# Wangkkklll/GausPcc

Measured on AMD Instinct MI355X. Metric: Mpoints/s encode+decode @1M anchors, higher is better.
Workload: dtype f32

## Files before the change

gauspcc_amd/csrc/codec.hip:

```cpp
#include <algorithm>
#include <chrono>

#include "hostcoder.hpp"
#include "codec_shared.hpp"
#include "container.hpp"
#include "rangecoder_dev.hpp"

using namespace gpcc;

namespace {

constexpr int ENC_RETRY_SMALLER_CHUNKS = -1000;
constexpr int DEC_RETRY_UNFUSED = -1001;

struct PosLevels {
    int L;
    uint32_t cbase[MAXLV], lohi_base[MAXLV], slots[MAXLV], nch[MAXLV];
    int clog[MAXLV];
    const uint32_t *m2r[MAXLV];
};

__global__ __launch_bounds__(256) void k_set_pos(PosLevels S, int64_t nC, uint32_t *__restrict__ pos_out, uint32_t *__restrict__ slots_out)
{
    const int64_t i = (int64_t)blockIdx.x * 256 + threadIdx.x;
// ... 70 lines not shown
    static const bool v0_device = dev_env_int("GAUSPCC_V0_DEVICE_CODER", 0) != 0;
    const int64_t no_origin[3] = {0, 0, 0};
    if (!chunk_log2 && !v0_device) {
        const Level *base = &T.lv[0];
        TAKE(base_xyz, int32_t, 3 * base->n);
        TAKE(base_occ, uint8_t, base->n);
        GP_TRY(level_to_raster(ctx, st, base, T.bias, base_xyz, base_occ));
        const size_t off_w = 0, off_pairs = ((size_t)4 * (size_t)std::max<int64_t>(lohi_words, 1) + 63) & ~(size_t)63;
        const size_t off_bx = off_pairs + 8 * (size_t)NCOUNTERS, off_bo = off_bx + 12 * (size_t)base->n;
        GP_TRY(ctx->hcoder.reserve(off_bo + (size_t)base->n + 64));
        uint8_t *hc = ctx->hcoder.p;
        {
            StageTimer tm(ctx, st, ST_CODER, (double)coded * 4 * 4);
            if (lohi_words) HIP_TRY(hipMemcpyAsync(hc + off_w, lohi, 4 * (size_t)lohi_words, hipMemcpyDeviceToHost, st));
        }
        HIP_TRY(hipMemcpyAsync(hc + off_pairs, pairs_dev, 8 * NCOUNTERS, hipMemcpyDeviceToHost, st));
        HIP_TRY(hipMemcpyAsync(hc + off_bx, base_xyz, 12 * (size_t)base->n, hipMemcpyDeviceToHost, st));
        HIP_TRY(hipMemcpyAsync(hc + off_bo, base_occ, (size_t)base->n, hipMemcpyDeviceToHost, st));
        ht.mark("enc all queued");
        HIP_TRY(hipStreamSynchronize(st));
        ht.mark("enc network done (sync)");
        std::vector<const uint32_t *> sp((size_t)std::max(nstreams, 1));
        std::vector<int64_t> sn((size_t)std::max(nstreams, 1));
        {
            const uint32_t *w = reinterpret_cast<const uint32_t *>(hc + off_w);
            int64_t pre = 0; int si = 0;
            for (int d = 1; d < L; ++d) {
                const int64_t nc = T.lv[d].n;
                for (int s = 0; s < 4; ++s, ++si) { sp[(size_t)si] = w + pre + (int64_t)s * nc; sn[(size_t)si] = nc; }
                pre += 4 * nc;
            }
        }
        std::vector<std::vector<uint8_t>> sb;
        GP_TRY(host_encode_streams(sp.data(), sn.data(), nstreams, &sb, 0));
        ht.mark("enc streams coded (host)");
        size_t fsize = 2 + 4 + 13 * (size_t)base->n + 2;
        for (int si = 0; si < nstreams; ++si) fsize += 4 + sb[(size_t)si].size();
        GP_TRY(ctx->hbytes.reserve(fsize + 16));
        uint8_t *out = ctx->hbytes.p;
        out[0] = (uint8_t)posq; out[1] = (uint8_t)(posq >> 8);
        size_t pos = 2 + base_block_put(out + 2, base->n, reinterpret_cast<const int32_t *>(hc + off_bx), no_origin, hc + off_bo, nstreams);
        for (int si = 0; si < nstreams; ++si) {
            const std::vector<uint8_t> &b = sb[(size_t)si];
            put32(out + pos, (uint32_t)b.size()); pos += 4;
            if (!b.empty()) memcpy(out + pos, b.data(), b.size());
            pos += b.size();
        }
        if (pos != fsize) return fail(GPCC_ERR_HIP, "internal: container size mismatch (%zu vs %zu)", pos, fsize);
        if (ctx->prof.on && ctx->prof.stages) ctx->prof.stage_bytes[ST_CODER] += 3.0 * (double)(fsize - (2 + 4 + 13 * (size_t)base->n + 2 + 4 * (size_t)nstreams));
        const unsigned long long *hp = reinterpret_cast<const unsigned long long *>(hc + off_pairs);
        unsigned long long set_pairs[2];
        sum_set_pairs(hp, L, set_pairs);
        if (ctx->prof.on) GP_TRY(prof_collect(ctx, set_pairs, 2));
        *bytes_out = out; *nbytes_out = (int64_t)pos;
        if (stats) fill_stats(stats, n, pos, T, coded, set_pairs, hp);
        return GPCC_OK;
    }
    LaneList lanes;
    std::vector<uint32_t> gaps;
    std::vector<uint32_t> stream_first(nstreams + 1, 0);
    {
        int64_t pre = 0; int si = 0;
        uint32_t gap = 0;
        for (int d = 1; d < L; ++d) {
            const int64_t nc = T.lv[d].n;
            const RcPlan pl = plan(nc);
            for (int s = 0; s < 4; ++s, ++si) {
                stream_first[si] = (uint32_t)lanes.chunks.size();
                gap += 4u;
                GP_TRY(lanes_append(&lanes, si, pre + (int64_t)s * slots(nc), nc, pl));
                gaps.insert(gaps.end(), pl.nlanes, chunk_log2 ? (uint32_t)si : gap);
            }
            pre += 4 * slots(nc);
        }
        stream_first[nstreams] = (uint32_t)lanes.chunks.size();
    }
    const std::vector<RcChunk> &chunks = lanes.chunks;
    const uint32_t max_syms = lanes.max_syms;
    const size_t table_bound = lanes.table_bound;
    const int nchunks = (int)chunks.size();
    const Level *base = &T.lv[0];
    TAKE(base_xyz, int32_t, 3 * base->n);
    TAKE(base_occ, uint8_t, base->n);
    GP_TRY(level_to_raster(ctx, st, base, T.bias, base_xyz, base_occ));
    const size_t off_desc = 0, off_cnt = off_desc + sizeof(RcChunk) * (size_t)std::max(nchunks, 1);
    const size_t off_pairs = off_cnt + 4 * (size_t)std::max(nchunks, 1) + 8, off_bx = off_pairs + 8 * NCOUNTERS, off_bo = off_bx + 12 * (size_t)base->n;
    const size_t off_gap = (off_bo + (size_t)base->n + 63) & ~(size_t)63;
    const size_t off_sf = off_gap + 4 * (size_t)std::max(nchunks, 1);
    GP_TRY(ctx->hstage.reserve(off_sf + 4 * (size_t)(nstreams + 1) + 64));
    const uint32_t gap_bound = 4u * (uint32_t)nstreams + (chunk_log2 ? (uint32_t)table_bound : 0u);
    uint8_t *hs = ctx->hstage.p;
    uint32_t total_payload = 0;
    uint8_t *payload_dev = nullptr;
    bool direct = false;
    const size_t pos0_hdr = (chunk_log2 ? 8 + 4 * (size_t)L + 4 : 2) + 4 + 13 * (size_t)base->n + 2;
    if (nchunks) {
        memcpy(hs + off_desc, chunks.data(), sizeof(RcChunk) * (size_t)nchunks);
        memcpy(hs + off_gap, gaps.data(), 4 * (size_t)nchunks);
        memcpy(hs + off_sf, stream_first.data(), 4 * (size_t)(nstreams + 1));
        const uint32_t stride = rc_scratch_stride(max_syms);
        TAKE(dchunks, RcChunk, nchunks);
        TAKE(dgap, uint32_t, nchunks);
        HIP_TRY(hipMemcpyAsync(dgap, hs + off_gap, 4 * (size_t)nchunks, hipMemcpyHostToDevice, st));
        TAKE(dcnt, uint32_t, nchunks + 1);
        TAKE(doff, uint32_t, nchunks + 1);
        TAKE(scratch, uint8_t, (size_t)nchunks * stride);
        HIP_TRY(hipMemcpyAsync(dchunks, hs + off_desc, sizeof(RcChunk) * (size_t)nchunks, hipMemcpyHostToDevice, st));
        StageTimer tm(ctx, st, ST_CODER, (double)coded * 4 * 4);
        GP_TRY(rc_encode_launch(st, lohi, dchunks, nchunks, scratch, stride, dcnt, chunk_log2 ? rc_coder_of_version(CONTAINER_VERSION) : RC_CODER_CARRYLESS));
        GP_TRY(dbg_mark(ctx, st, 10, dcnt, (size_t)nchunks * 4));
        GP_TRY(exclusive_scan_u32(ctx, st, dcnt, doff, nchunks, doff + nchunks));
        HIP_TRY(hipMemcpyAsync(hs + off_cnt, dcnt, 4 * (size_t)nchunks, hipMemcpyDeviceToHost, st));
        HIP_TRY(hipMemcpyAsync(hs + off_cnt + 4 * (size_t)nchunks, doff + nchunks, 4, hipMemcpyDeviceToHost, st));
        TAKE(payload, uint8_t, (size_t)nchunks * stride + gap_bound + 32);
        if (chunk_log2) {
            TAKE(dsf, uint32_t, nstreams + 1);
            TAKE(dlst, uint32_t, nchunks);
            TAKE(dgap_total, uint32_t, 1);
            HIP_TRY(hipMemcpyAsync(dsf, hs + off_sf, 4 * (size_t)(nstreams + 1), hipMemcpyHostToDevice, st));
            HIP_TRY(hipMemcpyAsync(dlst, hs + off_gap, 4 * (size_t)nchunks, hipMemcpyHostToDevice, st));
            GP_TRY(rc_layout_launch(st, dcnt, dsf, nstreams, dlst, nchunks, true, dgap, dgap_total));
            const size_t worst = pos0_hdr + (size_t)nchunks * stride + gap_bound + 64;
            GP_TRY(ctx->hbytes.reserve(worst));
            const uint32_t mis = (uint32_t)(pos0_hdr & 15);
            GP_TRY(rc_compact_launch(st, scratch, stride, dcnt, doff, dgap, nchunks, payload + mis, dchunks));
            GP_TRY(rc_to_host_launch(st, payload, doff + nchunks, mis, dgap_total, ctx->hbytes.p + (pos0_hdr - mis)));
            direct = true;
        } else {
            GP_TRY(rc_compact_launch(st, scratch, stride, dcnt, doff, dgap, nchunks, payload));
        }
        payload_dev = payload;
    }
    HIP_TRY(hipMemcpyAsync(hs + off_pairs, pairs_dev, 8 * NCOUNTERS, hipMemcpyDeviceToHost, st));
    HIP_TRY(hipMemcpyAsync(hs + off_bx, base_xyz, 12 * (size_t)base->n, hipMemcpyDeviceToHost, st));
    HIP_TRY(hipMemcpyAsync(hs + off_bo, base_occ, (size_t)base->n, hipMemcpyDeviceToHost, st));
    ht.mark("enc all queued");
    HIP_TRY(hipStreamSynchronize(st));
    ht.mark("enc coded (sync)");
    const uint32_t *hcnt = reinterpret_cast<const uint32_t *>(hs + off_cnt);
    if (nchunks) total_payload = hcnt[nchunks];
    if (ctx->prof.on && ctx->prof.stages) ctx->prof.stage_bytes[ST_CODER] += 3.0 * total_payload;
    const unsigned long long *hp = reinterpret_cast<const unsigned long long *>(hs + off_pairs);
    unsigned long long set_pairs[2];
    sum_set_pairs(hp, L, set_pairs);
    if (ctx->prof.on) GP_TRY(prof_collect(ctx, set_pairs, 2));
    std::vector<StreamSize> ssz((size_t)nstreams);
    size_t tables = 0;
    for (int si = 0; si < nstreams; ++si) {
        const StreamSize z = stream_size(hcnt, (int)stream_first[si], (int)stream_first[si + 1], si, chunk_log2 != 0);
        static const uint32_t test_cap = (uint32_t)env_int("GAUSPCC_TEST_CHUNK_BYTES", 0);
        if (!z.fits || (chunk_log2 > 7 && test_cap && z.max_chunk > test_cap)) {
            (void)fail(GPCC_ERR_ARG, "a chunk of stream %d takes %u bytes, more than the decoder's window holds at chunk_log2 = %d: use a smaller chunk_log2", si, z.max_chunk, chunk_log2);
            return ENC_RETRY_SMALLER_CHUNKS;
        }
        ssz[(size_t)si] = z;
        tables += z.tab;
    }
    size_t fsize = pos0_hdr + 4 * (size_t)nstreams + total_payload + tables;
    if (direct) { if (fsize + 16 > ctx->hbytes.cap) return fail(GPCC_ERR_HIP, "internal: payload beyond its bound"); }
    else GP_TRY(ctx->hbytes.reserve(fsize + 16));
    uint8_t *out = ctx->hbytes.p;
    size_t pos = 0;
    if (chunk_log2) {
        int64_t level_nodes[MAXLV];
        for (int d = 0; d < L; ++d) level_nodes[d] = T.lv[d].n;
        pos = chunked_header_put(out, CONTAINER_VERSION, chunk_log2, posq, L, level_nodes, n);
    } else {
        out[0] = (uint8_t)posq; out[1] = (uint8_t)(posq >> 8); pos = 2;
    }
    pos += base_block_put(out + pos, base->n, reinterpret_cast<const int32_t *>(hs + off_bx), no_origin, hs + off_bo, nstreams);
    {
        const size_t pos0 = pos, body = (size_t)total_payload + 4 * (size_t)nstreams + tables;
        if (pos0 != pos0_hdr) return fail(GPCC_ERR_HIP, "internal: header size mismatch");
        if (body && !direct) { HIP_TRY(hipMemcpyAsync(out + pos0, payload_dev, body, hipMemcpyDeviceToHost, st)); HIP_TRY(hipStreamSynchronize(st)); }
        size_t p = pos0;
        for (int si = 0; si < nstreams; ++si) {
            p += stream_head_put(out + p, hcnt, (int)stream_first[si], (int)stream_first[si + 1], ssz[(size_t)si], chunk_log2 != 0) + ssz[(size_t)si].pay;
        }
        pos = p;
    }
    ht.mark("enc payload d2h");
    if (pos != fsize) return fail(GPCC_ERR_HIP, "internal: container size mismatch (%zu vs %zu)", pos, fsize);
    *bytes_out = out; *nbytes_out = (int64_t)pos;
    if (stats) fill_stats(stats, n, pos, T, coded, set_pairs, hp);
    return GPCC_OK;
}

struct DecTail { const uint32_t *tot[MAXLV + 1]; int ntot; const unsigned long long *pairs; const uint32_t *tmo; };
__global__ __launch_bounds__(64) void k_dec_tail(DecTail t, uint32_t *__restrict__ h_tot, unsigned long long *__restrict__ h_pairs, uint32_t *__restrict__ h_tmo)
{
    const int l = (int)threadIdx.x;
    if (l < t.ntot) h_tot[l] = *t.tot[l];
    if (l < MAXLV) h_pairs[l] = t.pairs[l];
    if (l == 0) *h_tmo = t.tmo ? *t.tmo : 0u;
}

int decode_body(gpcc_ctx *ctx, const gpcc_model *m, const uint8_t *in, int64_t nbytes, const int32_t **xyz_out, int64_t *n_out,
                uint16_t *posq_out, gpcc_stats *stats, hipStream_t st, int32_t *out_user, int64_t out_cap)
{
    ctx->arena.reset();
    HostTrace ht;

    ContainerHdr hdr;
    GP_TRY(container_parse(in, nbytes, &hdr));
    const bool v1 = hdr.chunked;
    const int chunk_log2 = hdr.chunk_log2, version = hdr.version;
    const int L = hdr.L;
    int64_t lvl_n[MAXLV] = {0};
    for (int d = 0; d < MAXLV; ++d) lvl_n[d] = hdr.lvl_n[d];
    const int64_t npts_hdr = hdr.npts, bn = hdr.bn;
    const uint8_t *bxyz = hdr.bxyz, *bocc = hdr.bocc;
    const std::vector<int64_t> &s_len = hdr.s_len;
    *posq_out = hdr.posq;
    int64_t bias_base[3] = {CB >> L, CB >> L, CB >> L}, bias_leaf[3] = {CB, CB, CB};
    int64_t lo[3] = {INT64_MAX, INT64_MAX, INT64_MAX}, hi[3] = {INT64_MIN, INT64_MIN, INT64_MIN};
    {
        for (int64_t i = 0; i < bn; ++i)
            for (int a = 0; a < 3; ++a) { const int64_t c = (int32_t)get32(bxyz + 12 * i + 4 * a); lo[a] = std::min(lo[a], c); hi[a] = std::max(hi[a], c); }
        bool inside = true;
        for (int a = 0; a < 3; ++a) inside = inside && lo[a] + (int64_t)(CB >> L) >= 0 && hi[a] + (int64_t)(CB >> L) < ((int64_t)1 << (21 - L));
        if (!inside)
            for (int a = 0; a < 3; ++a) { bias_base[a] = -lo[a]; bias_leaf[a] = -lo[a] * ((int64_t)1 << L); }
    }
    std::vector<BaseNode> bnodes;
    GP_TRY(base_nodes_append(bxyz, bocc, bn, bias_base, (int64_t)1 << (21 - L), "", &bnodes));
    int hb = 1;
    for (int a = 0; a < 3; ++a) { int b = 0; uint64_t v = (uint64_t)(lo[a] + bias_base[a]) ^ (uint64_t)(hi[a] + bias_base[a]); while (v) { ++b; v >>= 1; } hb = std::max(hb, b); }

    TAKE(dbytes, uint8_t, nbytes + 16);
    GP_TRY(ctx->side_init());
    hipStream_t sd = ctx->side;
    SideGuard side_guard{sd, ctx->xfer};
    HIP_TRY(hipMemcpyAsync(dbytes, in, (size_t)nbytes, hipMemcpyHostToDevice, ctx->xfer));
    HIP_TRY(hipEventRecord(ctx->ev_bytes, ctx->xfer));
    size_t desc_total = 0;
    for (int g = 0; g + 1 < L; ++g) desc_total += 4 * (size_t)rc_plan(v1 ? lvl_n[g + 1] : 0, chunk_log2, version).nlanes;
    const size_t desc_off = (4096 + 16 * (size_t)bn + 63) & ~(size_t)63;
    GP_TRY(ctx->hstage.reserve(desc_off + sizeof(RcChunk) * desc_total + 64));
    RcChunk *hdesc = reinterpret_cast<RcChunk *>(ctx->hstage.p + desc_off);
    size_t desc_used = 0;
    uint32_t win_bytes[MAXLV][4] = {};
    auto level_chunks = [&](int g, int64_t nc, size_t *at) -> int {
        const RcPlan pl = rc_plan(nc, chunk_log2, version);
        if (desc_used + (size_t)4 * pl.nlanes > desc_total) return fail(GPCC_ERR_FORMAT, "level %d: chunk tables exceed the header's level sizes", g + 1);
        RcChunk *lanes = hdesc + desc_used;
        *at = desc_used;
        desc_used += (size_t)4 * pl.nlanes;
        GP_TRY(container_level_tables(in, hdr, g, nc, lanes, win_bytes[g]));
        return GPCC_OK;
    };
    RcChunk *dchunks_all = nullptr;
    size_t desc_at[MAXLV] = {0};
    if (v1 && L > 1) {
        for (int g = 0; g + 1 < L; ++g)
            if (lvl_n[g + 1] <= 0 || lvl_n[g + 1] > 8 * lvl_n[g]) return fail(GPCC_ERR_FORMAT, "bad node count at level %d", g + 1);
        TAKE(dca, RcChunk, std::max<size_t>(desc_total, 1));
        dchunks_all = dca;
    }
    constexpr int TAB_EARLY = 6;
    int tab_parsed = 0;
    auto upload_tables = [&](int g_end, hipEvent_t ev) -> int {
        const size_t from = desc_used;
        for (; tab_parsed < g_end && tab_parsed + 1 < L; ++tab_parsed) GP_TRY(level_chunks(tab_parsed, lvl_n[tab_parsed + 1], &desc_at[tab_parsed]));
        if (desc_used > from) HIP_TRY(hipMemcpyAsync(dchunks_all + from, hdesc + from, sizeof(RcChunk) * (desc_used - from), hipMemcpyHostToDevice, ctx->xfer));
        HIP_TRY(hipEventRecord(ev, ctx->xfer));
        return GPCC_OK;
    };
    Level cur;
    GP_TRY(alloc_level(ctx, &cur, bn, L));
    {
        uint64_t *hr = reinterpret_cast<uint64_t *>(ctx->hstage.p + 1024);
        uint8_t *ho = ctx->hstage.p + 1024 + 8 * (size_t)bn;
        for (int64_t i = 0; i < bn; ++i) { hr[i] = bnodes[(size_t)i].rk; ho[i] = bnodes[(size_t)i].occ; }
        HIP_TRY(hipMemcpyAsync(cur.rkey, hr, 8 * (size_t)bn, hipMemcpyHostToDevice, st));
        HIP_TRY(hipMemcpyAsync(cur.occ, ho, (size_t)bn, hipMemcpyHostToDevice, st));
        ht.mark("dec parse+h2d queued");
    }
    GP_TRY(level_raster_rank(ctx, st, &cur, hb));
    TAKE(dtotal, uint32_t, 4);
    uint32_t *htotal = reinterpret_cast<uint32_t *>(ctx->hstage.p);
    const int NPc = cell_map_entries(m->k);
    const int64_t zero_base[1] = {0};
    TAKE(pairs_dev, unsigned long long, MAXLV);
    HIP_TRY(hipMemsetAsync(pairs_dev, 0, sizeof(unsigned long long) * MAXLV, st));
    ConvTiles tilesP;
    int32_t *cellP = nullptr;
    {
        TAKE(cm, int32_t, (int64_t)NPc * bn);
        cellP = cm;
        const TileLevel tl = {&cur, nullptr, nullptr, cellP};
        const int R = conv_pick_rows(bn, m->k);
        TilePool pool;
        GP_TRY(tiles_build(ctx, st, &tl, 1, m->k, R, conv_pick_height(bn, R), &pool, pairs_dev));
        GP_TRY(tiles_view(ctx, st, pool, 0, 1, zero_base, &tilesP));
    }
    int64_t coded = 0;
    DecTail tail = {};
    const bool fuse_ctx = fused_enabled() && !ctx->fused_off && v1 && version >= 1 && m->C == 32;
    const int fmode = fused_mode();
    PairPlan planP;
    int64_t planP_np = 0;
    bool any_fused = false;
    HIP_TRY(hipEventRecord(ctx->ev_main, st));
    for (int g = 0; g + 1 < L; ++g) {
        const size_t top_mk = ctx->arena.top_mark();
        const int64_t np = cur.n;
        float *pA = nullptr;
        GP_TRY(dec_parent_trunk(ctx, st, m, g, cur.occ, np, tilesP, planP, planP_np, fmode, &pA, &any_fused));
        HIP_TRY(hipStreamWaitEvent(sd, ctx->ev_main, 0));
        Level chi;
        int64_t nc = lvl_n[g + 1];
        if (!v1) {
            GP_TRY(level_expand(ctx, sd, &cur, nullptr, dtotal));
            HIP_TRY(hipMemcpyAsync(htotal, dtotal, 4, hipMemcpyDeviceToHost, sd));
            HIP_TRY(hipStreamSynchronize(sd));
            nc = htotal[0];
            lvl_n[g + 1] = nc;
        }
        if (nc <= 0 || nc > 8 * cur.n) return fail(GPCC_ERR_FORMAT, "bad node count at level %d", g + 1);
        GP_TRY(alloc_level(ctx, &chi, nc, L - g - 1));
        {
            const int hbl = std::min(21, std::max(1, hb + g + 1));
            StageTimer tm(ctx, sd, ST_OCTREE, (double)np * 13 + (double)nc * 12 + (double)cdiv(3 * hbl, 8) * (double)nc * 24 + (double)nc * 8);
            GP_TRY(level_expand_rank(ctx, sd, &cur, &chi, v1 ? nullptr : dtotal, hb + g + 1));
            tail.tot[1 + g] = cur.cstart + np;
        }
        int32_t *cellC = nullptr;
        if (g + 2 < L) { TAKE(cm, int32_t, (int64_t)NPc * nc); cellC = cm; }
        if (v1 && g == 0) GP_TRY(upload_tables(TAB_EARLY, ctx->ev_bytes));
        const RcPlan pl = rc_plan(nc, chunk_log2, version);
        ConvTiles tilesC;
        PairPlan planC;
        const bool child_plan = fuse_ctx && fused_level_ok(nc, m->k) && pl.dual == (version >= 3) && fused_windows_fit(nc, cur.n, pl.nlanes, win_bytes[g]);
        GP_TRY(dec_child_lists(ctx, sd, m, &cur, cellP, &chi, cellC, child_plan, pairs_dev + g + 1, &planC, &tilesC));
        GP_TRY(dbg_mark(ctx, sd, g * 100 + 3, chi.rkey, (size_t)nc * 8)); GP_TRY(dbg_mark(ctx, sd, g * 100 + 4, chi.parent, (size_t)nc * 4));
        GP_TRY(dbg_mark(ctx, sd, g * 100 + 5, chi.m2r, (size_t)nc * 4));
        if (!child_plan) { GP_TRY(dbg_mark(ctx, sd, g * 100 + 6, tilesC.first, (size_t)(tilesC.nblk + 1) * 4)); GP_TRY(dbg_mark(ctx, sd, g * 100 + 7, tilesC.order, (size_t)tilesC.nblk * 4)); }
        HIP_TRY(hipEventRecord(ctx->ev_side, sd));
        HIP_TRY(hipStreamWaitEvent(st, ctx->ev_side, 0));
        const int64_t S = chunk_log2 ? (int64_t)1 << pl.llog : nc;
        const int nch = (int)pl.nlanes;
        const int clog = pl.llog;
        const RcChunk *dchunks = nullptr;
        if (v1) {
            dchunks = dchunks_all + desc_at[g];
        } else {
            size_t at = 0;
            GP_TRY(level_chunks(g, nc, &at));
            TAKE(dch, RcChunk, 4 * nch);
            HIP_TRY(hipMemcpyAsync(dch, hdesc + at, sizeof(RcChunk) * 4 * (size_t)nch, hipMemcpyHostToDevice, st));
            dchunks = dch;
        }
        LevelCoder lc = {nullptr, nullptr, (uint32_t)nch, clog, dchunks, {win_bytes[g][0], win_bytes[g][1], win_bytes[g][2], win_bytes[g][3]}, pl.dual, rc_coder_of_version(version)};
        ChildBufs cb;
        GP_TRY(child_bufs_take(ctx, m, nc, child_plan ? planC.pcap : 0, lc.nlanes, S, nc + 4, &cb));
        uint8_t *const *sym = cb.sym;
        uint16_t *const cdf = cb.cdf;
        if (child_plan && fmode == 1) {
            if (g == 0) HIP_TRY(hipStreamWaitEvent(st, ctx->ev_bytes, 0));
            if (g == TAB_EARLY) HIP_TRY(hipStreamWaitEvent(st, ctx->ev_tables, 0));
            GP_TRY(dec_child_fused(ctx, st, m, g, planC, pA, np, chi, dbytes, lc, cb));
            any_fused = true;
        } else {
        GP_TRY(dec_child_trunk(ctx, st, m, g, pA, chi, tilesC, child_plan ? &planC : nullptr, cb));
        for (int s = 0; s < 4; ++s) {
            GP_TRY(dec_child_stage(ctx, st, m, g, s, chi, tilesC, child_plan ? &planC : nullptr, lc, cb));
            const int row_bytes = stage_row_bytes(s);
            if (g == 0 && s == 0) HIP_TRY(hipStreamWaitEvent(st, ctx->ev_bytes, 0));
            if (g == TAB_EARLY && s == 0) HIP_TRY(hipStreamWaitEvent(st, ctx->ev_tables, 0));
            static const bool v0_device = dev_env_int("GAUSPCC_V0_DEVICE_CODER", 0) != 0;
            if (!v1 && !v0_device) {
                const int lp = STAGE_M[s] + 1, rs = rc_row_stride(lp);
                const size_t rows_b = (size_t)nc * (size_t)rs * 2, off_sym = (rows_b + 63) & ~(size_t)63;
                {
                    const size_t need = off_sym + (size_t)nc + 64;
                    if (need > ctx->hcoder.cap) GP_TRY(ctx->hcoder.reserve(std::max(need, 4 * ctx->hcoder.cap)));
                }
                StageTimer tm(ctx, st, ST_CODER, (double)nc * (row_bytes + 1) + (double)s_len[4 * g + s]);
                HIP_TRY(hipMemcpyAsync(ctx->hcoder.p, cdf, rows_b, hipMemcpyDeviceToHost, st));
                HIP_TRY(hipStreamSynchronize(st));
                GP_TRY(host_decode_compact(reinterpret_cast<const uint16_t *>(ctx->hcoder.p), lp, in + hdr.s_off[(size_t)(4 * g + s)], s_len[(size_t)(4 * g + s)], nc,
                                           ctx->hcoder.p + off_sym));
                HIP_TRY(hipMemcpyAsync(sym[s], ctx->hcoder.p + off_sym, (size_t)nc, hipMemcpyHostToDevice, st));
                HIP_TRY(hipStreamSynchronize(st));
            } else {
                StageTimer tm(ctx, st, ST_CODER, (double)nc * (row_bytes + 1) + (double)s_len[4 * g + s]);
                GP_TRY(rc_decode_launch(st, cdf, STAGE_M[s] + 1, dbytes, dchunks + (size_t)s * nch, nch, win_bytes[g][s], pl.dual, sym[s], rc_coder_of_version(version)));
            }
            GP_TRY(dbg_mark(ctx, st, g * 100 + 14 + 5 * s, sym[s], (size_t)nc));
        }
        { StageTimer tm(ctx, st, ST_ELEM, (double)nc * (4 + 4 + 1)); GP_TRY(assemble_occ(st, sym, chi.m2r, nc, chi.occ)); }
        }
        GP_TRY(dbg_mark(ctx, st, g * 100 + 30, chi.occ, (size_t)nc));
        HIP_TRY(hipEventRecord(ctx->ev_main, st));
        if (v1 && g == 0) GP_TRY(upload_tables(L, ctx->ev_tables));
        ctx->arena.top_rewind(top_mk);
        coded += nc;
        cur = chi; cellP = cellC; tilesP = tilesC; planP = child_plan ? planC : PairPlan(); planP_np = np;
        ht.mark("dec level queued", g + 1, nc);
    }
    GP_TRY(level_expand(ctx, st, &cur, nullptr, v1 ? nullptr : dtotal));
    if (!v1) HIP_TRY(hipMemcpyAsync(htotal, dtotal, 4, hipMemcpyDeviceToHost, st));
    tail.tot[0] = cur.cstart + cur.n;
    int64_t npts = npts_hdr;
    if (!v1) {
        HIP_TRY(hipStreamSynchronize(st));
        ht.mark("dec levels done (sync)");
        npts = htotal[0];
    }
    int32_t *xyz = out_user;
    if (out_user) {
        if (npts > out_cap) return fail(GPCC_ERR_ARG, "decoded %lld points, the output buffer holds %lld", (long long)npts, (long long)out_cap);
    } else {
        TAKE(own, int32_t, 3 * std::max<int64_t>(npts, 1));
        xyz = own;
    }
    GP_TRY(leaves_reference_order(ctx, st, &cur, bias_leaf, xyz, npts));
    unsigned long long *hpairs = reinterpret_cast<unsigned long long *>(ctx->hstage.p + 512);
    static_assert(512 + sizeof(unsigned long long) * MAXLV <= 1024, "hpairs sits in front of the base level's staging bytes");
    htotal[40] = 0;
    if (v1) {
        tail.ntot = L; tail.pairs = pairs_dev; tail.tmo = any_fused ? fused_timeout_word(ctx) : nullptr;
        k_dec_tail<<<1, 64, 0, st>>>(tail, htotal, hpairs, htotal + 40);
        LAUNCH_CHECK();
    } else {
        HIP_TRY(hipMemcpyAsync(hpairs, pairs_dev, sizeof(unsigned long long) * MAXLV, hipMemcpyDeviceToHost, st));
        if (any_fused && fused_timeout_word(ctx)) HIP_TRY(hipMemcpyAsync(htotal + 40, fused_timeout_word(ctx), 4, hipMemcpyDeviceToHost, st));
    }
    HIP_TRY(hipStreamSynchronize(st));
    ht.mark("dec leaves done (sync)");
    if (htotal[40]) {
        ctx->fused_off = true;
        GP_TRY(fused_reset(ctx, st));
        return DEC_RETRY_UNFUSED;
    }
    if (v1) {
        for (int g = 0; g + 1 < L; ++g)
            if (htotal[1 + g] != (uint32_t)lvl_n[g + 1])
                return fail(GPCC_ERR_FORMAT, "level %d: header says %lld nodes, occupancy expands to %u", g + 1, (long long)lvl_n[g + 1], htotal[1 + g]);
        if ((int64_t)htotal[0] != npts_hdr) return fail(GPCC_ERR_FORMAT, "decoded %lld points, header says %lld", (long long)htotal[0], (long long)npts_hdr);
    }
    if (ctx->prof.on) GP_TRY(prof_collect(ctx, hpairs, L));
    ht.mark("dec prof collect");
    *xyz_out = xyz; *n_out = npts;
    if (stats) {
        memset(stats, 0, sizeof *stats);
        stats->num_points = npts; stats->num_bytes = nbytes; stats->num_levels = L; stats->coded_nodes = coded;
        int64_t cp = 0;
        for (int d = 0; d < L; ++d) {
            stats->level_nodes[d] = lvl_n[d];
            cp += (int64_t)hpairs[d] * ((d + 1 < L ? 5 : 0) + (d > 0 ? 13 : 0));
        }
        stats->conv_pairs = cp;
    }
    return GPCC_OK;
}

}

extern "C" int gpcc_encode(gpcc_ctx *ctx, const gpcc_model *m, const int32_t *xyz_dev, int64_t n, int chunk_log2, uint16_t posq_f16,
                           const uint8_t **bytes_out, int64_t *nbytes_out, gpcc_stats *stats, void *stream)
{
    if (!ctx || !m || !xyz_dev || !bytes_out || !nbytes_out) return fail(GPCC_ERR_ARG, "null argument");
    if (chunk_log2 != 0 && (chunk_log2 < 6 || chunk_log2 > 14)) return fail(GPCC_ERR_ARG, "chunk_log2 must be 0 or 6..14");
    HIP_TRY(hipSetDevice(ctx->device));
    hipStream_t st = (hipStream_t)stream;
    const auto t0 = std::chrono::steady_clock::now();
    size_t want = arena_scaled(arena_estimate(n, m->K));
    int rc = GPCC_OK;
    for (int attempt = 0; attempt < 6; ++attempt) {
        GP_TRY(ctx->arena.reserve(want));
        rc = encode_body(ctx, m, xyz_dev, n, chunk_log2, posq_f16, bytes_out, nbytes_out, stats, st);
        if (rc == ENC_RETRY_SMALLER_CHUNKS) {
            HIP_TRY(hipStreamSynchronize(st));
            if (chunk_log2 <= 6) { rc = GPCC_ERR_ARG; break; }
            chunk_log2 -= 1; attempt -= 1;
            continue;
        }
        if (rc != GPCC_ERR_NOMEM) break;
        HIP_TRY(hipStreamSynchronize(st));
        want *= 2;
    }
    if (rc == GPCC_OK && stats) stats->device_ms = std::chrono::duration<double, std::milli>(std::chrono::steady_clock::now() - t0).count();
    if (const int de = device_error_check(ctx)) rc = de;
    return rc;
}

static int decode_entry(gpcc_ctx *ctx, const gpcc_model *m, const uint8_t *bytes, int64_t nbytes, const int32_t **xyz_dev_out,
                        int64_t *n_out, uint16_t *posq_f16_out, gpcc_stats *stats, void *stream, int32_t *out_user, int64_t out_cap)
{
    HIP_TRY(hipSetDevice(ctx->device));
    hipStream_t st = (hipStream_t)stream;
    const auto t0 = std::chrono::steady_clock::now();
    size_t want = arena_estimate(std::max<int64_t>(nbytes, 1 << 16), m->K);
    int64_t nodes = 0, nmax = 0, npts = 0;
    const int pre = container_precheck(bytes, nbytes, &nodes, &nmax, &npts);
    if (pre < 0) return pre;
    if (pre > 0) {
        const int L = bytes[6];
        want = (size_t)nmax * 2600 + (size_t)nodes * (size_t)(4 * 125 + m->K * 81 / 16 + 96) + (size_t)npts * 32 + (size_t)nbytes + ((size_t)48 << 20);
        if (fused_enabled()) {
            int64_t nf = 0;
            for (int d = 0; d < L; ++d) { const int64_t v = get32(bytes + 8 + 4 * d); if (fused_level_ok(v, m->k)) nf = std::max(nf, v); }
            want += (size_t)nf * (size_t)m->K * (128 + 10 + 9) + ((size_t)4 << 20);
        }
    }
    want = arena_scaled(want);
    ctx->fused_note_decode();
    int rc = GPCC_OK;
    const int32_t *xyz = nullptr;
    for (int attempt = 0; attempt < 6; ++attempt) {
        GP_TRY(ctx->arena.reserve(want));
        rc = decode_body(ctx, m, bytes, nbytes, &xyz, n_out, posq_f16_out, stats, st, out_user, out_cap);
        if (rc == DEC_RETRY_UNFUSED) {
            fused_timeout_notice(ctx);
            attempt -= 1;
            continue;
        }
        if (rc != GPCC_ERR_NOMEM) break;
        HIP_TRY(hipStreamSynchronize(st));
        want *= 2;
    }
    if (rc == GPCC_OK && xyz_dev_out) *xyz_dev_out = xyz;
    if (rc == GPCC_OK && stats) stats->device_ms = std::chrono::duration<double, std::milli>(std::chrono::steady_clock::now() - t0).count();
    if (const int de = device_error_check(ctx)) rc = de;
    return rc;
}

extern "C" int gpcc_decode(gpcc_ctx *ctx, const gpcc_model *m, const uint8_t *bytes, int64_t nbytes, const int32_t **xyz_dev_out,
                           int64_t *n_out, uint16_t *posq_f16_out, gpcc_stats *stats, void *stream)
{
    if (!ctx || !m || !bytes || !xyz_dev_out || !n_out || !posq_f16_out) return fail(GPCC_ERR_ARG, "null argument");
    return decode_entry(ctx, m, bytes, nbytes, xyz_dev_out, n_out, posq_f16_out, stats, stream, nullptr, 0);
}

extern "C" int gpcc_decode_to(gpcc_ctx *ctx, const gpcc_model *m, const uint8_t *bytes, int64_t nbytes, int32_t *xyz_dev, int64_t capacity_points,
                              int64_t *n_out, uint16_t *posq_f16_out, gpcc_stats *stats, void *stream)
{
    if (!ctx || !m || !bytes || !xyz_dev || capacity_points < 0 || !n_out || !posq_f16_out) return fail(GPCC_ERR_ARG, "null argument");
    return decode_entry(ctx, m, bytes, nbytes, nullptr, n_out, posq_f16_out, stats, stream, xyz_dev, capacity_points);
}
```

gauspcc_amd/csrc/codec_batch.hip:

```cpp
#include <algorithm>
#include <chrono>

#include "codec_shared.hpp"
#include "container.hpp"
#include "forest.hpp"
#include "rangecoder_dev.hpp"

using namespace gpcc;

extern "C" int gpcc_encode(gpcc_ctx *ctx, const gpcc_model *m, const int32_t *xyz_dev, int64_t n, int chunk_log2, uint16_t posq_f16, const uint8_t **bytes_out, int64_t *nbytes_out,
                           gpcc_stats *stats, void *stream);
extern "C" int gpcc_decode_to(gpcc_ctx *ctx, const gpcc_model *m, const uint8_t *bytes, int64_t nbytes, int32_t *xyz_dev, int64_t capacity_points, int64_t *n_out,
                              uint16_t *posq_f16_out, gpcc_stats *stats, void *stream);

namespace {

constexpr int BATCH_SOLO = -2001;
constexpr int BATCH_RETRY_UNFUSED = -2002;

struct FPosArgs {
    int L;
    uint32_t cbase[MAXLV];
    const uint32_t *m2r[MAXLV];
    const ForestSeg *seg[MAXLV];
// ... 173 lines not shown
    HIP_TRY(hipStreamSynchronize(st));
    ht.mark("benc coded (sync)");
    const uint32_t *hcnt = reinterpret_cast<const uint32_t *>(hs + off_cnt);
    unsigned long long set_pairs[2];
    sum_set_pairs(reinterpret_cast<const unsigned long long *>(hs + off_pairs), L, set_pairs);
    if (ctx->prof.on) GP_TRY(prof_collect(ctx, set_pairs, 2));
    uint8_t *out = ctx->hbytes.p;
    size_t pos = 0;
    const int32_t *hbx = reinterpret_cast<const int32_t *>(hs + off_bx);
    const uint8_t *hbo = hs + off_bo;
    for (int u = 0; u < K; ++u) {
        const int qi = internal_of[(size_t)u];
        const ForestScene &sc = F.sc[(size_t)qi];
        offsets_out[u] = (int64_t)pos;
        if (pos + hdr_bytes[(size_t)u] > ctx->hbytes.cap) return fail(GPCC_ERR_HIP, "internal: container beyond its bound");
        uint8_t *o = out + pos;
        size_t p = chunked_header_put(o, CONTAINER_VERSION, chunk_log2, posq[u], sc.L, sc.n, sc.npts);
        const uint32_t r0 = F.row0[0][(size_t)qi];
        const int64_t origin[3] = {sc.bias[0] >> sc.L, sc.bias[1] >> sc.L, sc.bias[2] >> sc.L};
        p += base_block_put(o + p, sc.n[0], hbx + 3 * (size_t)r0, origin, hbo + r0, 4 * (sc.L - 1));
        if (p != hdr_bytes[(size_t)u]) return fail(GPCC_ERR_HIP, "internal: header size mismatch");
        pos += p;
        for (size_t si = scene_stream0[(size_t)u]; si < scene_stream0[(size_t)u + 1]; ++si) {
            const int c0 = (int)stream_first[si], c1 = (int)stream_first[si + 1];
            const StreamSize z = stream_size(hcnt, c0, c1, (int)si, true);
            if (!z.fits) return BATCH_SOLO;
            if (pos + 4 + z.tab + z.pay > ctx->hbytes.cap) return fail(GPCC_ERR_HIP, "internal: container beyond its bound");
            pos += stream_head_put(out + pos, hcnt, c0, c1, z, true) + z.pay;
        }
        if (stats) {
            gpcc_stats *s = &stats[u];
            memset(s, 0, sizeof *s);
            s->num_points = sc.npts; s->num_bytes = (int64_t)pos - offsets_out[u]; s->num_levels = sc.L;
            for (int d = 0; d < sc.L; ++d) { s->level_nodes[d] = sc.n[d]; if (d) s->coded_nodes += sc.n[d]; }
        }
    }
    offsets_out[K] = (int64_t)pos;
    if (nchunks) {
        const size_t expect = (size_t)hcnt[nchunks] + hdr_total + 4 * (size_t)nstreams;
        if (pos < expect) return fail(GPCC_ERR_HIP, "internal: blob size mismatch (%zu below %zu)", pos, expect);
    }
    if (stats) stats[0].conv_pairs = (int64_t)set_pairs[0] * 5 + (int64_t)set_pairs[1] * 13;
    *bytes_out = out;
    return GPCC_OK;
}

int parse_chunked(const uint8_t *in, int64_t nbytes, int scene, ContainerHdr *h)
{
    const int rc = container_parse(in, nbytes, h);
    if (rc != GPCC_OK) { char msg[400]; snprintf(msg, sizeof msg, "%s", g_err); return fail(rc, "scene %d: %s", scene, msg); }
    if (!h->chunked) return BATCH_SOLO;
    int64_t nodes = 0;
    for (int d = 0; d < h->L; ++d) nodes += h->lvl_n[d];
    if (nodes > (nbytes << 13)) return fail(GPCC_ERR_FORMAT, "scene %d: header: %lld nodes cannot come from %lld bytes", scene, (long long)nodes, (long long)nbytes);
    return GPCC_OK;
}


struct BDecTail { const uint32_t *tot[MAXLV]; int ntot; const uint32_t *bounds_flag, *leaf_cnt; int K; const unsigned long long *pairs; const uint32_t *tmo; };
__global__ __launch_bounds__(64) void k_bdec_tail(BDecTail t, uint32_t *__restrict__ h_leaf, uint32_t *__restrict__ h_lvl, unsigned long long *__restrict__ h_pairs,
                                                  uint32_t *__restrict__ h_tmo)
{
    const int l = (int)threadIdx.x;
    for (int i = l; i < t.K; i += 64) h_leaf[i] = t.leaf_cnt[i];
    if (l < MAXLV) {
        h_lvl[l] = l == MAXLV - 1 ? *t.bounds_flag : l < t.ntot ? *t.tot[l] : 0u;
        h_pairs[l] = t.pairs[l];
    }
    if (l == 0) *h_tmo = t.tmo ? *t.tmo : 0u;
}

int decode_batch_body(gpcc_ctx *ctx, const gpcc_model *m, const uint8_t *const *in, const int64_t *nbytes, int K, int32_t *const *xyz_out, const int64_t *cap_out, int64_t *n_out,
                      uint16_t *posq_out, gpcc_stats *stats, hipStream_t st)
{
    ctx->arena.reset();
    HostTrace ht;
    std::vector<ContainerHdr> H((size_t)K);
    int64_t blob = 0;
    for (int u = 0; u < K; ++u) {
        GP_TRY(parse_chunked(in[u], nbytes[u], u, &H[(size_t)u]));
        if (H[(size_t)u].version != H[0].version) return BATCH_SOLO;
        if (cap_out[u] < H[(size_t)u].npts) return fail(GPCC_ERR_ARG, "scene %d: %lld points, the output buffer holds %lld", u, (long long)H[(size_t)u].npts, (long long)cap_out[u]);
        if (H[(size_t)u].L > 20) return BATCH_SOLO;
        blob += (nbytes[u] + 15) & ~(int64_t)15;
    }
    if (blob >= (int64_t)1 << 32) return BATCH_SOLO;
    const int version = H[0].version;
    std::vector<int> order((size_t)K);
    for (int u = 0; u < K; ++u) order[(size_t)u] = u;
    std::stable_sort(order.begin(), order.end(), [&](int a, int b) { return H[(size_t)a].L > H[(size_t)b].L; });
    Forest F;
    F.K = K; F.sc.resize((size_t)K);
    const int L = H[(size_t)order[0]].L;
    F.L = L;
    std::vector<BaseNode> bnodes;
    std::vector<uint32_t> bparent;
    std::vector<uint64_t> root_rk;
    std::vector<uint8_t> root_occ;
    std::vector<uint32_t> root_cs;
    F.root0.assign((size_t)K + 1, 0u);
    int64_t zcur = 0, xymax = 0;
    for (int qi = 0; qi < K; ++qi) {
        const int u = order[(size_t)qi];
        const ContainerHdr &h = H[(size_t)u];
        ForestScene &sc = F.sc[(size_t)qi];
        sc.user = u; sc.L = h.L; sc.npts = h.npts;
        for (int d = 0; d < h.L; ++d) sc.n[d] = h.lvl_n[d];
        int64_t lo[3] = {INT64_MAX, INT64_MAX, INT64_MAX}, hi[3] = {INT64_MIN, INT64_MIN, INT64_MIN};
        for (int64_t i = 0; i < h.bn; ++i)
            for (int a = 0; a < 3; ++a) { const int64_t c = (int32_t)get32(h.bxyz + 12 * i + 4 * a); lo[a] = std::min(lo[a], c); hi[a] = std::max(hi[a], c); }
        int64_t tz = 0;
        if (!forest_place(h.L, 0, hi[2] - lo[2], &zcur, &tz)) return BATCH_SOLO;
        for (int a = 0; a < 2; ++a) {
            if (((hi[a] - lo[a] + 1) << (h.L - 1)) > ((int64_t)1 << 21)) return BATCH_SOLO;
            xymax = std::max(xymax, hi[a] - lo[a]);
        }
        const int64_t t3[3] = {-lo[0], -lo[1], -lo[2] + tz};
        for (int a = 0; a < 3; ++a) sc.bias[a] = t3[a] * ((int64_t)1 << h.L);
        const size_t b0 = bnodes.size();
        char who[24];
        snprintf(who, sizeof who, "scene %d: ", u);
        GP_TRY(base_nodes_append(h.bxyz, h.bocc, h.bn, t3, (int64_t)1 << 21, who, &bnodes));
        F.root0[(size_t)qi] = (uint32_t)root_rk.size();
        for (size_t i = b0; i < bnodes.size(); ++i) {
            const uint64_t pk = bnodes[i].mk >> 3;
            if (i == b0 || (bnodes[i - 1].mk >> 3) != pk) {
                root_rk.push_back(rkey3(compact1by2(pk), compact1by2(pk >> 1), compact1by2(pk >> 2)));
                root_occ.push_back(0);
                root_cs.push_back((uint32_t)i);
            }
            root_occ.back() |= (uint8_t)(1u << (bnodes[i].mk & 7));
            bparent.push_back((uint32_t)root_rk.size() - 1u);
        }
        sc.nroot = (int64_t)root_rk.size() - F.root0[(size_t)qi];
    }
    F.root0[(size_t)K] = (uint32_t)root_rk.size();
    root_cs.push_back((uint32_t)bnodes.size());
    F.hb0 = 1;
    { int64_t v = std::max(zcur, xymax + 1); while (((int64_t)1 << F.hb0) < v + 1) ++F.hb0; }
    for (int d = 0; d <= L + 1; ++d) F.Kd[d] = 0;
    for (int qi = 0; qi < K; ++qi) for (int d = 0; d < F.sc[(size_t)qi].L; ++d) F.Kd[d] = qi + 1;
    int64_t lvl_n[MAXLV] = {0};
    int64_t total_pts = 0;
    for (int d = 0; d < L; ++d) {
        F.row0[d].assign((size_t)F.Kd[d] + 1, 0u);
        int64_t acc = 0;
        for (int qi = 0; qi < F.Kd[d]; ++qi) { F.row0[d][(size_t)qi] = (uint32_t)acc; acc += F.sc[(size_t)qi].n[d]; }
        if (acc >= (int64_t)1 << 31) return BATCH_SOLO;
        F.row0[d][(size_t)F.Kd[d]] = (uint32_t)acc;
        lvl_n[d] = acc;
    }
    for (int qi = 0; qi < K; ++qi) total_pts += F.sc[(size_t)qi].npts;
    F.npts = total_pts;
    const int64_t bn = lvl_n[0], nroot = (int64_t)root_rk.size();

    std::vector<ForestSeg> seg[MAXLV];
    uint32_t nch_tot[MAXLV] = {0}, smax[MAXLV] = {0};
    int64_t symlen[MAXLV] = {0};
    std::vector<int> clog2_of((size_t)K);
    for (int qi = 0; qi < K; ++qi) clog2_of[(size_t)qi] = H[(size_t)order[(size_t)qi]].chunk_log2;
    for (int d = 0; d < L; ++d) {
        seg[d].resize((size_t)F.Kd[d] + 1);
        uint32_t lane0 = 0;
        int64_t sym0 = 0;
        for (int qi = 0; qi < F.Kd[d]; ++qi) {
            ForestSeg &s = seg[d][(size_t)qi];
            s = ForestSeg{};
            s.row0 = F.row0[d][(size_t)qi];
            if (d) {
                const int64_t nc = F.sc[(size_t)qi].n[d];
                const RcPlan p = rc_plan(nc, clog2_of[(size_t)qi], version);
                if (p.dual != (version >= 3) || p.llog < 4) return BATCH_SOLO;
                s.lane0 = lane0; s.nlanes = p.nlanes; s.llog = p.llog; s.base = (uint32_t)sym0;
                lane0 += p.nlanes;
                smax[d] = std::max(smax[d], 1u << p.llog);
                sym0 = (sym0 + nc + 4 + 15) & ~(int64_t)15;
            }
        }
        ForestSeg &e = seg[d][(size_t)F.Kd[d]];
        e = ForestSeg{}; e.row0 = (uint32_t)lvl_n[d];
        nch_tot[d] = lane0; symlen[d] = sym0 + 16;
    }
    size_t desc_total = 0;
    for (int d = 1; d < L; ++d) desc_total += 4 * (size_t)nch_tot[d];
    const size_t pin_seg = 0, pin_seg_b = (size_t)MAXLV * (K + 1) * sizeof(ForestSeg);
    const size_t pin_leaf = pin_seg + pin_seg_b, pin_leaf_b = (size_t)K * sizeof(ForestLeafScene);
    const size_t pin_base = (pin_leaf + pin_leaf_b + 63) & ~(size_t)63, pin_base_b = (size_t)bn * (8 + 1 + 4) + (size_t)nroot * (8 + 1) + (size_t)(nroot + 1) * 4 + (size_t)(K + 1) * 4 + 64;
    const size_t pin_desc = (pin_base + pin_base_b + 63) & ~(size_t)63, pin_desc_b = sizeof(RcChunk) * std::max<size_t>(desc_total, 1);
    const size_t pin_cnt = (pin_desc + pin_desc_b + 63) & ~(size_t)63, pin_cnt_b = 4 * (size_t)(K + MAXLV * (K + 1) + MAXLV + 64) + 8 * (size_t)MAXLV + 8;
    GP_TRY(ctx->hbatch.reserve(pin_cnt + pin_cnt_b + 64));
    uint8_t *pin = ctx->hbatch.p;
    GP_TRY(ctx->side_init());
    hipStream_t sd = ctx->side;
    SideGuard side_guard{sd, ctx->xfer};
    TAKE(dbytes, uint8_t, blob + 16);
    std::vector<int64_t> byte0((size_t)K);
    {
        int64_t at = 0;
        for (int u = 0; u < K; ++u) {
            byte0[(size_t)u] = at;
            HIP_TRY(hipMemcpyAsync(dbytes + at, in[u], (size_t)nbytes[u], hipMemcpyHostToDevice, ctx->xfer));
            at += (nbytes[u] + 15) & ~(int64_t)15;
        }
    }
    RcChunk *hdesc = reinterpret_cast<RcChunk *>(pin + pin_desc);
    size_t desc_at[MAXLV + 1] = {0};
    uint32_t win_bytes[MAXLV][4] = {};
    for (int d = 1; d < L; ++d) desc_at[d + 1] = desc_at[d] + 4 * (size_t)nch_tot[d];
    TAKE(dchunks_all, RcChunk, std::max<size_t>(desc_total, 1));
    constexpr int TAB_EARLY = 5;
    auto parse_levels = [&](int d0, int d1, hipEvent_t ev) -> int {
        std::vector<RcChunk> tmp;
        for (int d = d0; d < d1; ++d) {
            const size_t at = desc_at[d];
            for (int qi = 0; qi < F.Kd[d]; ++qi) {
                const int u = order[(size_t)qi];
                const ContainerHdr &h = H[(size_t)u];
                const int64_t nc = F.sc[(size_t)qi].n[d];
                const RcPlan pl = rc_plan(nc, h.chunk_log2, version);
                const ForestSeg &sg = seg[d][(size_t)qi];
                tmp.resize(pl.nlanes);
                for (int s = 0; s < 4; ++s) {
                    const int si = 4 * (d - 1) + s;
                    uint32_t wb = 0;
                    const char *err = rc_parse_table(in[u] + h.s_off[(size_t)si], h.s_off[(size_t)si], h.s_len[(size_t)si], pl, nc, version, tmp.data(), &wb);
                    if (err) return fail(GPCC_ERR_FORMAT, "scene %d stream %d: %s", u, si, err);
                    win_bytes[d][s] = std::max(win_bytes[d][s], wb);
                    RcChunk *dst = hdesc + at + (size_t)s * nch_tot[d] + sg.lane0;
                    for (uint32_t l = 0; l < pl.nlanes; ++l) {
                        RcChunk c = tmp[l];
                        c.first = sg.lane0 + l; c.stride = nch_tot[d];
                        c.out = sg.base + (l << pl.llog);
                        c.byte_off += (uint32_t)byte0[(size_t)u];
                        dst[l] = c;
                    }
                }
            }
        }
        if (d1 > d0 && desc_at[d1] > desc_at[d0])
            HIP_TRY(hipMemcpyAsync(dchunks_all + desc_at[d0], hdesc + desc_at[d0], sizeof(RcChunk) * (desc_at[d1] - desc_at[d0]), hipMemcpyHostToDevice, ctx->xfer));
        HIP_TRY(hipEventRecord(ev, ctx->xfer));
        return GPCC_OK;
    };
    const int d_early = std::min(L, 1 + TAB_EARLY);
    GP_TRY(forest_upload_segs(ctx, st, &F, seg, pin + pin_seg, pin_seg_b));
    Tree &T = F.T;
    T.L = L; T.npts = total_pts; T.hb = std::min(21, F.hb0 + L);
    Level &cur0 = T.lv[0];
    GP_TRY(alloc_level(ctx, &cur0, bn, L));
    GP_TRY(alloc_level(ctx, &F.root, nroot, L + 1));
    TAKE(droot0, uint32_t, K + 1);
    {
        uint8_t *p = pin + pin_base;
        uint64_t *h_rk = reinterpret_cast<uint64_t *>(p); p += 8 * (size_t)bn;
        uint64_t *h_rrk = reinterpret_cast<uint64_t *>(p); p += 8 * (size_t)nroot;
        uint32_t *h_par = reinterpret_cast<uint32_t *>(p); p += 4 * (size_t)bn;
        uint32_t *h_rcs = reinterpret_cast<uint32_t *>(p); p += 4 * (size_t)(nroot + 1);
        uint32_t *h_r0 = reinterpret_cast<uint32_t *>(p); p += 4 * (size_t)(K + 1);
        uint8_t *h_occ = p; p += (size_t)bn;
        uint8_t *h_rocc = p;
        for (int64_t i = 0; i < bn; ++i) { h_rk[i] = bnodes[(size_t)i].rk; h_occ[i] = bnodes[(size_t)i].occ; h_par[i] = bparent[(size_t)i]; }
        for (int64_t i = 0; i < nroot; ++i) { h_rrk[i] = root_rk[(size_t)i]; h_rocc[i] = root_occ[(size_t)i]; }
        for (int64_t i = 0; i <= nroot; ++i) h_rcs[i] = root_cs[(size_t)i];
        for (int qi = 0; qi <= K; ++qi) h_r0[qi] = F.root0[(size_t)qi];
        HIP_TRY(hipMemcpyAsync(cur0.rkey, h_rk, 8 * (size_t)bn, hipMemcpyHostToDevice, st));
        HIP_TRY(hipMemcpyAsync(cur0.occ, h_occ, (size_t)bn, hipMemcpyHostToDevice, st));
        HIP_TRY(hipMemcpyAsync(cur0.parent, h_par, 4 * (size_t)bn, hipMemcpyHostToDevice, st));
        HIP_TRY(hipMemcpyAsync(F.root.rkey, h_rrk, 8 * (size_t)nroot, hipMemcpyHostToDevice, st));
        HIP_TRY(hipMemcpyAsync(F.root.occ, h_rocc, (size_t)nroot, hipMemcpyHostToDevice, st));
        HIP_TRY(hipMemcpyAsync(F.root.cstart, h_rcs, 4 * (size_t)(nroot + 1), hipMemcpyHostToDevice, st));
        HIP_TRY(hipMemcpyAsync(droot0, h_r0, 4 * (size_t)(K + 1), hipMemcpyHostToDevice, st));
    }
    const int NPc = cell_map_entries(m->k);
    TAKE(cell_root, int32_t, (int64_t)NPc * nroot);
    F.cell_root = cell_root;
    GP_TRY(forest_root_cells(ctx, st, &F.root, droot0, K, m->k, cell_root));
    GP_TRY(level_raster_rank(ctx, st, &cur0, F.hb0));
    ht.mark("bdec parse+h2d queued");
    TAKE(dtotal, uint32_t, 4);
    TAKE(dlevel_tot, uint32_t, MAXLV);
    HIP_TRY(hipMemsetAsync(dlevel_tot, 0, 4 * (size_t)MAXLV, st));
    const int64_t zero_base[1] = {0};
    TAKE(pairs_dev, unsigned long long, MAXLV);
    HIP_TRY(hipMemsetAsync(pairs_dev, 0, sizeof(unsigned long long) * MAXLV, st));
    ConvTiles tilesP;
    int32_t *cellP = nullptr;
    {
        TAKE(cm, int32_t, (int64_t)NPc * bn);
        cellP = cm;
        const TileLevel tl = {&cur0, &F.root, cell_root, cellP};
        const int R = conv_pick_rows(bn, m->k);
        TilePool pool;
        GP_TRY(tiles_build(ctx, st, &tl, 1, m->k, R, conv_pick_height(bn, R), &pool, pairs_dev));
        GP_TRY(tiles_view(ctx, st, pool, 0, 1, zero_base, &tilesP));
    }
    const bool fuse_ctx = fused_enabled() && !ctx->fused_off && m->C == 32;
    const int fmode = fused_mode();
    PairPlan planP;
    int64_t planP_np = 0;
    bool any_fused = false;
    BDecTail tail = {};
    HIP_TRY(hipEventRecord(ctx->ev_main, st));
    GP_TRY(parse_levels(1, d_early, ctx->ev_bytes));
    for (int g = 0; g + 1 < L; ++g) {
        const size_t top_mk = ctx->arena.top_mark();
        Level &cur = T.lv[g];
        const int64_t np = cur.n;
        const int64_t np_in = F.inner(g);
        float *pA = nullptr;
        GP_TRY(dec_parent_trunk(ctx, st, m, g, cur.occ, np, tilesP, planP, planP_np, fmode, &pA, &any_fused));
        HIP_TRY(hipStreamWaitEvent(sd, ctx->ev_main, 0));
        Level &chi = T.lv[g + 1];
        const int64_t nc = lvl_n[g + 1];
        GP_TRY(alloc_level(ctx, &chi, nc, L - g - 1));
        {
            Level pv = cur; pv.n = np_in;
            StageTimer tm(ctx, sd, ST_OCTREE, (double)np * 13 + (double)nc * 12 + (double)nc * 8);
            GP_TRY(level_expand_rank(ctx, sd, &pv, &chi, nullptr, F.hb0 + g + 1));
            tail.tot[g] = cur.cstart + np_in;
            GP_TRY(forest_check_bounds(sd, cur.cstart, F.seg_dev[g], F.seg_dev[g + 1], F.Kd[g + 1], dlevel_tot + MAXLV - 1));
        }
        int32_t *cellC = nullptr;
        if (g + 2 < L) { TAKE(cm, int32_t, (int64_t)NPc * nc); cellC = cm; }
        ConvTiles tilesC;
        PairPlan planC;
        const bool child_plan = fuse_ctx && fused_level_ok(nc, m->k) && fused_windows_fit(nc, cur.n, nch_tot[g + 1], win_bytes[g + 1]);
        GP_TRY(dec_child_lists(ctx, sd, m, &cur, cellP, &chi, cellC, child_plan, pairs_dev + g + 1, &planC, &tilesC));
        TAKE(cpos, uint32_t, nc);
        TAKE(spos, uint32_t, nc);
        GP_TRY(forest_cdf_pos(sd, F.seg_dev[g + 1], F.Kd[g + 1], chi.m2r, nc, nch_tot[g + 1], cpos, spos));
        HIP_TRY(hipEventRecord(ctx->ev_side, sd));
        HIP_TRY(hipStreamWaitEvent(st, ctx->ev_side, 0));
        const int64_t S = smax[g + 1];
        const int nch = (int)nch_tot[g + 1];
        const RcChunk *dchunks = dchunks_all + desc_at[g + 1];
        LevelCoder lc = {spos, cpos, (uint32_t)nch, 4, dchunks, {win_bytes[g + 1][0], win_bytes[g + 1][1], win_bytes[g + 1][2], win_bytes[g + 1][3]}, version >= 3, rc_coder_of_version(version)};
        ChildBufs cb;
        GP_TRY(child_bufs_take(ctx, m, nc, child_plan ? planC.pcap : 0, lc.nlanes, S, symlen[g + 1], &cb));
        if (g + 1 == d_early && d_early < L) HIP_TRY(hipStreamWaitEvent(st, ctx->ev_tables, 0));
        if (child_plan && fmode == 1) {
            if (g == 0) HIP_TRY(hipStreamWaitEvent(st, ctx->ev_bytes, 0));
            GP_TRY(dec_child_fused(ctx, st, m, g, planC, pA, np, chi, dbytes, lc, cb));
            any_fused = true;
        } else {
            GP_TRY(dec_child_trunk(ctx, st, m, g, pA, chi, tilesC, child_plan ? &planC : nullptr, cb));
            for (int s = 0; s < 4; ++s) {
                GP_TRY(dec_child_stage(ctx, st, m, g, s, chi, tilesC, child_plan ? &planC : nullptr, lc, cb));
                if (g == 0 && s == 0) HIP_TRY(hipStreamWaitEvent(st, ctx->ev_bytes, 0));
                StageTimer tm(ctx, st, ST_CODER, (double)nc * (stage_row_bytes(s) + 1));
                GP_TRY(rc_decode_launch(st, cb.cdf, STAGE_M[s] + 1, dbytes, dchunks + (size_t)s * nch, nch, lc.win_bytes[s], lc.dual, cb.sym[s], lc.coder));
            }
            { StageTimer tm(ctx, st, ST_ELEM, (double)nc * (4 + 4 + 1)); GP_TRY(assemble_occ(st, cb.sym, spos, nc, chi.occ)); }
        }
        HIP_TRY(hipEventRecord(ctx->ev_main, st));
        if (g == 0 && d_early < L) GP_TRY(parse_levels(d_early, L, ctx->ev_tables));
        ctx->arena.top_rewind(top_mk);
        cellP = cellC; tilesP = tilesC; planP = child_plan ? planC : PairPlan(); planP_np = np;
        ht.mark("bdec level queued", g + 1, nc);
    }
    ForestLeafScene *hleaf = reinterpret_cast<ForestLeafScene *>(pin + pin_leaf);
    TAKE(dleaf, ForestLeafScene, K);
    TAKE(dleaf_cnt, uint32_t, K);
    HIP_TRY(hipMemsetAsync(dleaf_cnt, 0, 4 * (size_t)K, st));
    for (int qi = 0; qi < K; ++qi) {
        const ForestScene &sc = F.sc[(size_t)qi];
        ForestLeafScene &ls = hleaf[qi];
        ls.rank0 = F.row0[sc.L - 1][(size_t)qi];
        ls.xyz = xyz_out[sc.user]; ls.cap = std::min<int64_t>(cap_out[sc.user], sc.npts);
        for (int a = 0; a < 3; ++a) ls.bias[a] = sc.bias[a];
    }
    HIP_TRY(hipMemcpyAsync(dleaf, hleaf, sizeof(ForestLeafScene) * (size_t)K, hipMemcpyHostToDevice, st));
    for (int d = 0; d < L; ++d) {
        const int q0 = d + 1 < L ? F.Kd[d + 1] : 0, q1 = F.Kd[d];
        if (q1 <= q0) continue;
        GP_TRY(forest_leaves(ctx, st, &T.lv[d], (int64_t)F.row0[d][(size_t)q0], dleaf + q0, q1 - q0, dleaf_cnt + q0));
    }
    uint32_t *hcnt = reinterpret_cast<uint32_t *>(pin + pin_cnt);
    uint32_t *h_leaf = hcnt, *h_lvl = hcnt + K;

    unsigned long long *hpairs = reinterpret_cast<unsigned long long *>(pin + ((pin_cnt + 4 * (size_t)(K + MAXLV * (K + 1) + MAXLV + 64) + 7) & ~(size_t)7));
    uint32_t *h_tmo = hcnt + K + MAXLV;
    *h_tmo = 0;
    tail.ntot = L - 1; tail.bounds_flag = dlevel_tot + MAXLV - 1; tail.leaf_cnt = dleaf_cnt; tail.K = K; tail.pairs = pairs_dev;
    tail.tmo = any_fused ? fused_timeout_word(ctx) : nullptr;
    k_bdec_tail<<<1, 64, 0, st>>>(tail, h_leaf, h_lvl, hpairs, h_tmo);
    LAUNCH_CHECK();
    HIP_TRY(hipStreamSynchronize(st));
    ht.mark("bdec leaves done (sync)");
    if (*h_tmo) {
        ctx->fused_off = true;
        GP_TRY(fused_reset(ctx, st));
        return BATCH_RETRY_UNFUSED;
    }
    for (int g = 0; g + 1 < L; ++g)
        if (h_lvl[g] != (uint32_t)lvl_n[g + 1]) return fail(GPCC_ERR_FORMAT, "level %d: the headers say %lld nodes, the occupancy expands to %u", g + 1, (long long)lvl_n[g + 1], h_lvl[g]);
    if (h_lvl[MAXLV - 1]) return fail(GPCC_ERR_FORMAT, "a scene's occupancy expands to a node count its header does not state");
    for (int qi = 0; qi < K; ++qi)
        if ((int64_t)h_leaf[qi] != F.sc[(size_t)qi].npts) return fail(GPCC_ERR_FORMAT, "scene %d: decoded %u points, header says %lld", F.sc[(size_t)qi].user, h_leaf[qi], (long long)F.sc[(size_t)qi].npts);
    if (ctx->prof.on) GP_TRY(prof_collect(ctx, hpairs, L));
    for (int u = 0; u < K; ++u) {
        const ContainerHdr &h = H[(size_t)u];
        n_out[u] = h.npts; posq_out[u] = h.posq;
        if (stats) {
            gpcc_stats *s = &stats[u];
            memset(s, 0, sizeof *s);
            s->num_points = h.npts; s->num_bytes = nbytes[u]; s->num_levels = h.L;
            for (int d = 0; d < h.L; ++d) { s->level_nodes[d] = h.lvl_n[d]; if (d) s->coded_nodes += h.lvl_n[d]; }
        }
    }
    if (stats) {
        int64_t cp = 0;
        for (int d = 0; d < L; ++d) cp += (int64_t)hpairs[d] * ((d + 1 < L ? 5 : 0) + (d > 0 ? 13 : 0));
        stats[0].conv_pairs = cp;
    }
    return GPCC_OK;
}

}

extern "C" int gpcc_encode_batch(gpcc_ctx *ctx, const gpcc_model *m, const int32_t *const *xyz_dev, const int64_t *n, int nscenes, int chunk_log2, const uint16_t *posq_f16,
                                 const uint8_t **bytes_out, int64_t *offsets_out, gpcc_stats *stats, int *batched_out, void *stream)
{
    if (!ctx || !m || !xyz_dev || !n || !posq_f16 || !bytes_out || !offsets_out || nscenes < 1) return fail(GPCC_ERR_ARG, "null argument");
    if (chunk_log2 != 0 && (chunk_log2 < 6 || chunk_log2 > 14)) return fail(GPCC_ERR_ARG, "chunk_log2 must be 0 or 6..14");
    HIP_TRY(hipSetDevice(ctx->device));
    hipStream_t st = (hipStream_t)stream;
    const auto t0 = std::chrono::steady_clock::now();
    int rc = BATCH_SOLO;
    if (batched_out) *batched_out = 0;
    static const bool never = env_int("GAUSPCC_BATCH", 1) == 0;
    if (chunk_log2 != 0 && nscenes <= FOREST_MAX_SCENES && !never) {
        int64_t total = 0;
        for (int q = 0; q < nscenes; ++q) total += n[q] > 0 ? n[q] : 0;
        size_t want = arena_scaled(arena_estimate(total, m->K) + (size_t)total * 40 + (size_t)nscenes * 65536);
        for (int attempt = 0; attempt < 6; ++attempt) {
            GP_TRY(ctx->arena.reserve(want));
            rc = encode_batch_body(ctx, m, xyz_dev, n, nscenes, chunk_log2, posq_f16, bytes_out, offsets_out, stats, st);
            if (rc != GPCC_ERR_NOMEM) break;
            HIP_TRY(hipStreamSynchronize(st));
            want *= 2;
        }
        if (rc == GPCC_OK && batched_out) *batched_out = 1;
        if (rc == FOREST_UNFIT) rc = BATCH_SOLO;
    }
    if (rc == BATCH_SOLO) {
        HIP_TRY(hipStreamSynchronize(st));
        static thread_local std::vector<uint8_t> blob;
        blob.clear();
        for (int q = 0; q < nscenes; ++q) {
            const uint8_t *b = nullptr; int64_t nb = 0;
            gpcc_stats s1; memset(&s1, 0, sizeof s1);
            const int r1 = gpcc_encode(ctx, m, xyz_dev[q], n[q], chunk_log2, posq_f16[q], &b, &nb, &s1, stream);
            if (r1 != GPCC_OK) {
                char msg[400]; snprintf(msg, sizeof msg, "%s", g_err);
                return fail(r1, "scene %d: %s", q, msg);
            }
            offsets_out[q] = (int64_t)blob.size();
            blob.insert(blob.end(), b, b + nb);
            if (stats) stats[q] = s1;
        }
        offsets_out[nscenes] = (int64_t)blob.size();
        GP_TRY(ctx->hbytes.reserve(blob.size() + 16));
        memcpy(ctx->hbytes.p, blob.data(), blob.size());
        *bytes_out = ctx->hbytes.p;
        rc = GPCC_OK;
    }
    if (rc == GPCC_OK && stats) stats[0].device_ms = std::chrono::duration<double, std::milli>(std::chrono::steady_clock::now() - t0).count();
    if (const int de = device_error_check(ctx)) rc = de;
    return rc;
}

extern "C" int gpcc_decode_batch(gpcc_ctx *ctx, const gpcc_model *m, const uint8_t *const *bytes, const int64_t *nbytes, int nscenes, int32_t *const *xyz_dev,
                                 const int64_t *capacity_points, int64_t *n_out, uint16_t *posq_f16_out, gpcc_stats *stats, int *batched_out, void *stream)
{
    if (!ctx || !m || !bytes || !nbytes || !xyz_dev || !capacity_points || !n_out || !posq_f16_out || nscenes < 1) return fail(GPCC_ERR_ARG, "null argument");
    for (int q = 0; q < nscenes; ++q) if (!bytes[q] || !xyz_dev[q] || capacity_points[q] < 0 || nbytes[q] < 0) return fail(GPCC_ERR_ARG, "scene %d: null argument", q);
    HIP_TRY(hipSetDevice(ctx->device));
    hipStream_t st = (hipStream_t)stream;
    const auto t0 = std::chrono::steady_clock::now();
    int rc = BATCH_SOLO;
    if (batched_out) *batched_out = 0;
    static const bool never = env_int("GAUSPCC_BATCH", 1) == 0;
    if (nscenes <= FOREST_MAX_SCENES && !never) {
        int64_t nodes = 0, nmax_sum[MAXLV] = {0}, total_bytes = 0, npts = 0;
        bool ok = true;
        for (int q = 0; q < nscenes && ok; ++q) {
            const uint8_t *b = bytes[q];
            total_bytes += nbytes[q];
            if (!(nbytes[q] >= 8 && b[0] == 0xFF && b[1] == 0xFF && b[6] >= 1 && b[6] <= 21 && nbytes[q] >= 12 + 4 * (int64_t)b[6])) { ok = false; break; }
            const int L = b[6];
            int64_t prev = 0, mine = 0;
            for (int d = 0; d < L; ++d) {
                const int64_t v = get32(b + 8 + 4 * d);
                if (v <= 0 || (d == 0 ? v >= 64 : v > 8 * prev)) { ok = false; break; }
                mine += v; nmax_sum[d] += v; prev = v;
            }
            if (!ok) break;
            const int64_t np = get32(b + 8 + 4 * L);
            if (np < 1 || np > 8 * prev || mine > (nbytes[q] << 13)) { ok = false; break; }
            nodes += mine; npts += np;
        }
        if (ok) {
            ctx->fused_note_decode();
            int64_t nmax = 0;
            for (int d = 0; d < MAXLV; ++d) nmax = std::max(nmax, nmax_sum[d]);
            size_t want = arena_scaled((size_t)nmax * 2700 + (size_t)nodes * (size_t)(4 * 125 + m->K * 81 / 16 + 96) + (size_t)npts * 32 + (size_t)total_bytes + (size_t)nscenes * 65536 + ((size_t)48 << 20));
            if (fused_enabled()) {
                int64_t nf = 0;
                for (int d = 0; d < MAXLV; ++d) if (nmax_sum[d] > 0 && fused_level_ok(nmax_sum[d], m->k)) nf = std::max(nf, nmax_sum[d]);
                want += (size_t)nf * (size_t)m->K * (128 + 10 + 9) + ((size_t)4 << 20);
            }
            for (int attempt = 0; attempt < 6; ++attempt) {
                GP_TRY(ctx->arena.reserve(want));
                rc = decode_batch_body(ctx, m, bytes, nbytes, nscenes, xyz_dev, capacity_points, n_out, posq_f16_out, stats, st);
                if (rc == BATCH_RETRY_UNFUSED) {
                    fused_timeout_notice(ctx);
                    attempt -= 1;
                    continue;
                }
                if (rc != GPCC_ERR_NOMEM) break;
                HIP_TRY(hipStreamSynchronize(st));
                want *= 2;
            }
            if (rc == GPCC_OK && batched_out) *batched_out = 1;
        }
    }
    if (rc == BATCH_SOLO) {
        HIP_TRY(hipStreamSynchronize(st));
        for (int q = 0; q < nscenes; ++q) {
            gpcc_stats s1; memset(&s1, 0, sizeof s1);
            const int r1 = gpcc_decode_to(ctx, m, bytes[q], nbytes[q], xyz_dev[q], capacity_points[q], &n_out[q], &posq_f16_out[q], &s1, stream);
            if (r1 != GPCC_OK) {
                char msg[400]; snprintf(msg, sizeof msg, "%s", g_err);
                return fail(r1, "scene %d: %s", q, msg);
            }
            if (stats) stats[q] = s1;
        }
        rc = GPCC_OK;
    }
    if (rc == GPCC_OK && stats) stats[0].device_ms = std::chrono::duration<double, std::milli>(std::chrono::steady_clock::now() - t0).count();
    if (const int de = device_error_check(ctx)) rc = de;
    return rc;
}
```

gauspcc_amd/csrc/codec_shared.hip:

```cpp
#include <algorithm>

#include "codec_shared.hpp"

namespace gpcc {

size_t arena_scaled(size_t want)
{
    static const double scale = [] { const char *e = getenv("GAUSPCC_ARENA_SCALE"); const double v = e ? atof(e) : 1.0; return v > 0.0 ? v : 1.0; }();
    return scale == 1.0 ? want : std::max<size_t>((size_t)((double)want * scale), (size_t)1 << 20);
}

void fused_timeout_notice(const gpcc_ctx *ctx)
{
    static const bool loud = getenv("GAUSPCC_FUSED_QUIET") == nullptr;
    if (loud) fprintf(stderr, "[gauspcc] a persistent small-level launch timed out on device %d; the launch-per-layer path serves this context's next %d decodes\n", ctx->device, ctx->fused_rearm_after);
}

int tile_sets(gpcc_ctx *ctx, hipStream_t st, const Tree &T, const Level *root, const int32_t *cell_root, int k, unsigned long long *pairs_dev, TilePool *pool, ConvTiles *setP,
              ConvTiles *setC)
{
    const int L = T.L, NPc = cell_map_entries(k);
    TileLevel tl[MAXLV];
    int64_t pb[MAXLV] = {0}, cb[MAXLV] = {0};
    const int32_t *cell_prev = cell_root;
    for (int d = 0; d < L; ++d) {
        int32_t *own = nullptr;
        if (d + 1 < L) { TAKE(cm, int32_t, (int64_t)NPc * T.lv[d].n); own = cm; }
        tl[d] = TileLevel{&T.lv[d], d ? &T.lv[d - 1] : root, cell_prev, own};
        cell_prev = own;
        if (d + 1 < L) { pb[d + 1] = pb[d] + T.lv[d].n; cb[d + 1] = cb[d] + T.lv[d + 1].n; }
    }
    const int64_t nC = cb[L - 1];
    const int R = conv_pick_rows(nC, k), H = conv_pick_height(nC, R);
    GP_TRY(tiles_build(ctx, st, tl, L, k, R, H, pool, pairs_dev));
    GP_TRY(tiles_view(ctx, st, *pool, 0, L - 1, pb, setP));
    GP_TRY(tiles_view(ctx, st, *pool, 1, L, cb, setC));
    return GPCC_OK;
}

namespace {

struct SetLevels {
    int L;
    uint32_t n[MAXLV], pb[MAXLV], cbase[MAXLV];
    const uint8_t *occ[MAXLV];
    const uint64_t *rkey[MAXLV];
    const uint32_t *parent[MAXLV];
};

__global__ __launch_bounds__(256) void k_set_rows(SetLevels S, int64_t nP, int64_t nC, uint8_t *__restrict__ occP, uint8_t *__restrict__ occC, uint64_t *__restrict__ rkeyC,
                                                  uint32_t *__restrict__ parentC)
{
    const int64_t i = (int64_t)blockIdx.x * 256 + threadIdx.x;
    if (i < nP) {
        int d = 0;
        for (int q = 1; q + 1 < S.L; ++q) d = i >= (int64_t)S.pb[q] ? q : d;
        occP[i] = S.occ[d][i - S.pb[d]];
    }
    if (i < nC) {
        int d = 1;
        for (int q = 2; q < S.L; ++q) d = i >= (int64_t)S.cbase[q] ? q : d;
        const int64_t j = i - S.cbase[d];
        occC[i] = S.occ[d][j];
        rkeyC[i] = S.rkey[d][j];
        parentC[i] = S.pb[d - 1] + S.parent[d][j];
    }
}

}

int encode_network(gpcc_ctx *ctx, const gpcc_model *m, hipStream_t st, hipStream_t sd, const EncodeNet &a)
{
    const Tree &T = *a.T;
    const int L = T.L;
    auto mark = [&](const char *what) {
        if (!a.ht->on) return;
        char label[48];
        snprintf(label, sizeof label, "%s %s", a.trace, what);
        a.ht->mark(label);
    };
    SetLevels S = {};
    S.L = L;
    int64_t nP = 0, nC = 0;
    for (int d = 0; d < L; ++d) {
        const Level *lv = &T.lv[d];
        S.n[d] = (uint32_t)lv->n; S.pb[d] = (uint32_t)nP; S.cbase[d] = (uint32_t)nC;
        S.occ[d] = lv->occ; S.rkey[d] = lv->rkey; S.parent[d] = lv->parent;
        if (d + 1 < L) nP += lv->n;
        if (d) nC += lv->n;
    }
    TAKE(occP, uint8_t, nP); TAKE(occC, uint8_t, nC); TAKE(rkeyC, uint64_t, nC);
    TAKE(parentC, uint32_t, nC); TAKE(posC, uint32_t, nC); TAKE(slotsC, uint32_t, nC);
    {
        StageTimer tm(ctx, st, ST_ELEM, (double)nP * 2 + (double)nC * (2 + 16 + 8));
        k_set_rows<<<(unsigned)cdiv(std::max(nP, nC), 256), 256, 0, st>>>(S, nP, nC, occP, occC, rkeyC, parentC);
        LAUNCH_CHECK();
    }
    HIP_TRY(hipEventRecord(ctx->ev_main, st));
    mark("meta queued");
    ConvTiles tilesP, tilesC;
    {
        TilePool pool;
        StageTimer tm(ctx, st, ST_TILES, 0.0);
        GP_TRY(tile_sets(ctx, st, T, a.root, a.cell_root, m->k, a.pairs_dev, &pool, &tilesP, &tilesC));
        tm.add_bytes(pool.alg_bytes);
    }
    mark("tiles built");
    TAKE(pF, float, nP * m->C); TAKE(pA, float, nP * m->C); TAKE(pB, float, nP * m->C);
    { StageTimer tm(ctx, st, ST_ELEM, (double)nP * 129); GP_TRY(embed_occ(st, m->prior_emb, occP, nP, pF, m->C)); }
    GP_TRY(run_trunk(ctx, 0, st, m, 0, Trunk{pF, pA, pB}, tilesP, nP));
    {
        HIP_TRY(hipStreamWaitEvent(sd, ctx->ev_main, 0));
        ctx->arena.flip = true;
        int rc = GPCC_OK;
        {
            StageTimer tm(ctx, sd, ST_OCTREE, 0.0);
            rc = a.ranks(sd);
        }
        ctx->arena.flip = false;
        GP_TRY(rc);
        {
            StageTimer tm(ctx, sd, ST_ELEM, (double)nC * (4 + 8));
            GP_TRY(a.set_pos(sd, posC, slotsC));
        }
        HIP_TRY(hipEventRecord(ctx->ev_side, sd));
    }
    TAKE(cX, float, nC * m->C); TAKE(cA, float, nC * m->C); TAKE(cB, float, nC * m->C);
    { StageTimer tm(ctx, st, ST_ELEM, (double)nC * (128 + 12 + 128)); GP_TRY(child_features(st, pA, parentC, rkeyC, m->temb, nC, cX, m->C)); }
    GP_TRY(run_trunk(ctx, 1, st, m, 5, Trunk{cX, cA, cB}, tilesC, nC));
    TAKE(u1, float, nC * m->C); TAKE(u2, float, nC * m->C); TAKE(u3, float, nC * m->C);
    TAKE(v1, float, nC * m->C); TAKE(v2, float, nC * m->C);
    float *u[4] = {cA, u1, u2, u3};
    float *v[4] = {cX, cB, v1, v2};
    {
        const float *const embs[3] = {m->semb[0], m->semb[1], m->semb[2]};
        float *const outs[3] = {u1, u2, u3};
        StageTimer tm(ctx, st, ST_ELEM, (double)nC * (128 + 1 + 3 * 128));
        GP_TRY(stage_inputs_gt(st, cA, embs, occC, nC, outs, m->C));
    }
    ConvBatch cb = {}; cb.C = m->C;
    for (int s = 0; s < 4; ++s) cb.job[s] = ConvJob{u[s], m->conv[10 + 2 * s], nullptr, v[s]};
    GP_TRY(sparse_conv(ctx, 1, st, cb, 4, tilesC, nC, 1));
    TAKE(y0, float, nC * m->C);
    float *y[4] = {y0, u1, u2, u3};
    for (int s = 0; s < 4; ++s) cb.job[s] = ConvJob{v[s], m->conv[10 + 2 * s + 1], nullptr, y[s]};
    GP_TRY(sparse_conv(ctx, 1, st, cb, 4, tilesC, nC, 0));
    GP_TRY(dbg_mark(ctx, st, 1, pA, (size_t)nP * 128)); GP_TRY(dbg_mark(ctx, st, 2, cA, (size_t)nC * 128));
    for (int s = 0; s < 4; ++s) GP_TRY(dbg_mark(ctx, st, 3 + s, y[s], (size_t)nC * 128));
    HIP_TRY(hipStreamWaitEvent(st, ctx->ev_side, 0));
    GP_TRY(dbg_mark(ctx, st, 7, posC, (size_t)nC * 4)); GP_TRY(dbg_mark(ctx, st, 8, slotsC, (size_t)nC * 4));
    ctx->arena.release_top_low();
    StageTimer tm_heads(ctx, st, ST_HEADS, (double)nC * 4 * (128 + 1 + 8 + 4));
    for (int s = 0; s < 4; ++s) {
        HeadArgs ha = {}; ha.C = m->C;
        ha.x = y[s]; ha.n = nC; ha.stage_m = STAGE_M[s];
        ha.w1 = m->hw1[s]; ha.b1 = m->hb1[s]; ha.w2 = m->hw2[s]; ha.b2 = m->hb2[s]; ha.frag = m->hfrag[s];
        ha.occ = occC; ha.stage = s; ha.lohi = a.lohi; ha.mode = 0; ha.pos = posC; ha.slots = slotsC;
        ha.bits = a.bits;
        GP_TRY(head_cdf(st, ha));
    }
    return GPCC_OK;
}

int lanes_append(LaneList *ll, int si, int64_t first_slot, int64_t nc, const RcPlan &pl)
{
    ll->table_bound += 6 * (size_t)pl.nchunks + 8;
    if (pl.dual && ((first_slot & 1) || pl.llog < 4)) return fail(GPCC_ERR_HIP, "internal: stream %d starts on an odd slot or has lanes below 16 symbols", si);
    for (uint32_t c = 0; c < pl.nlanes; ++c) {
        const int64_t cn = pl.lane_syms(nc, c);
        ll->chunks.push_back(RcChunk{(uint32_t)(first_slot + c), pl.nlanes, (uint32_t)cn, 0, 0, 0});
        ll->max_syms = std::max<uint32_t>(ll->max_syms, (uint32_t)cn);
    }
    return GPCC_OK;
}

StreamSize stream_size(const uint32_t *hcnt, int c0, int c1, int si, bool chunked)
{
    StreamSize z;
    for (int c = c0; c < c1; ++c) z.pay += hcnt[c];
    if (!chunked) return z;
    const uint32_t nch = (uint32_t)((c1 - c0 + 1) / 2);
    for (uint32_t c = 0; c < nch; ++c) z.max_chunk = std::max(z.max_chunk, chunk_bytes(hcnt, c0, c1, c));
    z.fits = rc_window_fits(STAGE_M[si & 3] + 1, z.max_chunk);
    z.tab = rc_table_size([&](uint32_t c) { return chunk_bytes(hcnt, c0, c1, c); }, nch);
    return z;
}

size_t stream_head_put(uint8_t *o, const uint32_t *hcnt, int c0, int c1, const StreamSize &z, bool chunked)
{
    put32(o, (uint32_t)(z.tab + z.pay));
    return 4 + (chunked ? rc_table_put(o + 4, [&](uint32_t c) { return chunk_bytes(hcnt, c0, c1, c); }, (uint32_t)((c1 - c0 + 1) / 2)) : 0);
}

size_t chunked_header_put(uint8_t *o, int version, int chunk_log2, uint16_t posq, int L, const int64_t *level_nodes, int64_t npts)
{
    o[0] = 0xFF; o[1] = 0xFF; o[2] = (uint8_t)version; o[3] = (uint8_t)chunk_log2; o[4] = (uint8_t)posq; o[5] = (uint8_t)(posq >> 8); o[6] = (uint8_t)L; o[7] = 0;
    size_t p = 8;
    for (int d = 0; d < L; ++d) { put32(o + p, (uint32_t)level_nodes[d]); p += 4; }
    put32(o + p, (uint32_t)npts); p += 4;
    return p;
}

size_t base_block_put(uint8_t *o, int64_t bn, const int32_t *xyz, const int64_t origin[3], const uint8_t *occ, int nstreams)
{
    size_t p = 0;
    put32(o + p, (uint32_t)bn); p += 4;
    for (int64_t i = 0; i < bn; ++i)
        for (int a = 0; a < 3; ++a) { put32(o + p, (uint32_t)((int64_t)xyz[3 * i + a] - origin[a])); p += 4; }
    memcpy(o + p, occ, (size_t)bn); p += (size_t)bn;
    o[p] = (uint8_t)nstreams; o[p + 1] = (uint8_t)(nstreams >> 8); p += 2;
    return p;
}

void sum_set_pairs(const unsigned long long *per_level, int L, unsigned long long set_pairs[2])
{
    set_pairs[0] = set_pairs[1] = 0;
    for (int d = 0; d < L; ++d) { if (d + 1 < L) set_pairs[0] += per_level[d]; if (d) set_pairs[1] += per_level[d]; }
}

int base_nodes_append(const uint8_t *bxyz, const uint8_t *bocc, int64_t bn, const int64_t t[3], int64_t lim, const char *who, std::vector<BaseNode> *out)
{
    const size_t b0 = out->size();
    for (int64_t i = 0; i < bn; ++i) {
        uint32_t b[3];
        for (int a = 0; a < 3; ++a) {
            const int64_t c = (int32_t)get32(bxyz + 12 * i + 4 * a) + t[a];
            if (c < 0 || c >= lim) return fail(GPCC_ERR_FORMAT, "%sbase coordinate out of range", who);
            b[a] = (uint32_t)c;
        }
        if (!bocc[i]) return fail(GPCC_ERR_FORMAT, "%sempty base occupancy", who);
        out->push_back(BaseNode{morton3(b[0], b[1], b[2]), rkey3(b[0], b[1], b[2]), bocc[i]});
    }
    std::sort(out->begin() + (ptrdiff_t)b0, out->end(), [](const BaseNode &a, const BaseNode &b) { return a.mk < b.mk; });
    for (size_t i = b0 + 1; i < out->size(); ++i) if ((*out)[i].mk == (*out)[i - 1].mk) return fail(GPCC_ERR_FORMAT, "%sduplicate base node", who);
    return GPCC_OK;
}

int alloc_level(gpcc_ctx *ctx, Level *lv, int64_t n, int lvl)
{
    lv->n = n; lv->lvl = lvl;
    TAKE(rkey, uint64_t, n); TAKE(occ, uint8_t, n); TAKE(cstart, uint32_t, n + 1); TAKE(parent, uint32_t, n); TAKE(m2r, uint32_t, n); TAKE(r2m, uint32_t, n);
    lv->rkey = rkey; lv->occ = occ; lv->cstart = cstart; lv->parent = parent; lv->m2r = m2r; lv->r2m = r2m;
    lv->span0 = reinterpret_cast<char *>(rkey); lv->span_bytes = (size_t)(reinterpret_cast<char *>(r2m + n) - reinterpret_cast<char *>(rkey));
    return GPCC_OK;
}

int dec_parent_trunk(gpcc_ctx *ctx, hipStream_t st, const gpcc_model *m, int g, const uint8_t *occ, int64_t np, const ConvTiles &tilesP, const PairPlan &planP, int64_t planP_np,
                     int fmode, float **pA_out, bool *any_fused)
{
    TAKE_TOP(pF, float, np * m->C); TAKE_TOP(pA, float, np * m->C); TAKE_TOP(pB, float, np * m->C);
    float *Pp = nullptr;
    if (planP.valid()) { TAKE_TOP(pp, float, planP.pcap * 32); Pp = pp; }
    if (planP.valid() && fmode == 1) {
        ConvRec rec = {0, 0, g, 1, 0, 0, (long long)np, 0, 5, 1};
        if (ctx->prof.on) GP_TRY(prof_event(ctx, st, &rec.e0));
        GP_TRY(fused_parent_trunk(ctx, st, m, planP, planP_np, occ, pF, pA, pB, Pp));
        if (ctx->prof.on) { GP_TRY(prof_event(ctx, st, &rec.e1)); ctx->prof.recs.push_back(rec); }
        *any_fused = true;
    } else {
        { StageTimer tm(ctx, st, ST_ELEM, (double)np * 129); GP_TRY(embed_occ(st, m->prior_emb, occ, np, pF, m->C)); }
        GP_TRY(dbg_mark(ctx, st, g * 100 + 1, pF, (size_t)np * 128));
        GP_TRY(run_trunk(ctx, g, st, m, 0, Trunk{pF, pA, pB}, tilesP, np, planP.valid() ? &planP : nullptr, Pp));
    }
    GP_TRY(dbg_mark(ctx, st, g * 100 + 2, pA, (size_t)np * 128));
    *pA_out = pA;
    return GPCC_OK;
}

int dec_child_lists(gpcc_ctx *ctx, hipStream_t sd, const gpcc_model *m, const Level *cur, const int32_t *cellP, const Level *chi, int32_t *cellC, bool child_plan,
                    unsigned long long *pairs_dev, PairPlan *planC, ConvTiles *tilesC)
{
    StageTimer tm(ctx, sd, ST_TILES, 0.0);
    if (child_plan) return pairplan_build(ctx, sd, cur, cellP, chi, cellC, m->k, planC, pairs_dev);
    const TileLevel tl = {chi, cur, cellP, cellC};
    const int R = conv_pick_rows(chi->n, m->k);
    const int64_t zero_base[1] = {0};
    TilePool pool;
    GP_TRY(tiles_build(ctx, sd, &tl, 1, m->k, R, conv_pick_height(chi->n, R), &pool, pairs_dev));
    GP_TRY(tiles_view(ctx, sd, pool, 0, 1, zero_base, tilesC));
    tm.add_bytes(pool.alg_bytes);
    return GPCC_OK;
}

int child_bufs_take(gpcc_ctx *ctx, const gpcc_model *m, int64_t nc, int64_t pcap, uint32_t nlanes, int64_t lane_syms, int64_t sym_bytes, ChildBufs *b)
{
    TAKE_TOP(cX, float, nc * m->C); TAKE_TOP(cA, float, nc * m->C); TAKE_TOP(cB, float, nc * m->C); TAKE_TOP(cU, float, nc * m->C);
    b->cX = cX; b->cA = cA; b->cB = cB; b->cU = cU; b->P = nullptr;
    if (pcap) { TAKE_TOP(pc, float, pcap * 32); b->P = pc; }
    TAKE_TOP(cdf, uint16_t, rc_rows_capacity(nlanes, lane_syms) * 16);
    b->cdf = cdf; b->cdf_bytes = (size_t)rc_rows_capacity(nlanes, lane_syms) * 16 * 2;
    for (int s = 0; s < 4; ++s) { TAKE_TOP(sy, uint8_t, sym_bytes); b->sym[s] = sy; }
    return GPCC_OK;
}

int dec_child_fused(gpcc_ctx *ctx, hipStream_t st, const gpcc_model *m, int g, const PairPlan &planC, const float *pA, int64_t np, const Level &chi, const uint8_t *dbytes,
                    const LevelCoder &lc, const ChildBufs &b)
{
    FusedChild fa = {};
    fa.pA = pA; fa.np = np; fa.parent = chi.parent; fa.rkey = chi.rkey; fa.m2r = chi.m2r; fa.bytes = dbytes; fa.chunks = lc.chunks; fa.nlanes = lc.nlanes; fa.llog = lc.llog;
    fa.cpos = lc.cpos; fa.spos = lc.spos;
    for (int s = 0; s < 4; ++s) { fa.win_bytes[s] = lc.win_bytes[s]; fa.sym[s] = b.sym[s]; }
    fa.cX = b.cX; fa.cA = b.cA; fa.cB = b.cB; fa.cU = b.cU; fa.P = b.P; fa.cdf = b.cdf; fa.occ = chi.occ; fa.coder = lc.coder;
    ConvRec rec = {0, 0, g + 1, 1, 0, 0, (long long)chi.n, 0, 13, 1};
    if (ctx->prof.on) GP_TRY(prof_event(ctx, st, &rec.e0));
    GP_TRY(fused_child_level(ctx, st, m, planC, fa));
    if (ctx->prof.on) { GP_TRY(prof_event(ctx, st, &rec.e1)); ctx->prof.recs.push_back(rec); }
    return GPCC_OK;
}

int dec_child_trunk(gpcc_ctx *ctx, hipStream_t st, const gpcc_model *m, int g, const float *pA, const Level &chi, const ConvTiles &tilesC, const PairPlan *planC, const ChildBufs &b)
{
    const int64_t nc = chi.n;
    { StageTimer tm(ctx, st, ST_ELEM, (double)nc * (128 + 12 + 128)); GP_TRY(child_features(st, pA, chi.parent, chi.rkey, m->temb, nc, b.cX, m->C)); }
    GP_TRY(dbg_mark(ctx, st, g * 100 + 8, b.cX, (size_t)nc * 128));
    GP_TRY(run_trunk(ctx, g + 1, st, m, 5, Trunk{b.cX, b.cA, b.cB}, tilesC, nc, planC, b.P));
    GP_TRY(dbg_mark(ctx, st, g * 100 + 9, b.cA, (size_t)nc * 128));
    return GPCC_OK;
}

int dec_child_stage(gpcc_ctx *ctx, hipStream_t st, const gpcc_model *m, int g, int s, const Level &chi, const ConvTiles &tilesC, const PairPlan *planC, const LevelCoder &lc,
                    const ChildBufs &b)
{
    const int64_t nc = chi.n;
    const float *xin = b.cA;
    if (s) {
        StageTimer tm(ctx, st, ST_ELEM, (double)nc * (128 + 4 + s + 128));
        GP_TRY(stage_input_dec(st, b.cA, m->semb[s - 1], b.sym, lc.spos ? lc.spos : chi.m2r, s, nc, b.cU, m->C));
        xin = b.cU;
    }
    if (planC) {
        GP_TRY(plan_conv(st, *planC, ConvJob{xin, m->conv[10 + 2 * s], nullptr, b.cX}, b.P, 1));
        GP_TRY(plan_conv(st, *planC, ConvJob{b.cX, m->conv[10 + 2 * s + 1], nullptr, b.cB}, b.P, 0));
    } else {
        ConvBatch cb = {}; cb.C = m->C;
        GP_TRY(conv_chain_begin(ctx, st));
        cb.job[0] = ConvJob{xin, m->conv[10 + 2 * s], nullptr, b.cX};
        GP_TRY(sparse_conv(ctx, g + 1, st, cb, 1, tilesC, nc, 1));
        cb.job[0] = ConvJob{b.cX, m->conv[10 + 2 * s + 1], nullptr, b.cB};
        GP_TRY(sparse_conv(ctx, g + 1, st, cb, 1, tilesC, nc, 0));
        GP_TRY(conv_chain_end(ctx, st));
    }
    GP_TRY(dbg_mark(ctx, st, g * 100 + 10 + 5 * s, xin, (size_t)nc * 128)); GP_TRY(dbg_mark(ctx, st, g * 100 + 11 + 5 * s, b.cX, (size_t)nc * 128));
    GP_TRY(dbg_mark(ctx, st, g * 100 + 12 + 5 * s, b.cB, (size_t)nc * 128));
    HeadArgs ha = {}; ha.C = m->C;
    ha.x = b.cB; ha.n = nc; ha.stage_m = STAGE_M[s];
    ha.w1 = m->hw1[s]; ha.b1 = m->hb1[s]; ha.w2 = m->hw2[s]; ha.b2 = m->hb2[s]; ha.frag = m->hfrag[s];
    ha.m2r = chi.m2r; ha.cdf = b.cdf; ha.mode = 1; ha.pos = lc.cpos; ha.chunk_log2 = lc.llog; ha.nch = lc.nlanes;
    if (ctx->dbg_on) HIP_TRY(hipMemsetAsync(b.cdf, 0, b.cdf_bytes, st));
    { StageTimer tm(ctx, st, ST_HEADS, (double)nc * (128 + 4 + stage_row_bytes(s))); GP_TRY(head_cdf(st, ha)); }
    GP_TRY(dbg_mark(ctx, st, g * 100 + 13 + 5 * s, b.cdf, b.cdf_bytes));
    return GPCC_OK;
}

}
```

gauspcc_amd/csrc/codec_shared.hpp:

```cpp
#pragma once
#include <functional>
#include <vector>

#include "fused.hpp"
#include "network.hpp"
#include "octree.hpp"
#include "primitives.hpp"

namespace gpcc {

struct Trunk { float *x, *a, *b; };

static inline int run_trunk(gpcc_ctx *ctx, int level, hipStream_t st, const gpcc_model *m, int conv0, const Trunk &t, const ConvTiles &tiles, int64_t n, const PairPlan *plan = nullptr,
              float *P = nullptr)
{
    ConvBatch cb = {}; cb.C = m->C;
    auto one = [&](const float *in, int ci, const float *res, float *out) {
        cb.job[0] = ConvJob{in, m->conv[ci], res, out};
        if (plan) return plan_conv(st, *plan, cb.job[0], P, 1);
        return sparse_conv(ctx, level, st, cb, 1, tiles, n, 1);
    };
    GP_TRY(conv_chain_begin(ctx, st));
    GP_TRY(one(t.x, conv0, nullptr, t.a));
    GP_TRY(one(t.a, conv0 + 1, nullptr, t.b));
    GP_TRY(one(t.b, conv0 + 2, t.a, t.x));
    GP_TRY(one(t.x, conv0 + 3, nullptr, t.b));
    GP_TRY(one(t.b, conv0 + 4, t.x, t.a));
    GP_TRY(conv_chain_end(ctx, st));
    return GPCC_OK;
}

static inline void put32(uint8_t *p, uint32_t v) { p[0] = (uint8_t)v; p[1] = (uint8_t)(v >> 8); p[2] = (uint8_t)(v >> 16); p[3] = (uint8_t)(v >> 24); }
static inline uint32_t get32(const uint8_t *p) { return p[0] | (p[1] << 8) | (p[2] << 16) | ((uint32_t)p[3] << 24); }

static inline size_t arena_estimate(int64_t n, int K) { return (size_t)n * 3 * (size_t)(4 * 125 + 300 + 12 * 128 + 96) + (size_t)n * 64 + (size_t)K * 4096 + ((size_t)64 << 20); }
size_t arena_scaled(size_t want);
void fused_timeout_notice(const gpcc_ctx *ctx);
struct SideGuard { hipStream_t s, x; ~SideGuard() { (void)hipStreamSynchronize(s); if (x) (void)hipStreamSynchronize(x); } };

int tile_sets(gpcc_ctx *ctx, hipStream_t st, const Tree &T, const Level *root, const int32_t *cell_root, int k, unsigned long long *pairs_dev, TilePool *pool, ConvTiles *setP,
              ConvTiles *setC);

struct EncodeNet {
    const Tree *T;
    const Level *root; const int32_t *cell_root;
    unsigned long long *pairs_dev;
    uint32_t *lohi;
    double *bits;
    std::function<int(hipStream_t)> ranks;
    std::function<int(hipStream_t, uint32_t *pos, uint32_t *slots)> set_pos;
    HostTrace *ht; const char *trace;
};
int encode_network(gpcc_ctx *ctx, const gpcc_model *m, hipStream_t st, hipStream_t sd, const EncodeNet &a);

struct LaneList {
    std::vector<RcChunk> chunks;
    uint32_t max_syms = 1;
    size_t table_bound = 0;
};
int lanes_append(LaneList *ll, int si, int64_t first_slot, int64_t nc, const RcPlan &pl);

static inline uint32_t chunk_bytes(const uint32_t *hcnt, int c0, int c1, uint32_t c) { const int l = c0 + 2 * (int)c; return hcnt[l] + (l + 1 < c1 ? hcnt[l + 1] : 0u); }
struct StreamSize { size_t pay = 0, tab = 0; uint32_t max_chunk = 0; bool fits = true; };
StreamSize stream_size(const uint32_t *hcnt, int c0, int c1, int si, bool chunked);
size_t stream_head_put(uint8_t *o, const uint32_t *hcnt, int c0, int c1, const StreamSize &z, bool chunked);
size_t chunked_header_put(uint8_t *o, int version, int chunk_log2, uint16_t posq, int L, const int64_t *level_nodes, int64_t npts);
size_t base_block_put(uint8_t *o, int64_t bn, const int32_t *xyz, const int64_t origin[3], const uint8_t *occ, int nstreams);
void sum_set_pairs(const unsigned long long *per_level, int L, unsigned long long set_pairs[2]);

struct BaseNode { uint64_t mk, rk; uint8_t occ; };
int base_nodes_append(const uint8_t *bxyz, const uint8_t *bocc, int64_t bn, const int64_t t[3], int64_t lim, const char *who, std::vector<BaseNode> *out);

int alloc_level(gpcc_ctx *ctx, Level *lv, int64_t n, int lvl);

int dec_parent_trunk(gpcc_ctx *ctx, hipStream_t st, const gpcc_model *m, int g, const uint8_t *occ, int64_t np, const ConvTiles &tilesP, const PairPlan &planP, int64_t planP_np,
                     int fmode, float **pA, bool *any_fused);
int dec_child_lists(gpcc_ctx *ctx, hipStream_t sd, const gpcc_model *m, const Level *cur, const int32_t *cellP, const Level *chi, int32_t *cellC, bool child_plan,
                    unsigned long long *pairs_dev, PairPlan *planC, ConvTiles *tilesC);

struct LevelCoder {
    const uint32_t *spos, *cpos;
    uint32_t nlanes; int llog;
    const RcChunk *chunks;
    uint32_t win_bytes[4];
    bool dual; int coder;
};
struct ChildBufs { float *cX, *cA, *cB, *cU, *P; uint16_t *cdf; size_t cdf_bytes; uint8_t *sym[4]; };
int child_bufs_take(gpcc_ctx *ctx, const gpcc_model *m, int64_t nc, int64_t pcap, uint32_t nlanes, int64_t lane_syms, int64_t sym_bytes, ChildBufs *b);
int dec_child_fused(gpcc_ctx *ctx, hipStream_t st, const gpcc_model *m, int g, const PairPlan &planC, const float *pA, int64_t np, const Level &chi, const uint8_t *dbytes,
                    const LevelCoder &lc, const ChildBufs &b);
int dec_child_trunk(gpcc_ctx *ctx, hipStream_t st, const gpcc_model *m, int g, const float *pA, const Level &chi, const ConvTiles &tilesC, const PairPlan *planC, const ChildBufs &b);
int dec_child_stage(gpcc_ctx *ctx, hipStream_t st, const gpcc_model *m, int g, int s, const Level &chi, const ConvTiles &tilesC, const PairPlan *planC, const LevelCoder &lc,
                    const ChildBufs &b);
static inline int stage_row_bytes(int s) { return STAGE_M[s] == 2 ? 2 : STAGE_M[s] == 4 ? 8 : 32; }

}
```

gauspcc_amd/csrc/common.hpp:

```cpp
#pragma once
#include <hip/hip_runtime.h>
#include <stdarg.h>
#include <stdint.h>
#include <stdio.h>
#include <stdlib.h>
#include <string.h>

#include <chrono>
#include <string>
#include <mutex>
#include <vector>

#include "../../include/gauspcc.h"

#include "errors.hpp"

namespace gpcc {

#define HIP_TRY(expr)                                                                                  \
    do {                                                                                               \
        hipError_t e_ = (expr);                                                                        \
        if (e_ != hipSuccess)                                                                          \
            return gpcc::fail(GPCC_ERR_HIP, "%s:%d %s -> %s", __FILE__, __LINE__, #expr, hipGetErrorString(e_)); \
    } while (0)

inline bool debug_sync_on() { static const bool on = [] { const char *e = getenv("GAUSPCC_DEBUG_SYNC"); return e && atoi(e) != 0; }(); return on; }
inline hipError_t launch_check(const char *file, int line)
{
    hipError_t e = hipGetLastError();
    ++g_launches;
    if (e == hipSuccess && debug_sync_on()) { fprintf(stderr, "[launch] %s:%d\n", file, line); fflush(stderr); e = hipDeviceSynchronize(); }
    return e;
}
#define LAUNCH_CHECK() HIP_TRY(gpcc::launch_check(__FILE__, __LINE__))

constexpr int CB = 1 << 20;
constexpr int CLIM = CB - 8;
constexpr int NSTAGE = 4;
constexpr int CH = 32;

static inline int64_t cdiv(int64_t a, int64_t b) { return (a + b - 1) / b; }

struct Arena {
    char *base = nullptr;
    size_t cap = 0, off = 0, top = 0;
    int reserve(size_t bytes)
    {
        if (bytes <= cap) return GPCC_OK;
        if (base) HIP_TRY(hipFree(base));
        base = nullptr; cap = 0;
        size_t want = bytes + (bytes >> 3) + (1 << 20);
        HIP_TRY(hipMalloc((void **)&base, want));
        cap = want; top = want & ~size_t(255);
        return GPCC_OK;
    }
    bool flip = false;
    size_t top_low = ~size_t(0);
    void release_top_low() { top_low = ~size_t(0); }
    void reset() { off = 0; top = cap & ~size_t(255); flip = false; top_low = ~size_t(0); }
    template <typename T> T *take(size_t count)
    {
        if (flip) return take_top<T>(count);
        size_t bytes = (count * sizeof(T) + 255) & ~size_t(255);
        if (off + bytes > (top < top_low ? top : top_low)) return nullptr;
        T *p = reinterpret_cast<T *>(base + off);
        off += bytes;
        return p;
    }
    template <typename T> T *take_top(size_t count)
    {
        size_t bytes = (count * sizeof(T) + 255) & ~size_t(255);
        if (off + bytes > top) return nullptr;
        top -= bytes;
        if (flip && top < top_low) top_low = top;
        return reinterpret_cast<T *>(base + top);
    }
    size_t top_mark() const { return top; }
    void top_rewind(size_t m) { top = m; }
    size_t mark() const { return flip ? top : off; }
    void rewind(size_t m) { if (flip) top = m; else off = m; }
};

inline size_t align256(size_t b) { return (b + 255) & ~size_t(255); }
template <class T> int caller_alloc(gsr_alloc_fn alloc, void *user, size_t bytes, T **out, const char *who)
{
    *out = static_cast<T *>(alloc(user, bytes));
    return *out ? GPCC_OK : fail(GPCC_ERR_NOMEM, "%s: workspace (%zu bytes)", who, bytes);
}
struct Carver {
    char *base = nullptr;
    size_t bytes = 0;
    template <class T> T *take(size_t count)
    {
        T *p = base ? reinterpret_cast<T *>(base + bytes) : nullptr;
        bytes += align256(count * sizeof(T));
        return p;
    }
};
template <class Layout> int caller_block(gsr_alloc_fn alloc, void *user, const char *who, Layout &&layout)
{
    Carver c;
    layout(c);
    GP_TRY(caller_alloc(alloc, user, c.bytes, &c.base, who));
    c.bytes = 0;
    layout(c);
    return GPCC_OK;
}

inline int env_int(const char *name, int dflt) { const char *e = getenv(name); return e ? atoi(e) : dflt; }
inline long long env_ll(const char *name, long long dflt) { const char *e = getenv(name); return e ? atoll(e) : dflt; }
inline bool dev_mode() { static const bool on = env_int("GAUSPCC_DEV", 0) != 0; return on; }
inline long long dev_env_ll(const char *name, long long dflt)
{
    const char *e = getenv(name);
    if (!e) return dflt;
    if (dev_mode()) return atoll(e);
    static std::mutex m;
    static bool told = false;
    std::lock_guard<std::mutex> g(m);
    if (!told) { told = true; fprintf(stderr, "[gauspcc] %s is a developer knob and is ignored without GAUSPCC_DEV=1 (as are the other kernel-selection knobs)\n", name); }
    return dflt;
}
inline int dev_env_int(const char *name, int dflt) { return (int)dev_env_ll(name, dflt); }
struct PerDeviceOnce {
    std::mutex m;
    uint64_t done = 0;
    template <typename F> int run(int device, F f)
    {
        std::lock_guard<std::mutex> g(m);
        const uint64_t bit = 1ull << (device & 63);
        if (done & bit) return GPCC_OK;
        const int rc = f();
        if (rc == GPCC_OK) done |= bit;
        return rc;
    }
};

template <typename T> struct HostBuf {
    T *p = nullptr;
    size_t cap = 0;
    int reserve(size_t n)
    {
        if (n <= cap) return GPCC_OK;
        if (p) HIP_TRY(hipHostFree(p));
        p = nullptr; cap = 0;
        size_t want = n + (n >> 2) + 1024;
        HIP_TRY(hipHostMalloc((void **)&p, want * sizeof(T), hipHostMallocDefault));
        cap = want;
        return GPCC_OK;
    }
};

}

namespace gpcc {
struct ConvRec { int e0, e1, level, njobs, R, H; long long n, nblk; int launches; int fused = 0; };
struct Prof {
    bool on = false;
    bool chain_open = false;
    ConvRec chain = {};
    std::vector<hipEvent_t> pool;
    int used = 0;
    std::vector<ConvRec> recs;
    double conv_ms = 0.0;
    int64_t conv_launches = 0, conv_pair_jobs = 0;
    double fused_ms = 0.0;
    int64_t fused_launches = 0, fused_pair_jobs = 0;
    bool stages = false;
    struct StageRec { int id, e0, e1; };
    std::vector<StageRec> srecs;
    double stage_ms[8] = {0}, stage_bytes[8] = {0};
    double stage_crit_ms[8] = {0};
    int64_t stage_n[8] = {0};
};
enum { ST_OCTREE = 0, ST_TILES, ST_ELEM, ST_HEADS, ST_CODER, ST_COUNT };
}

namespace gpcc {
struct HostTrace {
    bool on;
    std::chrono::steady_clock::time_point t0, last;
    HostTrace() : on(getenv("GAUSPCC_HOST_TRACE") && atoi(getenv("GAUSPCC_HOST_TRACE")) > 0) { t0 = last = std::chrono::steady_clock::now(); }
    void mark(const char *what, long long a = -1, long long b = -1)
    {
        if (!on) return;
        const auto t = std::chrono::steady_clock::now();
        fprintf(stderr, "[host] %-22s %8.3f ms  (+%.3f)", what, std::chrono::duration<double, std::milli>(t - t0).count(), std::chrono::duration<double, std::milli>(t - last).count());
        if (a >= 0) fprintf(stderr, "  %lld", a);
        if (b >= 0) fprintf(stderr, " %lld", b);
        fputc('\n', stderr);
        last = t;
    }
};
}

struct gpcc_ctx {
    int device = 0;
    gpcc::Prof prof;
    gpcc::Arena arena;
    gpcc::HostBuf<uint8_t> hbytes;
    gpcc::HostBuf<uint8_t> hstage;
    gpcc::HostBuf<uint8_t> hcoder;
    gpcc::HostBuf<uint8_t> hbatch;
    std::vector<int32_t> stream_cnt;
    hipEvent_t ev0 = nullptr, ev1 = nullptr;
    hipStream_t side = nullptr, xfer = nullptr;
    hipEvent_t ev_main = nullptr, ev_side = nullptr, ev_bytes = nullptr, ev_tables = nullptr;
    float *conv_products = nullptr;
    size_t conv_products_cap = 0;
    struct ScanState { hipStream_t st; unsigned long long *status; uint32_t *ticket; uint32_t epoch; };
    std::vector<ScanState> scan_states;
    uint32_t *dev_err_dev = nullptr;
    uint32_t *dev_err = nullptr;
    int container_version = 4;
    void *fused_state = nullptr;
    int fused_flip = 0;
    bool fused_off = false;
    int fused_off_decodes = 0, fused_rearm_after = 32;
    void fused_note_decode()
    {
        if (!fused_off) return;
        if (++fused_off_decodes >= fused_rearm_after) { fused_off = false; fused_off_decodes = 0; fused_rearm_after = fused_rearm_after < 4096 ? 2 * fused_rearm_after : 4096; }
    }
    hipEvent_t fused_ev = nullptr;
    bool dbg_on = false;
    unsigned long long *dbg_dev = nullptr;
    std::vector<int> dbg_tags;
    struct DbgCap { int tag; void *dev; size_t cap, bytes; };
    std::vector<DbgCap> dbg_caps;
    int dbg_capture_tag_mod = -1;
    int side_init()
    {
        if (side) return GPCC_OK;
        HIP_TRY(hipStreamCreateWithFlags(&side, hipStreamNonBlocking));
        HIP_TRY(hipStreamCreateWithFlags(&xfer, hipStreamNonBlocking));
        HIP_TRY(hipEventCreateWithFlags(&ev_main, hipEventDisableTiming));
        HIP_TRY(hipEventCreateWithFlags(&ev_side, hipEventDisableTiming));
        HIP_TRY(hipEventCreateWithFlags(&ev_bytes, hipEventDisableTiming));
        HIP_TRY(hipEventCreateWithFlags(&ev_tables, hipEventDisableTiming));
        return GPCC_OK;
    }
};

namespace gpcc {
int dbg_mark(gpcc_ctx *ctx, hipStream_t st, int tag, const void *p, size_t bytes);
int prof_event(gpcc_ctx *ctx, hipStream_t st, int *idx);
struct StageTimer {
    gpcc_ctx *c; hipStream_t st; int id, e0 = -1;
    StageTimer(gpcc_ctx *ctx, hipStream_t stream, int stage, double bytes) : c(ctx), st(stream), id(stage)
    {
        if (!c || !c->prof.on || !c->prof.stages) { c = nullptr; return; }
        if (prof_event(c, st, &e0) != GPCC_OK) { c = nullptr; return; }
        c->prof.stage_bytes[id] += bytes;
    }
    void add_bytes(double b) { if (c) c->prof.stage_bytes[id] += b; }
    ~StageTimer()
    {
        int e1;
        if (c && prof_event(c, st, &e1) == GPCC_OK) c->prof.srecs.push_back(Prof::StageRec{id, e0, e1});
    }
};
}

#define TAKE_TOP(var, T, count)                                                                    \
    T *var = ctx->arena.take_top<T>((size_t)(count));                                              \
    if (!var) return gpcc::fail(GPCC_ERR_NOMEM, "%s:%d workspace arena exhausted (%s x %lld)", __FILE__, __LINE__, #T, (long long)(count))

#define TAKE(var, T, count)                                                                        \
    T *var = ctx->arena.take<T>((size_t)(count));                                                  \
    if (!var) return gpcc::fail(GPCC_ERR_NOMEM, "%s:%d workspace arena exhausted (%s x %lld)", __FILE__, __LINE__, #T, (long long)(count))
```

gauspcc_amd/csrc/network.hip:

```cpp
#include <algorithm>
#include <utility>
#include <vector>

#include "network_dev.hpp"
#include "octree.hpp"
#include "primitives.hpp"
#include "rangecoder.hpp"
#ifndef CONV_LOOP_INC
#define CONV_LOOP_INC "conv_loop_gfx950.inc"
#endif
#include CONV_LOOP_INC
#include "conv_loop2_gfx950.inc"
static_assert(CONV_LOOP2_ROW_BYTES == CONV_LDS_ROW_BYTES, "both asm loops address the running sums at one LDS row pitch");

namespace gpcc {

#ifndef CONV_SC_WAVES_N
#define CONV_SC_WAVES_N 4
#endif
constexpr int SC_WAVES = CONV_SC_WAVES_N;
constexpr int HDR_R = 768, HDR_O = 960, HDR_DWORDS = 1008;
constexpr int ROWF = CONV_LDS_ROW_BYTES / 4;
static_assert(ROWF >= 32 && ROWF % 4 == 0, "row pitch: whole 16-byte units");
__host__ __device__ constexpr int conv_lds_wave_floats(int R) { return (R + 1) * ROWF + HDR_DWORDS; }

static int conv_rows_forced()
{
    static const int forced = [] {
        const int f = dev_env_int("GAUSPCC_CONV_R", 0);
        return (f != 0 && f != 16 && f != 32 && f != 64 && f != 96 && f != 128 && f != 255) ? 0 : f;
    }();
    return forced;
}
static int64_t conv_tall_min()
{
    static const int64_t tall_min = 64 * 256 + 1;
    return tall_min;
}

int conv_coop_rows(int64_t n, int k)
{
    static const int tall = dev_env_int("GAUSPCC_COOP_TALL", 1);
    if (!tall || k > 5) return 16;
    return n <= 16 * 256 ? 16 : n <= 32 * 256 ? 32 : 64;
}
bool conv_is_coop(int64_t n, int R)
{
    static const int use_coop = dev_env_int("GAUSPCC_CONV_COOP", 1) != 0;
    if (!use_coop) return false;
    if (R == 16) return true;
    return (R == 32 || R == 64) && !conv_rows_forced() && n < conv_tall_min() && n <= 64 * 256;
}

int conv_pick_rows(int64_t n, int k)
{
    if (conv_rows_forced()) return conv_rows_forced();
    if (n >= conv_tall_min() && n < ((int64_t)1 << 25)) return 255;
    if (n >= 192 * 1024) return 128;
    if (n >= 96 * 1024) return 64;
    if (n >= 24 * 1024) return 32;
    return conv_coop_rows(n, k);
}

int conv_pick_height(int64_t n, int R)
{
    static const int balance = dev_env_int("GAUSPCC_CONV_BALANCE", 2);
    if (!balance || R <= 16 || conv_is_coop(n, R)) return R;
    const int64_t slots = 1024 * (int64_t)(R >= 255 ? 1 : 2);
    const int64_t k = cdiv(n, slots * R);
    if (balance == 2 && (double)(k * slots * R - n) < 0.2 * (double)(k * slots * R)) return R;
    const int64_t H = cdiv(n, slots * k);
    return (int)std::min<int64_t>(R, std::max<int64_t>(H, 16));
}

#ifdef CONV_TIMING
__device__ unsigned long long g_conv_timing[16];
#define CT_STAMP(v) const long long v = clock64()
#else
#define CT_STAMP(v)
#endif

#ifdef CONV_ONE_PER_SIMD
#define CONV_MIN_WAVES(R, ASM) 1
#else
#define CONV_MIN_WAVES(R, ASM) ((ASM) || (R) >= 128 ? 2 : (R) >= 96 ? 3 : 4)
#endif
template <int R, int DIST, bool ASM, int PAIR = 0>
__global__ __launch_bounds__(64 * SC_WAVES, CONV_MIN_WAVES(R, ASM)) void k_sparse_conv(ConvBatch jobs, ConvTiles T, int n, int relu, int njobs)
{
#ifdef CONV_ONE_PER_SIMD
    asm volatile("" ::: "a0", "a1", "a2", "a3", "a4", "a5", "a6", "a7", "a8", "a9", "a10", "a11", "a12", "a13", "a14", "a15", "a16", "a17", "a18", "a19", "a20", "a21", "a22", "a23",
                 "a24", "a25", "a26", "a27", "a28", "a29", "a30", "a31", "a32", "a33", "a34", "a35", "a36", "a37", "a38", "a39", "a40", "a41", "a42", "a43", "a44", "a45", "a46", "a47",
                 "a48", "a49", "a50", "a51", "a52", "a53", "a54", "a55", "a56", "a57", "a58", "a59", "a60", "a61", "a62", "a63", "a64", "a65", "a66", "a67", "a68", "a69", "a70", "a71",
                 "a72", "a73", "a74", "a75", "a76", "a77", "a78", "a79", "a80", "a81", "a82", "a83", "a84", "a85", "a86", "a87", "a88", "a89", "a90", "a91", "a92", "a93", "a94", "a95");
#endif
    constexpr int CONV_LDS_WAVE = conv_lds_wave_floats(R);
    extern __shared__ __attribute__((aligned(16))) float lds[];
    const int lane = threadIdx.x & 63;
    const int wave = __builtin_amdgcn_readfirstlane(threadIdx.x >> 6);
    const uint32_t total = (uint32_t)T.nblk * (uint32_t)njobs;
    const uint32_t w = (uint32_t)(blockIdx.x * SC_WAVES + wave);
    if (w >= total) return;
    {
    CT_STAMP(ct0);
#ifdef CONV_TIMING
    const unsigned long long rt0 = __builtin_amdgcn_s_memrealtime();
#endif
    const uint32_t job = w % (uint32_t)njobs, slot = w / (uint32_t)njobs;
    ConvJob J = jobs.job[0];
    if (job == 1) J = jobs.job[1];
    if (job == 2) J = jobs.job[2];
    if (job == 3) J = jobs.job[3];
    const int blk = __builtin_amdgcn_readfirstlane((int)T.order[slot]);
    int lvi = 0;
    for (int i = 1; i < T.nlv; ++i) lvi = blk >= (int)T.lv_blk0[i] ? i : lvi;
    const int lrow0 = (blk - (int)T.lv_blk0[lvi]) * T.H;
    const int nrows = min(T.H, (int)T.lv_rows[lvi] - lrow0);
    const int row0 = (int)T.lv_row0[lvi] + lrow0;
    J.in += (size_t)T.lv_row0[lvi] * 32;
    float *acc = lds + wave * CONV_LDS_WAVE;
    float4 *acc4 = reinterpret_cast<float4 *>(acc);
    int32_t *hdr = reinterpret_cast<int32_t *>(acc + (R + 1) * ROWF);
    constexpr int RQ = ROWF / 4;
#pragma unroll
    for (int it = 0; it < (R * RQ + 63) / 64; ++it)
        if (it * 64 + lane < R * RQ) acc4[RQ + it * 64 + lane] = make_float4(0.f, 0.f, 0.f, 0.f);
    const int e = lane & 15, g = lane >> 4;
    const int col0 = 4 * (e & 3) + (e >> 2), col1 = col0 + 16;
    const uint32_t t0 = (uint32_t)__builtin_amdgcn_readfirstlane((int)T.first[blk]), t1 = (uint32_t)__builtin_amdgcn_readfirstlane((int)T.first[blk + 1]);
    const float *__restrict__ in = J.in + 4 * g;
    const float *__restrict__ wf = J.w + lane * 4;
    const int32_t *hj = hdr + e;
    const int32_t *hr = hdr + HDR_R + g;
    const int32_t *ho = hdr + HDR_O;
    struct AB { float4 a0, a1, b00, b01, b10, b11; };
    auto load_ab = [&](int j, uint32_t o) -> AB {
        const float *p = in + (size_t)(uint32_t)j * 32;
        const float *w = wf + (size_t)o * 1024;
        AB r;
        r.a0 = ld4(p); r.a1 = ld4(p + 16);
        r.b00 = ld4(w); r.b01 = ld4(w + 256); r.b10 = ld4(w + 512); r.b11 = ld4(w + 768);
        return r;
    };
    struct PT { f32x4 c0, c1; uint32_t r4; };
#define MF(c, a, b) c = __builtin_amdgcn_mfma_f32_16x16x4f32(a, b, c, 0, 0, 0)
    auto step = [&](const AB &v, const PT &p, PT &q) {
        f32x4 c0 = {0.f, 0.f, 0.f, 0.f}, c1 = {0.f, 0.f, 0.f, 0.f};
        float s0[4], s1[4];
        int row[4];
#pragma unroll
        for (int k = 0; k < 4; ++k) {
            row[k] = (int)((p.r4 >> (8 * k)) & 255u) * ROWF;
            s0[k] = acc[row[k] + col0];
            s1[k] = acc[row[k] + col1];
        }
        MF(c0, v.a0.x, v.b00.x); MF(c1, v.a0.x, v.b10.x);
        MF(c0, v.a0.y, v.b00.y); MF(c1, v.a0.y, v.b10.y);
        MF(c0, v.a0.z, v.b00.z); MF(c1, v.a0.z, v.b10.z);
        __builtin_amdgcn_sched_barrier(0);
#pragma unroll
        for (int k = 0; k < 4; ++k) {
            acc[row[k] + col0] = s0[k] + p.c0[k];
            acc[row[k] + col1] = s1[k] + p.c1[k];
        }
        MF(c0, v.a0.w, v.b00.w); MF(c1, v.a0.w, v.b10.w);
        MF(c0, v.a1.x, v.b01.x); MF(c1, v.a1.x, v.b11.x);
        __builtin_amdgcn_sched_barrier(0);
        MF(c0, v.a1.y, v.b01.y); MF(c1, v.a1.y, v.b11.y);
        MF(c0, v.a1.z, v.b01.z); MF(c1, v.a1.z, v.b11.z);
        MF(c0, v.a1.w, v.b01.w); MF(c1, v.a1.w, v.b11.w);
        q.c0 = c0; q.c1 = c1;
    };
#undef MF
    auto accumulate = [&](const PT &p) {
#pragma unroll
        for (int k = 0; k < 4; ++k) {
            const int row = (int)((p.r4 >> (8 * k)) & 255u) * ROWF;
            acc[row + col0] = acc[row + col0] + p.c0[k];
            acc[row + col1] = acc[row + col1] + p.c1[k];
        }
    };
    if (t0 < t1) {
        constexpr int RING = DIST + 1;
        constexpr uint32_t DUMMY4 = 0u;
        const uint32_t nt = t1 - t0;
        const int4 *__restrict__ gtj = reinterpret_cast<const int4 *>(T.tj + (size_t)t0 * 16) + lane;
        const uint32_t *__restrict__ gtr = reinterpret_cast<const uint32_t *>(T.tr + (size_t)t0 * 16) + lane;
        const uint32_t *__restrict__ gto = T.toc + t0 + (lane & 15);
        int4 *sj = reinterpret_cast<int4 *>(hdr) + lane;
        int32_t *sr = hdr + HDR_R + lane;
        int32_t *so = hdr + HDR_O + (lane & 15);
        {
            const int4 a0 = gtj[0], a1 = gtj[64];
            const uint32_t b0 = gtr[0], b1 = gtr[64], c0 = gto[0], c1 = gto[16];
            sj[0] = a0; sj[64] = a1;
            sr[0] = (int32_t)b0; sr[64] = (int32_t)b1;
            so[0] = (int32_t)(c0 & 0xFFFFu); so[16] = (int32_t)(c1 & 0xFFFFu);
            sj[128] = a0;
            sr[128] = (int32_t)b0;
            so[32] = (int32_t)(c0 & 0xFFFFu);
        }
        CT_STAMP(ct1);
        if constexpr (ASM) {
            uint32_t su, st0, st1;
            const uint32_t acc_lds = __builtin_amdgcn_groupstaticsize() + (uint32_t)(wave * CONV_LDS_WAVE * 4);
            const uint32_t hdr_lds = acc_lds + (uint32_t)((R + 1) * ROWF * 4);
#ifdef CONV_LOOP_STAMPS
            uint32_t sw0, sw1, sw2, sw3;
            asm volatile(CONV_LOOP_ASM
                         : [u] "=&s"(su), [t0] "=&s"(st0), [t1] "=&s"(st1), [w0] "=&s"(sw0), [w1] "=&s"(sw1), [w2] "=&s"(sw2), [w3] "=&s"(sw3)
                         : [in] "s"(J.in), [w] "s"(J.w + (size_t)T.K * 1024), [tj] "s"(T.tj + (size_t)t0 * 16), [tr] "s"(T.tr + (size_t)t0 * 16), [toc] "s"(T.toc + t0),
                           [nt] "s"(nt), [acc] "s"(acc_lds), [hdr] "s"(hdr_lds), [lane] "v"(lane)
                         : CONV_LOOP_CLOBBERS);
            if (lane == 0) {
                atomicAdd(&g_conv_timing[12], (unsigned long long)sw0); atomicAdd(&g_conv_timing[13], (unsigned long long)sw1);
                atomicAdd(&g_conv_timing[14], (unsigned long long)sw2); atomicAdd(&g_conv_timing[15], (unsigned long long)sw3);
            }
#else
            if (PAIR == 1 && __builtin_amdgcn_readfirstlane((int)T.pflag[blk]))
                asm volatile(CONV_LOOP2_ASM
                             : [u] "=&s"(su), [t0] "=&s"(st0), [t1] "=&s"(st1)
                             : [in] "s"(J.in), [w] "s"(J.w + (size_t)T.K * 1024), [tj] "s"(T.tj + (size_t)t0 * 16), [tr] "s"(T.tr + (size_t)t0 * 16), [toc] "s"(T.toc + t0),
                               [nt] "s"(nt), [acc] "s"(acc_lds), [hdr] "s"(hdr_lds), [lane] "v"(lane)
                             : CONV_LOOP2_CLOBBERS);
            else
                asm volatile(CONV_LOOP_ASM
                             : [u] "=&s"(su), [t0] "=&s"(st0), [t1] "=&s"(st1)
                             : [in] "s"(J.in), [w] "s"(J.w + (size_t)T.K * 1024), [tj] "s"(T.tj + (size_t)t0 * 16), [tr] "s"(T.tr + (size_t)t0 * 16), [toc] "s"(T.toc + t0),
                               [nt] "s"(nt), [acc] "s"(acc_lds), [hdr] "s"(hdr_lds), [lane] "v"(lane)
                             : CONV_LOOP_CLOBBERS);
#endif
        } else {
        int4 st_j = make_int4(0, 0, 0, 0);
        uint32_t st_r = 0, st_o = 0;
        AB ring[RING];
        uint32_t r4r[RING];
#pragma unroll
        for (int s = 0; s < DIST; ++s) {
            const uint32_t r4_ld = (uint32_t)hr[s * 4];
            r4r[s] = (uint32_t)s < nt ? r4_ld : DUMMY4;
            ring[s] = load_ab(hj[s * 16], (uint32_t)ho[s] & 0xFFFFu);
        }
        int j_n = hj[DIST * 16];
        const uint32_t r4_ld0 = (uint32_t)hr[DIST * 4];
        uint32_t r4_n = (uint32_t)DIST < nt ? r4_ld0 : DUMMY4, o_n = (uint32_t)ho[DIST] & 0xFFFFu;
        PT prev;
        prev.c0 = f32x4{0.f, 0.f, 0.f, 0.f}; prev.c1 = prev.c0; prev.r4 = DUMMY4;
        for (uint32_t u = 0; u < nt; u += RING) {
#pragma unroll
            for (int s = 0; s < RING; ++s) {
                const uint32_t us = u + (uint32_t)s;
                if ((us & 15u) == 0u && us != 0u) {
                    const uint32_t bo = (us >> 4) + 1u;
                    st_j = gtj[bo * 64]; st_r = gtr[bo * 64]; st_o = gto[bo * 16];
                }
                if ((us & 15u) == 8u && us > 8u) {
                    const uint32_t bb = ((us >> 4) + 1u) & 1u;
                    sj[bb * 64] = st_j; sr[bb * 64] = (int32_t)st_r; so[bb * 16] = (int32_t)(st_o & 0xFFFFu);
                }
                const int sl = (s + DIST) % RING;
                const uint32_t tq = us + (uint32_t)(DIST + 1);
                const uint32_t slot = tq & 31u;
                const int j_nn = hj[slot * 16];
                const uint32_t r4_ld = (uint32_t)hr[slot * 4], o_nn = (uint32_t)ho[slot] & 0xFFFFu;
                __builtin_amdgcn_sched_barrier(0);
                const uint32_t r4_cur = r4r[s];
                r4r[sl] = r4_n;
                ring[sl] = load_ab(j_n, o_n);
                __builtin_amdgcn_sched_barrier(0);
                PT cur;
                step(ring[s], prev, cur);
                cur.r4 = r4_cur;
                prev = cur;
                const uint32_t r4_nn = tq < nt ? r4_ld : DUMMY4;
                __builtin_amdgcn_sched_barrier(0);
                j_n = j_nn; r4_n = r4_nn; o_n = o_nn;
            }
        }
        accumulate(prev);
        }
#ifdef CONV_TIMING
        const long long ct2 = clock64();
        if (lane == 0) { atomicAdd(&g_conv_timing[0], (unsigned long long)(ct1 - ct0)); atomicAdd(&g_conv_timing[1], (unsigned long long)(ct2 - ct1)); atomicAdd(&g_conv_timing[3], (unsigned long long)nt); }
#endif
    }
    CT_STAMP(ct3);
#ifdef CONV_TIMING
    __builtin_amdgcn_s_waitcnt(0);
    const long long ct3a = clock64();
#endif
#ifdef CONV_NO_EPILOGUE
    if (lane == 0 && nrows > 0) J.out[(size_t)row0 * 32] = acc[ROWF];
    if (false)
#endif
    {
        const int nvec = nrows * 8;
        const bool has_res = J.res != nullptr;
        const float4 *__restrict__ res4 = reinterpret_cast<const float4 *>(J.res) + (size_t)row0 * 8;
        float4 *__restrict__ out4 = reinterpret_cast<float4 *>(J.out) + (size_t)row0 * 8;
        const float4 *src = acc4 + RQ + (lane >> 3) * RQ + (lane & 7);
        constexpr int NG = (R * 8 + 63) / 64;
        constexpr int NB = (NG + 7) / 8;
        float4 r[NG];
        if (has_res) {
#pragma unroll
            for (int g8 = 0; g8 < NG; ++g8) r[g8] = res4[min(g8 * 64 + lane, nvec - 1)];
        }
#ifdef CONV_TIMING
        long long te[NB + 1];
        te[0] = clock64();
#endif
#pragma unroll
        for (int bt = 0; bt < NB; ++bt) {
            if (bt * 512 < nvec) {
                float4 v[8];
#pragma unroll
                for (int b = 0; b < 8; ++b)
                    if (bt * 8 + b < NG) v[b] = src[(bt * 8 + b) * 8 * RQ];
                if (has_res) {
#pragma unroll
                    for (int b = 0; b < 8; ++b)
                        if (bt * 8 + b < NG) { const float4 q = r[bt * 8 + b]; v[b].x = v[b].x + q.x; v[b].y = v[b].y + q.y; v[b].z = v[b].z + q.z; v[b].w = v[b].w + q.w; }
                }
                if (relu) {
#pragma unroll
                    for (int b = 0; b < 8; ++b)
                        if (bt * 8 + b < NG) { v[b].x = v[b].x > 0.f ? v[b].x : 0.f; v[b].y = v[b].y > 0.f ? v[b].y : 0.f; v[b].z = v[b].z > 0.f ? v[b].z : 0.f; v[b].w = v[b].w > 0.f ? v[b].w : 0.f; }
                }
#pragma unroll
                for (int b = 0; b < 8; ++b)
                    if (bt * 8 + b < NG && (bt * 8 + b) * 64 + lane < nvec) out4[(bt * 8 + b) * 64 + lane] = v[b];
            }
#ifdef CONV_TIMING
            te[bt + 1] = clock64();
#endif
        }
#ifdef CONV_TIMING
#ifndef CONV_LOOP_STAMPS
        if (lane == 0 && NB == 4) {
            atomicAdd(&g_conv_timing[12], (unsigned long long)(te[1] - te[0])); atomicAdd(&g_conv_timing[13], (unsigned long long)(te[2] - te[1]));
            atomicAdd(&g_conv_timing[14], (unsigned long long)(te[3] - te[2])); atomicAdd(&g_conv_timing[15], (unsigned long long)(te[4] - te[3]));
        }
#endif
#endif
    }
#ifdef CONV_TIMING
    const long long ct3b = clock64();
    __builtin_amdgcn_s_waitcnt(0);
    const long long ct4 = clock64();
    if (lane == 0) { atomicAdd(&g_conv_timing[10], (unsigned long long)(ct3a - ct3)); atomicAdd(&g_conv_timing[11], (unsigned long long)(ct3b - ct3a)); }
    const unsigned long long rt1 = __builtin_amdgcn_s_memrealtime();
    if (lane == 0) {
        atomicAdd(&g_conv_timing[2], (unsigned long long)(ct4 - ct3)); atomicAdd(&g_conv_timing[4], 1ull); atomicAdd(&g_conv_timing[5], (unsigned long long)(ct4 - ct0));
        atomicAdd(&g_conv_timing[6], rt1 - rt0); atomicMin(&g_conv_timing[7], rt0); atomicMax(&g_conv_timing[8], rt1); atomicMax(&g_conv_timing[9], rt1 - rt0);
    }
#endif
    }
}



constexpr int COOP_TILES = 32;
#ifndef COOP_WAVES_N
#define COOP_WAVES_N 16
#endif
constexpr int COOP_WAVES = COOP_WAVES_N;
constexpr int COOP_TPW = COOP_TILES / COOP_WAVES;
static inline size_t coop_lds_bytes(int K, int rows) { return (size_t)COOP_TILES * 16 * 32 * 4 + (size_t)rows * COOP_TILES + (size_t)K * (rows / 16) * 84; }

template <int ROWS>
__global__ __launch_bounds__(64 * COOP_WAVES) void k_sparse_conv_coop(ConvBatch jobs, ConvTiles T, int n, int relu)
{
    extern __shared__ __attribute__((aligned(16))) float lds[];
    const int NTMAX = T.K * (ROWS / 16);
    float *P = lds;
    uint8_t *inv = reinterpret_cast<uint8_t *>(lds + COOP_TILES * 16 * 32);
    int32_t *hj = reinterpret_cast<int32_t *>(inv + ROWS * COOP_TILES);
    uint32_t *hr = reinterpret_cast<uint32_t *>(hj + (size_t)NTMAX * 16);
    uint32_t *ho = hr + (size_t)NTMAX * 4;
#ifdef COOP_TIMING
    const long long q0 = clock64();
#endif
    const ConvJob J = jobs.job[blockIdx.y];
    const int tid = threadIdx.x, lane = tid & 63;
    const int wave = __builtin_amdgcn_readfirstlane(tid >> 6);
    const int blk = (int)T.lv_blk0[0] + (int)blockIdx.x;
    int lvi = 0;
    for (int i = 1; i < T.nlv; ++i) lvi = blk >= (int)T.lv_blk0[i] ? i : lvi;
    const int lrow0 = (blk - (int)T.lv_blk0[lvi]) * ROWS;
    const int nrows = min(ROWS, (int)T.lv_rows[lvi] - lrow0);
    const int row0 = (int)T.lv_row0[lvi] + lrow0;
    const int e = lane & 15, g = lane >> 4;
    const int col0 = 4 * (e & 3) + (e >> 2), col1 = col0 + 16;
    const uint32_t t0 = (uint32_t)__builtin_amdgcn_readfirstlane((int)T.first[blk]), t1 = (uint32_t)__builtin_amdgcn_readfirstlane((int)T.first[blk + 1]);
    const int nt = (int)min(t1 - t0, (uint32_t)NTMAX);
    for (int i = tid; i < nt * 16; i += 64 * COOP_WAVES) hj[i] = T.tj[(size_t)t0 * 16 + i];
    for (int i = tid; i < nt * 4; i += 64 * COOP_WAVES) hr[i] = reinterpret_cast<const uint32_t *>(T.tr + (size_t)t0 * 16)[i];
    for (int i = tid; i < nt; i += 64 * COOP_WAVES) ho[i] = T.toc[t0 + i];
    __syncthreads();
#ifdef COOP_TIMING
    const long long q1 = clock64();
#endif
    const float *__restrict__ in = J.in + (size_t)T.lv_row0[lvi] * 32 + 4 * g;
    const float *__restrict__ wf = J.w + lane * 4;
    constexpr int NEL = ROWS * 32;
    constexpr int COOP_EPT = NEL / (64 * COOP_WAVES) > 0 ? NEL / (64 * COOP_WAVES) : 1;
    float acc[COOP_EPT];
#pragma unroll
    for (int u = 0; u < COOP_EPT; ++u) acc[u] = 0.0f;
    struct AB { float4 a0, a1, b00, b01, b10, b11; };
    const uint32_t nlv_rows = max(T.lv_rows[lvi], 1u);
    auto fetch = [&](int t) -> AB {
        const float *p = in + (size_t)min((uint32_t)hj[t * 16 + e], nlv_rows - 1u) * 32;
        const float *w = wf + (size_t)min(ho[t] & 0xFFFFu, (uint32_t)T.K - 1u) * 1024;
        AB r;
        r.a0 = ld4(p); r.a1 = ld4(p + 16);
        r.b00 = ld4(w); r.b01 = ld4(w + 256); r.b10 = ld4(w + 512); r.b11 = ld4(w + 768);
        return r;
    };
    auto products = [&](const AB &v, int t, int tl) {
        const f32x4 z = {0.f, 0.f, 0.f, 0.f};
        f32x4 c0 = z, c1 = z;
#define MF(c, a, b) c = __builtin_amdgcn_mfma_f32_16x16x4f32(a, b, c, 0, 0, 0)
        MF(c0, v.a0.x, v.b00.x); MF(c1, v.a0.x, v.b10.x);
        MF(c0, v.a0.y, v.b00.y); MF(c1, v.a0.y, v.b10.y);
        MF(c0, v.a0.z, v.b00.z); MF(c1, v.a0.z, v.b10.z);
        MF(c0, v.a0.w, v.b00.w); MF(c1, v.a0.w, v.b10.w);
        MF(c0, v.a1.x, v.b01.x); MF(c1, v.a1.x, v.b11.x);
        MF(c0, v.a1.y, v.b01.y); MF(c1, v.a1.y, v.b11.y);
        MF(c0, v.a1.z, v.b01.z); MF(c1, v.a1.z, v.b11.z);
        MF(c0, v.a1.w, v.b01.w); MF(c1, v.a1.w, v.b11.w);
#undef MF
        float *dst = P + (size_t)tl * 512;
#pragma unroll
        for (int k = 0; k < 4; ++k) {
            dst[(4 * g + k) * 32 + col0] = c0[k];
            dst[(4 * g + k) * 32 + col1] = c1[k];
        }
        if (lane < ROWS) inv[lane * COOP_TILES + tl] = 255;
        const uint32_t cnt = ho[t] >> 16;
        const uint32_t r = (hr[t * 4 + (e >> 2)] >> (8 * (e & 3))) & 255u;
        if (lane < 16 && (uint32_t)lane < cnt && r >= 1u && r <= (uint32_t)ROWS) inv[(r - 1u) * COOP_TILES + tl] = (uint8_t)lane;
    };
    AB cur[COOP_TPW], nxt[COOP_TPW];
#pragma unroll
    for (int q = 0; q < COOP_TPW; ++q)
        if (wave * COOP_TPW + q < nt) cur[q] = fetch(wave * COOP_TPW + q);
    for (int base = 0; base < nt; base += COOP_TILES) {
#pragma unroll
        for (int q = 0; q < COOP_TPW; ++q) {
            const int t = base + COOP_TILES + wave * COOP_TPW + q;
            if (t < nt) nxt[q] = fetch(t);
        }
#pragma unroll
        for (int q = 0; q < COOP_TPW; ++q) {
            const int t = base + wave * COOP_TPW + q;
            if (t < nt) products(cur[q], t, wave * COOP_TPW + q);
        }
        __syncthreads();
#pragma unroll
        for (int u = 0; u < COOP_EPT; ++u) {
            const int el = tid + u * 64 * COOP_WAVES;
            if (el < NEL) {
                const int orow = el >> 5, och = el & 31;
                const int ntl = min(COOP_TILES, nt - base);
                const uint4 w0 = *reinterpret_cast<const uint4 *>(inv + orow * COOP_TILES), w1 = *reinterpret_cast<const uint4 *>(inv + orow * COOP_TILES + 16);
                const uint32_t wd[8] = {w0.x, w0.y, w0.z, w0.w, w1.x, w1.y, w1.z, w1.w};
                float pv[COOP_TILES];
#pragma unroll
                for (int tl = 0; tl < COOP_TILES; ++tl) {
                    const uint32_t i = (wd[tl >> 2] >> (8 * (tl & 3))) & 255u;
                    const float pvv = P[(size_t)tl * 512 + (i & 15u) * 32 + och];
                    pv[tl] = (tl < ntl && i != 255u) ? pvv : 0.0f;
                }
#pragma unroll
                for (int tl = 0; tl < COOP_TILES; ++tl) acc[u] = acc[u] + pv[tl];
            }
        }
        __syncthreads();
#pragma unroll
        for (int q = 0; q < COOP_TPW; ++q) cur[q] = nxt[q];
    }
#ifdef COOP_TIMING
    const long long q2 = clock64();
#endif
#pragma unroll
    for (int u = 0; u < COOP_EPT; ++u) {
        const int el = tid + u * 64 * COOP_WAVES;
        const int grow = row0 + (el >> 5), och = el & 31;
        if (el < NEL && (el >> 5) < nrows) {
            float v = acc[u];
            if (J.res) v = v + J.res[(size_t)grow * 32 + och];
            if (relu) v = v > 0.f ? v : 0.f;
            J.out[(size_t)grow * 32 + och] = v;
        }
    }
#ifdef COOP_TIMING
    if (tid == 0 && blockIdx.x == 0 && blockIdx.y == 0) printf("[coop] blocks %u nt %d: headers %lld rounds %lld epilogue %lld cycles\n", gridDim.x, nt, q1 - q0, q2 - q1, clock64() - q2);
#endif
}

constexpr int PROD_WAVES = 4;
__global__ __launch_bounds__(64 * PROD_WAVES) void k_conv_products(ConvJob J, ConvTiles T, float *__restrict__ P)
{
    const int lane = threadIdx.x & 63;
    const int wave = __builtin_amdgcn_readfirstlane(threadIdx.x >> 6);
    const int blk = (int)T.lv_blk0[0] + (int)blockIdx.x;
    int lvi = 0;
    for (int i = 1; i < T.nlv; ++i) lvi = blk >= (int)T.lv_blk0[i] ? i : lvi;
    const uint32_t t0 = (uint32_t)__builtin_amdgcn_readfirstlane((int)T.first[blk]), t1 = (uint32_t)__builtin_amdgcn_readfirstlane((int)T.first[blk + 1]);
    const int e = lane & 15, g = lane >> 4;
    const float *__restrict__ in = J.in + (size_t)T.lv_row0[lvi] * 32 + 4 * g;
    const float *__restrict__ wt = J.w + (size_t)T.K * 1024 + lane * 4;
    const uint32_t nlv_rows = max(T.lv_rows[lvi], 1u);
    P -= (size_t)T.first[T.lv_blk0[0]] * 512;
    const uint32_t tend = t0 + min(t1 - t0, (uint32_t)T.K);
    for (uint32_t t = t0 + blockIdx.y * PROD_WAVES + (uint32_t)wave; t < tend; t += gridDim.y * PROD_WAVES) {
        const uint32_t oc = T.toc[t];
        const uint32_t cnt = oc >> 16;
        const float *p = in + (size_t)min((uint32_t)T.tj[(size_t)t * 16 + e], nlv_rows - 1u) * 32;
        const float *w = wt + (size_t)min(oc & 0xFFFFu, (uint32_t)T.K - 1u) * 1024;
        const float4 x0 = ld4(p), x1 = ld4(p + 16);
        const float4 w0 = ld4(w), w1 = ld4(w + 256), w2 = ld4(w + 512), w3 = ld4(w + 768);
        f32x4 c0 = {0.f, 0.f, 0.f, 0.f}, c1 = {0.f, 0.f, 0.f, 0.f};
#define MF(c, a, b) c = __builtin_amdgcn_mfma_f32_16x16x4f32(a, b, c, 0, 0, 0)
        MF(c0, w0.x, x0.x); MF(c1, w2.x, x0.x);
        MF(c0, w0.y, x0.y); MF(c1, w2.y, x0.y);
        MF(c0, w0.z, x0.z); MF(c1, w2.z, x0.z);
        MF(c0, w0.w, x0.w); MF(c1, w2.w, x0.w);
        MF(c0, w1.x, x1.x); MF(c1, w3.x, x1.x);
        MF(c0, w1.y, x1.y); MF(c1, w3.y, x1.y);
        MF(c0, w1.z, x1.z); MF(c1, w3.z, x1.z);
        MF(c0, w1.w, x1.w); MF(c1, w3.w, x1.w);
#undef MF
        if ((uint32_t)e < cnt) {
            float *dst = P + ((size_t)t * 16 + e) * 32 + 4 * g;
            *reinterpret_cast<float4 *>(dst) = make_float4(c0[0], c0[1], c0[2], c0[3]);
            *reinterpret_cast<float4 *>(dst + 16) = make_float4(c1[0], c1[1], c1[2], c1[3]);
        }
    }
}

__global__ void k_check_tiles(ConvTiles T, int64_t n, unsigned long long total_cap, int *bad, int koff)
{
    const int blk = (int)T.lv_blk0[0] + (int)blockIdx.x;
    const uint32_t t0 = T.first[blk], t1 = T.first[blk + 1];
    if (threadIdx.x == 0 && (t1 < t0 || t1 - t0 > (uint32_t)T.K || t1 > total_cap)) { if (atomicAdd(bad, 1) < 8) printf("[check] block %d: tiles %u .. %u (at most %d, cap %llu)\n", blk, t0, t1, T.K, total_cap); }
    const uint32_t tend = t0 + min(t1 - t0, (uint32_t)T.K);
    for (uint32_t t = t0 + threadIdx.x / 16; t < tend && t < total_cap; t += blockDim.x / 16) {
        const int e = threadIdx.x & 15;
        const int32_t j = T.tj[(size_t)t * 16 + e];
        const uint32_t oc = T.toc[t];
        const uint32_t r = T.tr[(size_t)t * 16 + e];
        if (j < 0 || j >= n || (oc & 0xFFFFu) >= (uint32_t)koff || (oc >> 16) > 16u || r > (uint32_t)T.H) { if (atomicAdd(bad, 1) < 8) printf("[check] block %d tile %u entry %d: j %d (n %lld) toc %08x slot %u\n", blk, t, e, j, (long long)n, oc, r); }
    }
}

constexpr int SUM_BATCH = 32;
__global__ __launch_bounds__(512) void k_conv_sum(ConvJob J, ConvTiles T, const float *__restrict__ P, int relu)
{
    extern __shared__ __attribute__((aligned(16))) uint8_t inv[];
    const int tid = threadIdx.x;
    const int blk = (int)T.lv_blk0[0] + (int)blockIdx.x;
    int lvi = 0;
    for (int i = 1; i < T.nlv; ++i) lvi = blk >= (int)T.lv_blk0[i] ? i : lvi;
    const int lrow0 = (blk - (int)T.lv_blk0[lvi]) * 16;
    const int nrows = min(16, (int)T.lv_rows[lvi] - lrow0);
    const int row0 = (int)T.lv_row0[lvi] + lrow0;
    const uint32_t t0 = T.first[blk], t1 = T.first[blk + 1];
    const int nt = (int)min(t1 - t0, (uint32_t)T.K);
    const int ntp = (T.K + SUM_BATCH - 1) / SUM_BATCH * SUM_BATCH;
    for (int i = tid; i < 16 * ntp; i += 512) inv[i] = 255;
    __syncthreads();
    for (int i = tid; i < nt * 16; i += 512) {
        const int t = i >> 4, en = i & 15;
        const uint32_t cnt = T.toc[t0 + t] >> 16;
        const uint32_t r = T.tr[(size_t)(t0 + t) * 16 + en];
        if ((uint32_t)en < cnt && r >= 1u && r <= 16u) inv[(r - 1u) * ntp + t] = (uint8_t)en;
    }
    __syncthreads();
    const int r = tid >> 5, ch = tid & 31;
    const float *__restrict__ Pb = P + (size_t)(t0 - T.first[T.lv_blk0[0]]) * 512 + ch;
    const uint8_t *iv = inv + r * ntp;
    float acc = 0.0f;
    for (int tb = 0; tb < nt; tb += SUM_BATCH) {
        float pv[SUM_BATCH];
#pragma unroll
        for (int u = 0; u < SUM_BATCH; ++u) {
            const int t = tb + u;
            const uint32_t en = iv[t];
            const float v = Pb[(size_t)(t < nt ? t : 0) * 512 + (en & 15u) * 32];
            pv[u] = (t < nt && en != 255u) ? v : 0.0f;
        }
#pragma unroll
        for (int u = 0; u < SUM_BATCH; ++u) acc = acc + pv[u];
    }
    if (r < nrows) {
        const size_t at = (size_t)(row0 + r) * 32 + ch;
        float v = acc;
        if (J.res) v = v + J.res[at];
        if (relu) v = v > 0.f ? v : 0.f;
        J.out[at] = v;
    }
}

int prof_event(gpcc_ctx *ctx, hipStream_t st, int *idx)
{
    Prof &p = ctx->prof;
    if (p.used == (int)p.pool.size()) {
        hipEvent_t e;
        HIP_TRY(hipEventCreate(&e));
        p.pool.push_back(e);
    }
    *idx = p.used++;
    HIP_TRY(hipEventRecord(p.pool[(size_t)*idx], st));
    return GPCC_OK;
}

int sparse_conv(gpcc_ctx *ctx, int level, hipStream_t st, const ConvBatch &jobs, int njobs, const ConvTiles &T, int64_t n, int relu)
{
    if (n <= 0) return GPCC_OK;
    if (n >= (int64_t)1 << 31) return fail(GPCC_ERR_ARG, "level too large");
    if (jobs.C != 0 && jobs.C != 32) return any_sparse_conv(st, jobs, njobs, T, n, relu, jobs.C);
    const bool chained = ctx && ctx->prof.on && ctx->prof.chain_open;
    const bool prof = ctx && ctx->prof.on && !chained;
    ConvRec rec = {0, 0, level, njobs, T.R, T.H, (long long)n, (long long)T.nblk, 1};
    if (chained) { ConvRec &c = ctx->prof.chain; c.level = level; c.njobs = njobs; c.R = T.R; c.H = T.H; c.n = (long long)n; c.nblk = (long long)T.nblk; c.launches += 1; }
    if (prof) GP_TRY(prof_event(ctx, st, &rec.e0));
    static const int use_asm = dev_env_int("GAUSPCC_CONV_ASM", 1) != 0;
    static PerDeviceOnce lds_attr;
    int cur_dev = 0;
    HIP_TRY(hipGetDevice(&cur_dev));
    GP_TRY(lds_attr.run(cur_dev, [&]() -> int {
        const int bytes = SC_WAVES * conv_lds_wave_floats(128) * 4;
        HIP_TRY(hipFuncSetAttribute(reinterpret_cast<const void *>(k_sparse_conv<128, 1, true>), hipFuncAttributeMaxDynamicSharedMemorySize, bytes));
        HIP_TRY(hipFuncSetAttribute(reinterpret_cast<const void *>(k_sparse_conv<255, 1, true>), hipFuncAttributeMaxDynamicSharedMemorySize, SC_WAVES * conv_lds_wave_floats(255) * 4));
        HIP_TRY(hipFuncSetAttribute(reinterpret_cast<const void *>(k_sparse_conv<255, 1, true, 1>), hipFuncAttributeMaxDynamicSharedMemorySize, SC_WAVES * conv_lds_wave_floats(255) * 4));
        HIP_TRY(hipFuncSetAttribute(reinterpret_cast<const void *>(k_sparse_conv<255, 1, false>), hipFuncAttributeMaxDynamicSharedMemorySize, SC_WAVES * conv_lds_wave_floats(255) * 4));
        HIP_TRY(hipFuncSetAttribute(reinterpret_cast<const void *>(k_sparse_conv<128, 1, false>), hipFuncAttributeMaxDynamicSharedMemorySize, bytes));
        HIP_TRY(hipFuncSetAttribute(reinterpret_cast<const void *>(k_sparse_conv_coop<16>), hipFuncAttributeMaxDynamicSharedMemorySize, (int)coop_lds_bytes(343, 16)));
        HIP_TRY(hipFuncSetAttribute(reinterpret_cast<const void *>(k_sparse_conv_coop<32>), hipFuncAttributeMaxDynamicSharedMemorySize, (int)coop_lds_bytes(125, 32)));
        HIP_TRY(hipFuncSetAttribute(reinterpret_cast<const void *>(k_sparse_conv_coop<64>), hipFuncAttributeMaxDynamicSharedMemorySize, (int)coop_lds_bytes(125, 64)));
        return GPCC_OK;
    }));
    static const int use_split = dev_env_int("GAUSPCC_CONV_SPLIT", 1) != 0;
    const bool use_coop = conv_is_coop(n, T.R) && T.H == T.R;
    static const int split_max = 64;
    const size_t prod_floats = ((size_t)T.nblk * (size_t)T.K + CONV_HDR_PAD) * 512;
    if (T.R == 16 && use_coop && use_split && ctx && T.K <= 343 && T.nblk <= split_max && prod_floats * 4 <= ((size_t)768 << 20)) {
        if (ctx->conv_products_cap < prod_floats) {
            HIP_TRY(hipStreamSynchronize(st));
            if (ctx->conv_products) HIP_TRY(hipFree(ctx->conv_products));
            ctx->conv_products = nullptr; ctx->conv_products_cap = 0;
            const size_t want = std::max(prod_floats, (size_t)16 << 20);
            HIP_TRY(hipMalloc(reinterpret_cast<void **>(&ctx->conv_products), want * 4));
            ctx->conv_products_cap = want;
        }
        const unsigned split = (unsigned)std::max<int64_t>(1, std::min<int64_t>({(int64_t)32, (int64_t)cdiv(T.K, PROD_WAVES), (int64_t)cdiv(2048, T.nblk)}));
        const int ntp = (T.K + SUM_BATCH - 1) / SUM_BATCH * SUM_BATCH;
        static const bool dbg = getenv("GAUSPCC_DEBUG_LAUNCH") != nullptr;
        for (int j = 0; j < njobs; ++j) {
            if (dbg) {
                int *bad = nullptr, hb = 0;
                HIP_TRY(hipMalloc(reinterpret_cast<void **>(&bad), 4));
                HIP_TRY(hipMemsetAsync(bad, 0, 4, st));
                k_check_tiles<<<(unsigned)T.nblk, 256, 0, st>>>(T, n, (unsigned long long)((size_t)T.nblk * T.K + CONV_HDR_PAD), bad, T.K);
                HIP_TRY(hipMemcpyAsync(&hb, bad, 4, hipMemcpyDeviceToHost, st));
                HIP_TRY(hipStreamSynchronize(st));
                (void)hipFree(bad);
                fprintf(stderr, "[dbg] tile check: %d bad\n", hb);
            }
            if (dbg) { fprintf(stderr, "[dbg] products level %d n %lld nblk %lld split %u K %d cap %zu need %zu\n", level, (long long)n, (long long)T.nblk, split, T.K, ctx->conv_products_cap, prod_floats); fflush(stderr); }
            k_conv_products<<<dim3((unsigned)T.nblk, split), 64 * PROD_WAVES, 0, st>>>(jobs.job[j], T, ctx->conv_products);
            LAUNCH_CHECK();
            if (dbg) { HIP_TRY(hipStreamSynchronize(st)); fprintf(stderr, "[dbg] sum\n"); fflush(stderr); }
            k_conv_sum<<<(unsigned)T.nblk, 512, (size_t)16 * ntp, st>>>(jobs.job[j], T, ctx->conv_products, relu);
            LAUNCH_CHECK();
            if (dbg) { HIP_TRY(hipStreamSynchronize(st)); fprintf(stderr, "[dbg] done\n"); fflush(stderr); }
        }
        if (prof) { GP_TRY(prof_event(ctx, st, &rec.e1)); ctx->prof.recs.push_back(rec); }
        return GPCC_OK;
    }
    if (use_coop) {
        if (T.K > 343 || (T.R > 16 && T.K > 125)) return fail(GPCC_ERR_ARG, "kernel size > 7 is not supported");
        const dim3 cg((unsigned)T.nblk, (unsigned)njobs);
        const size_t cl = coop_lds_bytes(T.K, T.R);
        if (T.R == 16) k_sparse_conv_coop<16><<<cg, 64 * COOP_WAVES, cl, st>>>(jobs, T, (int)n, relu);
        else if (T.R == 32) k_sparse_conv_coop<32><<<cg, 64 * COOP_WAVES, cl, st>>>(jobs, T, (int)n, relu);
        else k_sparse_conv_coop<64><<<cg, 64 * COOP_WAVES, cl, st>>>(jobs, T, (int)n, relu);
        LAUNCH_CHECK();
        if (prof) { GP_TRY(prof_event(ctx, st, &rec.e1)); ctx->prof.recs.push_back(rec); }
        return GPCC_OK;
    }
    if (debug_sync_on()) {
        int *bad = nullptr, hb = 0;
        HIP_TRY(hipMalloc(reinterpret_cast<void **>(&bad), 4));
        HIP_TRY(hipMemsetAsync(bad, 0, 4, st));
        ConvTiles Tc = T; Tc.K = T.K * ((T.H + 15) / 16);
        k_check_tiles<<<(unsigned)T.nblk, 256, 0, st>>>(Tc, n, ~0ull, bad, T.K);
        HIP_TRY(hipMemcpyAsync(&hb, bad, 4, hipMemcpyDeviceToHost, st));
        HIP_TRY(hipStreamSynchronize(st));
        (void)hipFree(bad);
        fflush(stdout);
        fprintf(stderr, "[conv] level %d n %lld R %d H %d blocks %lld paired %d: tile check %d bad\n", level, (long long)n, T.R, T.H, (long long)T.nblk, T.paired, hb); fflush(stderr);
        if (hb) return fail(GPCC_ERR_FORMAT, "developer check: %d tile entries out of bounds at level %d", hb, level);
    }
    dim3 grid((unsigned)cdiv(T.nblk * njobs, SC_WAVES), 1u);
    const size_t lds_bytes = (size_t)SC_WAVES * conv_lds_wave_floats(T.R) * 4;
    const bool asm_ok = use_asm && n < ((int64_t)1 << 25);
#define CONV_LAUNCH(RR, DD, AA) k_sparse_conv<RR, DD, AA><<<grid, 64 * SC_WAVES, lds_bytes, st>>>(jobs, T, (int)n, relu, njobs)
    switch (T.R) {
    case 16: if (asm_ok) CONV_LAUNCH(16, 1, true); else CONV_LAUNCH(16, 1, false); break;
    case 32: if (asm_ok) CONV_LAUNCH(32, 1, true); else CONV_LAUNCH(32, 1, false); break;
    case 64: if (asm_ok) CONV_LAUNCH(64, 1, true); else CONV_LAUNCH(64, 1, false); break;
    case 96: if (asm_ok) CONV_LAUNCH(96, 1, true); else CONV_LAUNCH(96, 1, false); break;
    case 255:
        if (asm_ok && T.paired) k_sparse_conv<255, 1, true, 1><<<grid, 64 * SC_WAVES, lds_bytes, st>>>(jobs, T, (int)n, relu, njobs);
        else if (asm_ok) CONV_LAUNCH(255, 1, true);
        else CONV_LAUNCH(255, 1, false);
        break;
    default:
        if (asm_ok) CONV_LAUNCH(128, 1, true);
        else CONV_LAUNCH(128, 1, false);
        break;
    }
#undef CONV_LAUNCH
    LAUNCH_CHECK();
    if (prof) { GP_TRY(prof_event(ctx, st, &rec.e1)); ctx->prof.recs.push_back(rec); }
#ifdef CONV_TIMING
    if (prof) {
        unsigned long long h[16], z[16] = {0};
        z[7] = ~0ull;
        HIP_TRY(hipStreamSynchronize(st));
        float ms = 0.f;
        HIP_TRY(hipEventElapsedTime(&ms, ctx->prof.pool[(size_t)rec.e0], ctx->prof.pool[(size_t)rec.e1]));
        HIP_TRY(hipMemcpyFromSymbol(h, HIP_SYMBOL(g_conv_timing), sizeof h));
        HIP_TRY(hipMemcpyToSymbol(HIP_SYMBOL(g_conv_timing), z, sizeof z));
        const double waves = (double)h[4], tiles = (double)h[3];
        fprintf(stderr, "[conv] R %3d H %3d jobs %d n %8lld blocks %6.0f tiles %9.0f  %.1f us | per wave: setup %.0f loop %.0f epilogue %.0f total %.0f cyc | loop %.0f cyc/tile | clock %.0f MHz | span %.1f us, wave time / 1024 slots %.1f us, longest block %.1f us\n",
                T.R, T.H, njobs, (long long)n, waves, tiles, ms * 1e3, h[0] / waves, h[1] / waves, h[2] / waves, h[5] / waves, h[1] / tiles, 100.0 * h[5] / (double)h[6],
                (h[8] - h[7]) / 100.0, h[6] / 100.0 / 1024.0, h[9] / 100.0);
        fprintf(stderr, "[conv]    epilogue: loop drain %.0f, copy-out issue %.0f, store drain %.0f cycles; residual %d relu %d\n", h[10] / waves, h[11] / waves,
                (h[2] - h[10] - h[11]) / waves, jobs.job[0].res != nullptr, relu);
        if (h[12] + h[13] + h[14] + h[15])
#ifdef CONV_LOOP_STAMPS
            fprintf(stderr, "[conv]    per tile: step-start wait %.0f, first pair + VALU burst + LDS issue %.0f, second pair + loads issue %.0f, remaining 12 MFMAs %.0f cycles\n",
                    h[12] / tiles, h[13] / tiles, h[14] / tiles, h[15] / tiles);
#else
            fprintf(stderr, "[conv]    copy-out batches of 64 rows: %.0f %.0f %.0f %.0f cycles\n", h[12] / waves, h[13] / waves, h[14] / waves, h[15] / waves);
#endif
    }
#endif
    return GPCC_OK;
}

int conv_chain_begin(gpcc_ctx *ctx, hipStream_t st)
{
    if (!ctx || !ctx->prof.on) return GPCC_OK;
#ifdef CONV_TIMING
    return GPCC_OK;
#endif
    ctx->prof.chain = ConvRec{};
    GP_TRY(prof_event(ctx, st, &ctx->prof.chain.e0));
    ctx->prof.chain_open = true;
    return GPCC_OK;
}

int conv_chain_end(gpcc_ctx *ctx, hipStream_t st)
{
    if (!ctx || !ctx->prof.on || !ctx->prof.chain_open) return GPCC_OK;
    ctx->prof.chain_open = false;
    GP_TRY(prof_event(ctx, st, &ctx->prof.chain.e1));
    if (ctx->prof.chain.launches > 0) ctx->prof.recs.push_back(ctx->prof.chain);
    return GPCC_OK;
}

int prof_collect(gpcc_ctx *ctx, const unsigned long long *pairs, int nlevels)
{
    Prof &p = ctx->prof;
    p.chain_open = false;
    static const int log = env_int("GAUSPCC_CONV_LOG", 0);
    for (const ConvRec &r : p.recs) {
        float ms = 0.f;
        HIP_TRY(hipEventElapsedTime(&ms, p.pool[(size_t)r.e0], p.pool[(size_t)r.e1]));
        if (log)
            for (int q = 0; q < r.launches; ++q)
                fprintf(stderr, "[conv] level %2d n %8lld R %3d H %3d blocks %6lld jobs %d  %8.1f us pairs %llu\n", r.level, r.n, r.R, r.H, r.nblk, r.njobs, ms * 1e3 / r.launches,
                        (r.level >= 0 && r.level < nlevels) ? pairs[r.level] : 0ull);
        if (r.fused) {
            p.fused_ms += ms;
            p.fused_launches += r.launches;
            if (r.level >= 0 && r.level < nlevels) p.fused_pair_jobs += (int64_t)pairs[r.level] * r.njobs * r.launches;
            continue;
        }
        p.conv_ms += ms;
        p.conv_launches += r.launches;
        if (r.level >= 0 && r.level < nlevels) p.conv_pair_jobs += (int64_t)pairs[r.level] * r.njobs * r.launches;
    }
    std::vector<std::pair<float, float>> busy;
    if (!p.srecs.empty() && p.used > 0) {
        for (const ConvRec &r : p.recs) {
            float a = 0.f, b = 0.f;
            if (hipEventElapsedTime(&a, p.pool[0], p.pool[(size_t)r.e0]) != hipSuccess || hipEventElapsedTime(&b, p.pool[0], p.pool[(size_t)r.e1]) != hipSuccess) { busy.clear(); break; }
            busy.emplace_back(a, b);
        }
        std::sort(busy.begin(), busy.end());
        size_t w = 0;
        for (size_t i = 0; i < busy.size(); ++i) {
            if (w && busy[i].first <= busy[w - 1].second) busy[w - 1].second = std::max(busy[w - 1].second, busy[i].second);
            else busy[w++] = busy[i];
        }
        busy.resize(w);
    }
    p.recs.clear();
    for (const Prof::StageRec &r : p.srecs) {
        float ms = 0.f;
        HIP_TRY(hipEventElapsedTime(&ms, p.pool[(size_t)r.e0], p.pool[(size_t)r.e1]));
        p.stage_ms[r.id] += ms;
        p.stage_n[r.id] += 1;
        float a = 0.f, b = 0.f, cov = 0.f;
        if (p.used > 0 && hipEventElapsedTime(&a, p.pool[0], p.pool[(size_t)r.e0]) == hipSuccess && hipEventElapsedTime(&b, p.pool[0], p.pool[(size_t)r.e1]) == hipSuccess) {
            for (const auto &iv : busy) cov += std::max(0.f, std::min(b, iv.second) - std::max(a, iv.first));
            p.stage_crit_ms[r.id] += std::max(0.f, (b - a) - cov);
        } else p.stage_crit_ms[r.id] += ms;
    }
    p.srecs.clear();
    p.used = 0;
    return GPCC_OK;
}

constexpr int TB = 256;
static inline unsigned nblk(int64_t n) { return (unsigned)cdiv(n, TB); }

__global__ __launch_bounds__(TB) void k_embed_occ(const float4 *__restrict__ emb, const uint8_t *__restrict__ occ, int64_t n, float4 *__restrict__ out)
{
    int64_t t = (int64_t)blockIdx.x * TB + threadIdx.x;
    int64_t i = t >> 3;
    if (i >= n) return;
    out[t] = emb[(size_t)occ[i] * 8 + (t & 7)];
}
int embed_occ(hipStream_t st, const float *emb, const uint8_t *occ, int64_t n, float *out, int C)
{
    if (C != 32) return any_embed_occ(st, emb, occ, n, out, C);
    k_embed_occ<<<nblk(n * 8), TB, 0, st>>>((const float4 *)emb, occ, n, (float4 *)out);
    LAUNCH_CHECK();
    return GPCC_OK;
}

__device__ __forceinline__ float4 add4(float4 a, float4 b) { return make_float4(a.x + b.x, a.y + b.y, a.z + b.z, a.w + b.w); }

__global__ __launch_bounds__(TB) void k_child_features(const float4 *__restrict__ F, const uint32_t *__restrict__ parent, const uint64_t *__restrict__ rkey_c,
                                                       const float4 *__restrict__ temb, int64_t n, float4 *__restrict__ out)
{
    int64_t t = (int64_t)blockIdx.x * TB + threadIdx.x;
    int64_t i = t >> 3;
    if (i >= n) return;
    const int g = (int)(t & 7);
    const uint64_t k = rkey_c[i];
    const int q = (int)((rk_x(k) & 1) | ((rk_y(k) & 1) << 1) | ((rk_z(k) & 1) << 2));
    out[t] = add4(F[(size_t)parent[i] * 8 + g], temb[q * 8 + g]);
}
int child_features(hipStream_t st, const float *F, const uint32_t *parent, const uint64_t *rkey_c, const float *temb, int64_t n, float *out, int C)
{
    if (C != 32) return any_child_features(st, F, parent, rkey_c, temb, n, out, C);
    k_child_features<<<nblk(n * 8), TB, 0, st>>>((const float4 *)F, parent, rkey_c, (const float4 *)temb, n, (float4 *)out);
    LAUNCH_CHECK();
    return GPCC_OK;
}

__global__ __launch_bounds__(TB) void k_stage_inputs_gt(const float4 *__restrict__ X, const float4 *__restrict__ e1, const float4 *__restrict__ e2, const float4 *__restrict__ e3,
                                                        const uint8_t *__restrict__ occ, int64_t n, float4 *__restrict__ o1, float4 *__restrict__ o2, float4 *__restrict__ o3)
{
    int64_t t = (int64_t)blockIdx.x * TB + threadIdx.x;
    int64_t i = t >> 3;
    if (i >= n) return;
    const uint32_t o = occ[i];
    const float4 x = X[t];
    const int c = (int)(t & 7);
    o1[t] = add4(x, e1[((o >> 7) & 1u) * 8 + c]);
    o2[t] = add4(x, e2[((o >> 6) & 3u) * 8 + c]);
    o3[t] = add4(x, e3[((o >> 4) & 15u) * 8 + c]);
}
int stage_inputs_gt(hipStream_t st, const float *X, const float *const emb[3], const uint8_t *occ, int64_t n, float *const out[3], int C)
{
    if (C != 32) return any_stage_inputs_gt(st, X, emb, occ, n, out, C);
    k_stage_inputs_gt<<<nblk(n * 8), TB, 0, st>>>((const float4 *)X, (const float4 *)emb[0], (const float4 *)emb[1], (const float4 *)emb[2], occ, n,
                                                  (float4 *)out[0], (float4 *)out[1], (float4 *)out[2]);
    LAUNCH_CHECK();
    return GPCC_OK;
}

struct SymPtrs { const uint8_t *s[4]; };

__global__ __launch_bounds__(TB) void k_stage_input_dec(const float4 *__restrict__ X, const float4 *__restrict__ emb, SymPtrs sp, const uint32_t *__restrict__ m2r,
                                                        int stage, int64_t n, float4 *__restrict__ out)
{
    int64_t t = (int64_t)blockIdx.x * TB + threadIdx.x;
    int64_t i = t >> 3;
    if (i >= n) return;
    const uint32_t r = m2r[i];
    uint32_t prev = sp.s[0][r];
    if (stage >= 2) prev = prev * 2 + sp.s[1][r];
    if (stage >= 3) prev = prev * 4 + sp.s[2][r];
    out[t] = add4(X[t], emb[prev * 8 + (t & 7)]);
}
int stage_input_dec(hipStream_t st, const float *X, const float *emb, const uint8_t *const sym_r[3], const uint32_t *m2r, int stage, int64_t n, float *out, int C)
{
    if (C != 32) return any_stage_input_dec(st, X, emb, sym_r, m2r, stage, n, out, C);
    SymPtrs sp = {{sym_r[0], sym_r[1], sym_r[2], nullptr}};
    k_stage_input_dec<<<nblk(n * 8), TB, 0, st>>>((const float4 *)X, (const float4 *)emb, sp, m2r, stage, n, (float4 *)out);
    LAUNCH_CHECK();
    return GPCC_OK;
}

__global__ __launch_bounds__(TB) void k_assemble_occ(SymPtrs sp, const uint32_t *__restrict__ m2r, int64_t n, uint8_t *__restrict__ occ)
{
    int64_t i = (int64_t)blockIdx.x * TB + threadIdx.x;
    if (i >= n) return;
    const uint32_t r = m2r[i];
    occ[i] = (uint8_t)(sp.s[0][r] * 128 + sp.s[1][r] * 64 + sp.s[2][r] * 16 + sp.s[3][r]);
}
int assemble_occ(hipStream_t st, const uint8_t *const sym_r[4], const uint32_t *m2r, int64_t n, uint8_t *occ)
{
    SymPtrs sp = {{sym_r[0], sym_r[1], sym_r[2], sym_r[3]}};
    k_assemble_occ<<<nblk(n), TB, 0, st>>>(sp, m2r, n, occ);
    LAUNCH_CHECK();
    return GPCC_OK;
}

__global__ __launch_bounds__(TB) void k_rows_permute(const float *__restrict__ in, float *__restrict__ out, int64_t n, int to_physical)
{
    int64_t t = (int64_t)blockIdx.x * TB + threadIdx.x;
    if (t >= n * 32) return;
    const int64_t i = t >> 5;
    const int c = (int)(t & 31);
    if (to_physical) out[i * 32 + phys_of(c)] = in[t];
    else out[t] = in[i * 32 + phys_of(c)];
}
int rows_permute(hipStream_t st, const float *in, float *out, int64_t n, int to_physical)
{
    k_rows_permute<<<nblk(n * 32), TB, 0, st>>>(in, out, n, to_physical);
    LAUNCH_CHECK();
    return GPCC_OK;
}

template <int M, int MODE>
__global__ __launch_bounds__(TB) void k_head(HeadArgs a)
{
    const int64_t i = (int64_t)blockIdx.x * TB + threadIdx.x;
    if (i >= a.n) return;
    float x[32];
    {
        const float4 *__restrict__ px = reinterpret_cast<const float4 *>(a.x + (size_t)i * 32);
        float raw[32];
#pragma unroll
        for (int g = 0; g < 8; ++g) {
            float4 v = px[g];
            raw[4 * g] = v.x; raw[4 * g + 1] = v.y; raw[4 * g + 2] = v.z; raw[4 * g + 3] = v.w;
        }
#pragma unroll
        for (int c = 0; c < 32; ++c) x[c] = MODE == 2 ? raw[c] : raw[phys_of(c)];
    }
    const float *__restrict__ W1 = a.w1;
    const float *__restrict__ B1 = a.b1;
    const float *__restrict__ W2 = a.w2;
    const float *__restrict__ B2 = a.b2;
    float hdn[32];
#pragma unroll
    for (int c = 0; c < 32; ++c) {
        float acc = B1[c];
#pragma unroll
        for (int k = 0; k < 32; ++k) acc = __builtin_fmaf(x[k], W1[c * 32 + k], acc);
        hdn[c] = acc > 0.0f ? acc : 0.0f;
    }
    float z[M];
    float mx = -__builtin_inff();
#pragma unroll
    for (int j = 0; j < M; ++j) {
        float acc = B2[j];
#pragma unroll
        for (int k = 0; k < 32; ++k) acc = __builtin_fmaf(hdn[k], W2[j * 32 + k], acc);
        z[j] = acc;
        mx = acc > mx ? acc : mx;
    }
    head_tail<M, MODE>(a, i, z, mx, blockIdx.x);
}

template <int M, int MODE>
__global__ __launch_bounds__(TB) void k_head_mfma(HeadArgs a)
{
    __shared__ __attribute__((aligned(16))) float sm[(TB / 64) * HEAD_LDS_FLOATS];
    const int lane = threadIdx.x & 63, wave = threadIdx.x >> 6;
    head_wave<M, MODE>(a, ((int64_t)blockIdx.x * (TB / 64) + wave) * 64, a.n, lane, sm + wave * HEAD_LDS_FLOATS, blockIdx.x);
}

template <int MODE>
static int head_launch(hipStream_t st, const HeadArgs &a)
{
    if (MODE != 2 && a.frag) {
        const unsigned g = (unsigned)cdiv(a.n, TB);
        switch (a.stage_m) {
        case 2: k_head_mfma<2, MODE><<<g, TB, 0, st>>>(a); break;
        case 4: k_head_mfma<4, MODE><<<g, TB, 0, st>>>(a); break;
        case 16: k_head_mfma<16, MODE><<<g, TB, 0, st>>>(a); break;
        default: return fail(GPCC_ERR_ARG, "head width must be 2, 4 or 16");
        }
        LAUNCH_CHECK();
        return GPCC_OK;
    }
    const unsigned g = nblk(a.n);
    switch (a.stage_m) {
    case 2: k_head<2, MODE><<<g, TB, 0, st>>>(a); break;
    case 4: k_head<4, MODE><<<g, TB, 0, st>>>(a); break;
    case 16: k_head<16, MODE><<<g, TB, 0, st>>>(a); break;
    default: return fail(GPCC_ERR_ARG, "head width must be 2, 4 or 16");
    }
    LAUNCH_CHECK();
    return GPCC_OK;
}

int head_cdf(hipStream_t st, const HeadArgs &a)
{
    if (a.n <= 0) return GPCC_OK;
    if (a.C != 0 && a.C != 32) return any_head_cdf(st, a, a.C);
    if (a.mode == 0) return head_launch<0>(st, a);
    if (a.mode == 1) return head_launch<1>(st, a);
    return head_launch<2>(st, a);
}

}
```

gauspcc_amd/csrc/network.hpp:

```cpp
#pragma once
#include "common.hpp"

struct gpcc_model {
    int C = 32, k = 5, K = 125;
    float *slab = nullptr;
    const float *prior_emb = nullptr;
    const float *conv[18] = {0};
    const float *temb = nullptr;
    const float *hw1[4] = {0}, *hb1[4] = {0}, *hw2[4] = {0}, *hb2[4] = {0};
    const float *hfrag[4] = {0};
    const float *semb[3] = {0};
};

namespace gpcc {

__host__ __device__ __forceinline__ int phys_of(int c)
{
    const int kk = c >> 2, g = c & 3;
    return kk < 4 ? 4 * g + kk : 16 + 4 * g + (kk - 4);
}
__host__ __device__ __forceinline__ int logical_of(int p)
{
    const int kk = 4 * (p >> 4) + (p & 3), g = (p & 15) >> 2;
    return 4 * kk + g;
}

inline void conv_weight_fragments(const float *W, int K, float *out)
{
    for (int o = 0; o < K; ++o)
        for (int hh = 0; hh < 2; ++hh)
            for (int q = 0; q < 2; ++q)
                for (int lane = 0; lane < 64; ++lane)
                    for (int r = 0; r < 4; ++r)
                        out[((((size_t)o * 2 + hh) * 2 + q) * 64 + lane) * 4 + r] = W[((size_t)o * 32 + (4 * (4 * q + r) + (lane >> 4))) * 32 + 16 * hh + (lane & 15)];
}

inline void conv_weight_fragments_t(const float *W, int K, float *out)
{
    for (int o = 0; o < K; ++o)
        for (int hh = 0; hh < 2; ++hh)
            for (int q = 0; q < 2; ++q)
                for (int lane = 0; lane < 64; ++lane)
                    for (int r = 0; r < 4; ++r) {
                        const int m = lane & 15;
                        out[((((size_t)o * 2 + hh) * 2 + q) * 64 + lane) * 4 + r] = W[((size_t)o * 32 + (4 * (4 * q + r) + (lane >> 4))) * 32 + 16 * hh + 4 * (m & 3) + (m >> 2)];
                    }
}

constexpr int STAGE_M[4] = {2, 2, 4, 16};

struct ConvJob {
    const float *in;
    const float *w;
    const float *res;
    float *out;
};
struct ConvBatch { ConvJob job[4]; int C = 0; };

constexpr int CONV_R_MAX = 255;
constexpr int CONV_HDR_PAD = 48;
struct ConvTiles {
    int32_t *tj = nullptr;
    uint8_t *tr = nullptr;
    uint32_t *toc = nullptr;
    uint32_t *first = nullptr;
    uint32_t *order = nullptr;
    int64_t nblk = 0;
    int R = CONV_R_MAX;
    int H = CONV_R_MAX;
    int K = 0;
    int paired = 0;
    const uint8_t *pflag = nullptr;
    int nlv = 0;
    uint32_t lv_blk0[MAXLV + 1] = {0};
    uint32_t lv_row0[MAXLV] = {0};
    uint32_t lv_rows[MAXLV] = {0};
};
int conv_pick_rows(int64_t n, int k = 5);
bool conv_is_coop(int64_t n, int R);
int conv_pick_height(int64_t n, int R);

struct Level;
struct TileLevel { const Level *lv; const Level *par; const int32_t *cell_par; int32_t *cell_own; };
struct TilePool {
    int32_t *tj = nullptr; uint8_t *tr = nullptr; uint32_t *toc = nullptr; uint32_t *first = nullptr;
    int64_t nblk = 0;
    int R = 0, H = 0, K = 0, nlv = 0, paired = 0;
    uint8_t *pflag = nullptr;
    uint32_t lv_blk0[MAXLV + 1] = {0}, lv_rows[MAXLV] = {0};
    double alg_bytes = 0.0;
};
int cell_map_entries(int k);
int tiles_build(gpcc_ctx *ctx, hipStream_t st, const TileLevel *lv, int nlv, int k, int R, int H, TilePool *pool, unsigned long long *pairs_dev);
int tiles_dense_map(hipStream_t st, const Level *par, const int32_t *cell_par, const Level *chi, int32_t *cell_own, int k, int32_t *nbr, uint16_t *rk, uint32_t *rowcnt);
int tiles_view(gpcc_ctx *ctx, hipStream_t st, const TilePool &pool, int l0, int l1, const int64_t *row_base, ConvTiles *T);

int sparse_conv(gpcc_ctx *ctx, int level, hipStream_t st, const ConvBatch &jobs, int njobs, const ConvTiles &T, int64_t n, int relu);
int conv_chain_begin(gpcc_ctx *ctx, hipStream_t st);
int conv_chain_end(gpcc_ctx *ctx, hipStream_t st);
int prof_collect(gpcc_ctx *ctx, const unsigned long long *pairs_per_level, int nlevels);

int embed_occ(hipStream_t st, const float *emb, const uint8_t *occ, int64_t n, float *out, int C = 32);
int child_features(hipStream_t st, const float *F, const uint32_t *parent, const uint64_t *rkey_c, const float *temb, int64_t n, float *out, int C = 32);
int stage_inputs_gt(hipStream_t st, const float *X, const float *const emb[3], const uint8_t *occ, int64_t n, float *const out[3], int C = 32);
int stage_input_dec(hipStream_t st, const float *X, const float *emb, const uint8_t *const sym_r[3], const uint32_t *m2r, int stage, int64_t n, float *out, int C = 32);

constexpr int HEAD_FRAG_FLOATS = 1024 + 512 + 32 + 16;
struct HeadArgs {
    const float *x; int64_t n; int stage_m;
    const float *w1, *b1, *w2, *b2;
    const float *frag;
    const uint32_t *m2r; const uint8_t *occ; int stage;
    uint32_t *lohi; uint16_t *cdf; float *prob; int mode;
    int chunk_log2; uint32_t nch;
    const uint32_t *pos; const uint32_t *slots;
    double *bits;
    int C;
};
int head_cdf(hipStream_t st, const HeadArgs &a);

int assemble_occ(hipStream_t st, const uint8_t *const sym_r[4], const uint32_t *m2r, int64_t n, uint8_t *occ);

int any_embed_occ(hipStream_t st, const float *emb, const uint8_t *occ, int64_t n, float *out, int C);
int any_child_features(hipStream_t st, const float *F, const uint32_t *parent, const uint64_t *rkey_c, const float *temb, int64_t n, float *out, int C);
int any_stage_inputs_gt(hipStream_t st, const float *X, const float *const emb[3], const uint8_t *occ, int64_t n, float *const out[3], int C);
int any_stage_input_dec(hipStream_t st, const float *X, const float *emb, const uint8_t *const sym_r[3], const uint32_t *m2r, int stage, int64_t n, float *out, int C);
int any_sparse_conv(hipStream_t st, const ConvBatch &jobs, int njobs, const ConvTiles &T, int64_t n, int relu, int C);
int any_head_cdf(hipStream_t st, const HeadArgs &a, int C);

int rows_permute(hipStream_t st, const float *in, float *out, int64_t n, int to_physical);

}
```

Baseline: 21.12.

## Fuse stage-input fan-out into last trunk conv and embed into occupancy assembly

The last sparse convolution of the child trunk can now write the three stage inputs directly, adding occupancy-selected stage embeddings from a table staged in the tile-header LDS ring. This removes a separate stage_inputs_gt pass that re-read the conv output. In decode, occupancy assembly also writes the prior embedding for the next level into the arena slot that dec_parent_trunk will claim, so the separate embed_occ launch is skipped. This adds kernel template variants and extra stores inside the conv epilogue, and depends on the arena placing the next level's buffer at a predictable address.

```diff
diff --git a/gauspcc_amd/csrc/codec.hip b/gauspcc_amd/csrc/codec.hip
--- a/gauspcc_amd/csrc/codec.hip
+++ b/gauspcc_amd/csrc/codec.hip
@@ -396,11 +396,13 @@
     int64_t planP_np = 0;
     bool any_fused = false;
     HIP_TRY(hipEventRecord(ctx->ev_main, st));
+    const float *pF_ready = nullptr;
     for (int g = 0; g + 1 < L; ++g) {
         const size_t top_mk = ctx->arena.top_mark();
         const int64_t np = cur.n;
         float *pA = nullptr;
-        GP_TRY(dec_parent_trunk(ctx, st, m, g, cur.occ, np, tilesP, planP, planP_np, fmode, &pA, &any_fused));
+        GP_TRY(dec_parent_trunk(ctx, st, m, g, cur.occ, np, tilesP, planP, planP_np, fmode, &pA, &any_fused, pF_ready));
+        pF_ready = nullptr;
         HIP_TRY(hipStreamWaitEvent(sd, ctx->ev_main, 0));
         Level chi;
         int64_t nc = lvl_n[g + 1];
@@ -483,7 +485,7 @@
             }
             GP_TRY(dbg_mark(ctx, st, g * 100 + 14 + 5 * s, sym[s], (size_t)nc));
         }
-        { StageTimer tm(ctx, st, ST_ELEM, (double)nc * (4 + 4 + 1)); GP_TRY(assemble_occ(st, sym, chi.m2r, nc, chi.occ)); }
+        GP_TRY(dec_level_occ(ctx, st, m, sym, chi.m2r, nc, chi.occ, g + 2 < L && !child_plan, top_mk, &pF_ready));
         }
         GP_TRY(dbg_mark(ctx, st, g * 100 + 30, chi.occ, (size_t)nc));
         HIP_TRY(hipEventRecord(ctx->ev_main, st));
diff --git a/gauspcc_amd/csrc/codec_batch.hip b/gauspcc_amd/csrc/codec_batch.hip
--- a/gauspcc_amd/csrc/codec_batch.hip
+++ b/gauspcc_amd/csrc/codec_batch.hip
@@ -499,13 +499,15 @@
     BDecTail tail = {};
     HIP_TRY(hipEventRecord(ctx->ev_main, st));
     GP_TRY(parse_levels(1, d_early, ctx->ev_bytes));
+    const float *pF_ready = nullptr;
     for (int g = 0; g + 1 < L; ++g) {
         const size_t top_mk = ctx->arena.top_mark();
         Level &cur = T.lv[g];
         const int64_t np = cur.n;
         const int64_t np_in = F.inner(g);
         float *pA = nullptr;
-        GP_TRY(dec_parent_trunk(ctx, st, m, g, cur.occ, np, tilesP, planP, planP_np, fmode, &pA, &any_fused));
+        GP_TRY(dec_parent_trunk(ctx, st, m, g, cur.occ, np, tilesP, planP, planP_np, fmode, &pA, &any_fused, pF_ready));
+        pF_ready = nullptr;
         HIP_TRY(hipStreamWaitEvent(sd, ctx->ev_main, 0));
         Level &chi = T.lv[g + 1];
         const int64_t nc = lvl_n[g + 1];
@@ -547,7 +549,7 @@
                 StageTimer tm(ctx, st, ST_CODER, (double)nc * (stage_row_bytes(s) + 1));
                 GP_TRY(rc_decode_launch(st, cb.cdf, STAGE_M[s] + 1, dbytes, dchunks + (size_t)s * nch, nch, lc.win_bytes[s], lc.dual, cb.sym[s], lc.coder));
             }
-            { StageTimer tm(ctx, st, ST_ELEM, (double)nc * (4 + 4 + 1)); GP_TRY(assemble_occ(st, cb.sym, spos, nc, chi.occ)); }
+            GP_TRY(dec_level_occ(ctx, st, m, cb.sym, spos, nc, chi.occ, g + 2 < L && !child_plan, top_mk, &pF_ready));
         }
         HIP_TRY(hipEventRecord(ctx->ev_main, st));
         if (g == 0 && d_early < L) GP_TRY(parse_levels(d_early, L, ctx->ev_tables));
diff --git a/gauspcc_amd/csrc/codec_shared.hip b/gauspcc_amd/csrc/codec_shared.hip
--- a/gauspcc_amd/csrc/codec_shared.hip
+++ b/gauspcc_amd/csrc/codec_shared.hip
@@ -127,17 +127,20 @@
     }
     TAKE(cX, float, nC * m->C); TAKE(cA, float, nC * m->C); TAKE(cB, float, nC * m->C);
     { StageTimer tm(ctx, st, ST_ELEM, (double)nC * (128 + 12 + 128)); GP_TRY(child_features(st, pA, parentC, rkeyC, m->temb, nC, cX, m->C)); }
-    GP_TRY(run_trunk(ctx, 1, st, m, 5, Trunk{cX, cA, cB}, tilesC, nC));
+    GP_TRY(dbg_mark(ctx, st, 41, cX, (size_t)nC * 4 * m->C));
     TAKE(u1, float, nC * m->C); TAKE(u2, float, nC * m->C); TAKE(u3, float, nC * m->C);
+    const bool fan_on = conv_fanout_ok(tilesC, nC, m->C);
+    const ConvFan fan = {{m->semb[0], m->semb[1], m->semb[2]}, occC, {u1, u2, u3}};
+    GP_TRY(run_trunk(ctx, 1, st, m, 5, Trunk{cX, cA, cB}, tilesC, nC, nullptr, nullptr, fan_on ? &fan : nullptr));
     TAKE(v1, float, nC * m->C); TAKE(v2, float, nC * m->C);
     float *u[4] = {cA, u1, u2, u3};
     float *v[4] = {cX, cB, v1, v2};
-    {
-        const float *const embs[3] = {m->semb[0], m->semb[1], m->semb[2]};
-        float *const outs[3] = {u1, u2, u3};
+    if (!fan_on) {
         StageTimer tm(ctx, st, ST_ELEM, (double)nC * (128 + 1 + 3 * 128));
-        GP_TRY(stage_inputs_gt(st, cA, embs, occC, nC, outs, m->C));
-    }
+        GP_TRY(stage_inputs_gt(st, cA, fan.emb, occC, nC, fan.out, m->C));
+    }
+    for (int s = 1; s < 4; ++s) GP_TRY(dbg_mark(ctx, st, 41 + s, u[s], (size_t)nC * 4 * m->C));
+    GP_TRY(dbg_mark(ctx, st, 45, occP, (size_t)nP)); GP_TRY(dbg_mark(ctx, st, 46, occC, (size_t)nC));
     ConvBatch cb = {}; cb.C = m->C;
     for (int s = 0; s < 4; ++s) cb.job[s] = ConvJob{u[s], m->conv[10 + 2 * s], nullptr, v[s]};
     GP_TRY(sparse_conv(ctx, 1, st, cb, 4, tilesC, nC, 1));
@@ -246,7 +249,7 @@
 }
 
 int dec_parent_trunk(gpcc_ctx *ctx, hipStream_t st, const gpcc_model *m, int g, const uint8_t *occ, int64_t np, const ConvTiles &tilesP, const PairPlan &planP, int64_t planP_np,
-                     int fmode, float **pA_out, bool *any_fused)
+                     int fmode, float **pA_out, bool *any_fused, const float *pF_ready)
 {
     TAKE_TOP(pF, float, np * m->C); TAKE_TOP(pA, float, np * m->C); TAKE_TOP(pB, float, np * m->C);
     float *Pp = nullptr;
@@ -258,13 +261,29 @@
         if (ctx->prof.on) { GP_TRY(prof_event(ctx, st, &rec.e1)); ctx->prof.recs.push_back(rec); }
         *any_fused = true;
     } else {
-        { StageTimer tm(ctx, st, ST_ELEM, (double)np * 129); GP_TRY(embed_occ(st, m->prior_emb, occ, np, pF, m->C)); }
+        if (!pF_ready || pF != pF_ready) { StageTimer tm(ctx, st, ST_ELEM, (double)np * 129); GP_TRY(embed_occ(st, m->prior_emb, occ, np, pF, m->C)); }
         GP_TRY(dbg_mark(ctx, st, g * 100 + 1, pF, (size_t)np * 128));
         GP_TRY(run_trunk(ctx, g, st, m, 0, Trunk{pF, pA, pB}, tilesP, np, planP.valid() ? &planP : nullptr, Pp));
     }
     GP_TRY(dbg_mark(ctx, st, g * 100 + 2, pA, (size_t)np * 128));
     *pA_out = pA;
     return GPCC_OK;
+}
+
+int dec_level_occ(gpcc_ctx *ctx, hipStream_t st, const gpcc_model *m, const uint8_t *const sym[4], const uint32_t *m2r, int64_t nc, uint8_t *occ, bool next_trunk_on_tiles,
+                  size_t top_mk, const float **pF_ready)
+{
+    *pF_ready = nullptr;
+    float *pF = nullptr;
+    if (next_trunk_on_tiles && conv_fanout_on() && m->C == 32 && nc > 64 * 256) pF = ctx->arena.peek_top<float>(top_mk, (size_t)nc * 32);
+    if (pF) {
+        StageTimer tm(ctx, st, ST_ELEM, (double)nc * (4 + 4 + 1 + 128));
+        GP_TRY(assemble_embed_occ(st, sym, m2r, nc, occ, m->prior_emb, pF));
+        *pF_ready = pF;
+        return GPCC_OK;
+    }
+    StageTimer tm(ctx, st, ST_ELEM, (double)nc * (4 + 4 + 1));
+    return assemble_occ(st, sym, m2r, nc, occ);
 }
 
 int dec_child_lists(gpcc_ctx *ctx, hipStream_t sd, const gpcc_model *m, const Level *cur, const int32_t *cellP, const Level *chi, int32_t *cellC, bool child_plan,
diff --git a/gauspcc_amd/csrc/codec_shared.hpp b/gauspcc_amd/csrc/codec_shared.hpp
--- a/gauspcc_amd/csrc/codec_shared.hpp
+++ b/gauspcc_amd/csrc/codec_shared.hpp
@@ -12,20 +12,20 @@
 struct Trunk { float *x, *a, *b; };
 
 static inline int run_trunk(gpcc_ctx *ctx, int level, hipStream_t st, const gpcc_model *m, int conv0, const Trunk &t, const ConvTiles &tiles, int64_t n, const PairPlan *plan = nullptr,
-              float *P = nullptr)
+              float *P = nullptr, const ConvFan *last_fan = nullptr)
 {
     ConvBatch cb = {}; cb.C = m->C;
-    auto one = [&](const float *in, int ci, const float *res, float *out) {
+    auto one = [&](const float *in, int ci, const float *res, float *out, const ConvFan *fan = nullptr) {
         cb.job[0] = ConvJob{in, m->conv[ci], res, out};
-        if (plan) return plan_conv(st, *plan, cb.job[0], P, 1);
-        return sparse_conv(ctx, level, st, cb, 1, tiles, n, 1);
+        if (plan) return fan ? fail(GPCC_ERR_ARG, "internal: copy-out fan-out on a pair plan") : plan_conv(st, *plan, cb.job[0], P, 1);
+        return sparse_conv(ctx, level, st, cb, 1, tiles, n, 1, fan);
     };
     GP_TRY(conv_chain_begin(ctx, st));
     GP_TRY(one(t.x, conv0, nullptr, t.a));
     GP_TRY(one(t.a, conv0 + 1, nullptr, t.b));
     GP_TRY(one(t.b, conv0 + 2, t.a, t.x));
     GP_TRY(one(t.x, conv0 + 3, nullptr, t.b));
-    GP_TRY(one(t.b, conv0 + 4, t.x, t.a));
+    GP_TRY(one(t.b, conv0 + 4, t.x, t.a, last_fan));
     GP_TRY(conv_chain_end(ctx, st));
     return GPCC_OK;
 }
@@ -74,7 +74,9 @@
 int alloc_level(gpcc_ctx *ctx, Level *lv, int64_t n, int lvl);
 
 int dec_parent_trunk(gpcc_ctx *ctx, hipStream_t st, const gpcc_model *m, int g, const uint8_t *occ, int64_t np, const ConvTiles &tilesP, const PairPlan &planP, int64_t planP_np,
-                     int fmode, float **pA, bool *any_fused);
+                     int fmode, float **pA, bool *any_fused, const float *pF_ready = nullptr);
+int dec_level_occ(gpcc_ctx *ctx, hipStream_t st, const gpcc_model *m, const uint8_t *const sym[4], const uint32_t *m2r, int64_t nc, uint8_t *occ, bool next_trunk_on_tiles,
+                  size_t top_mk, const float **pF_ready);
 int dec_child_lists(gpcc_ctx *ctx, hipStream_t sd, const gpcc_model *m, const Level *cur, const int32_t *cellP, const Level *chi, int32_t *cellC, bool child_plan,
                     unsigned long long *pairs_dev, PairPlan *planC, ConvTiles *tilesC);
 
diff --git a/gauspcc_amd/csrc/common.hpp b/gauspcc_amd/csrc/common.hpp
--- a/gauspcc_amd/csrc/common.hpp
+++ b/gauspcc_amd/csrc/common.hpp
@@ -74,6 +74,12 @@
         top -= bytes;
         if (flip && top < top_low) top_low = top;
         return reinterpret_cast<T *>(base + top);
+    }
+    template <typename T> T *peek_top(size_t m, size_t count) const
+    {
+        const size_t bytes = (count * sizeof(T) + 255) & ~size_t(255);
+        if (flip || off + bytes > m) return nullptr;
+        return reinterpret_cast<T *>(base + (m - bytes));
     }
     size_t top_mark() const { return top; }
     void top_rewind(size_t m) { top = m; }
diff --git a/gauspcc_amd/csrc/network.hip b/gauspcc_amd/csrc/network.hip
--- a/gauspcc_amd/csrc/network.hip
+++ b/gauspcc_amd/csrc/network.hip
@@ -73,6 +73,8 @@
     return (int)std::min<int64_t>(R, std::max<int64_t>(H, 16));
 }
 
+__device__ __forceinline__ float4 add4(float4 a, float4 b) { return make_float4(a.x + b.x, a.y + b.y, a.z + b.z, a.w + b.w); }
+
 #ifdef CONV_TIMING
 __device__ unsigned long long g_conv_timing[16];
 #define CT_STAMP(v) const long long v = clock64()
@@ -85,8 +87,12 @@
 #else
 #define CONV_MIN_WAVES(R, ASM) ((ASM) || (R) >= 128 ? 2 : (R) >= 96 ? 3 : 4)
 #endif
-template <int R, int DIST, bool ASM, int PAIR = 0>
-__global__ __launch_bounds__(64 * SC_WAVES, CONV_MIN_WAVES(R, ASM)) void k_sparse_conv(ConvBatch jobs, ConvTiles T, int n, int relu, int njobs)
+template <int FAN> struct ConvFanArg {};
+template <> struct ConvFanArg<1> { const float4 *e1, *e2, *e3; const uint8_t *occ; float4 *o1, *o2, *o3; };
+constexpr int FAN_TAB4 = (2 + 4 + 16) * 8;
+static_assert(FAN_TAB4 * 4 <= HDR_DWORDS, "the stage tables fit the tile-header ring");
+template <int R, int DIST, bool ASM, int PAIR = 0, int FAN = 0>
+__global__ __launch_bounds__(64 * SC_WAVES, CONV_MIN_WAVES(R, ASM)) void k_sparse_conv(ConvBatch jobs, ConvTiles T, int n, int relu, int njobs, ConvFanArg<FAN> fan)
 {
 #ifdef CONV_ONE_PER_SIMD
     asm volatile("" ::: "a0", "a1", "a2", "a3", "a4", "a5", "a6", "a7", "a8", "a9", "a10", "a11", "a12", "a13", "a14", "a15", "a16", "a17", "a18", "a19", "a20", "a21", "a22", "a23",
@@ -306,6 +312,22 @@
 #pragma unroll
             for (int g8 = 0; g8 < NG; ++g8) r[g8] = res4[min(g8 * 64 + lane, nvec - 1)];
         }
+        uint32_t occw = 0;
+        float4 *ftab = reinterpret_cast<float4 *>(hdr);
+        if constexpr (FAN == 1) {
+            const uint8_t *__restrict__ po = fan.occ + row0;
+            const float4 *fe1 = fan.e1, *fe2 = fan.e2, *fe3 = fan.e3;
+#pragma unroll
+            for (int j = 0; j < 4; ++j) occw |= (uint32_t)po[min(lane * 4 + j, nrows - 1)] << (8 * j);
+            asm volatile("" ::: "memory");
+            static_assert(FAN_TAB4 > 128 && FAN_TAB4 <= 192, "three float4 per lane cover the tables");
+            const float4 ta = lane < 16 ? fe1[lane] : lane < 48 ? fe2[lane - 16] : fe3[lane - 48];
+            const float4 tb = fe3[lane + 16];
+            const float4 tc = fe3[min(lane, 47) + 80];
+            ftab[lane] = ta;
+            ftab[lane + 64] = tb;
+            if (lane < 48) ftab[lane + 128] = tc;
+        }
 #ifdef CONV_TIMING
         long long te[NB + 1];
         te[0] = clock64();
@@ -330,6 +352,22 @@
 #pragma unroll
                 for (int b = 0; b < 8; ++b)
                     if (bt * 8 + b < NG && (bt * 8 + b) * 64 + lane < nvec) out4[(bt * 8 + b) * 64 + lane] = v[b];
+                if constexpr (FAN == 1) {
+                    const int c = lane & 7;
+                    float4 *__restrict__ o1 = fan.o1 + (size_t)row0 * 8, *__restrict__ o2 = fan.o2 + (size_t)row0 * 8, *__restrict__ o3 = fan.o3 + (size_t)row0 * 8;
+#pragma unroll
+                    for (int b = 0; b < 8; ++b)
+                        if (bt * 8 + b < NG) {
+                            const int g8 = bt * 8 + b;
+                            const uint32_t o = ((uint32_t)__shfl((int)occw, 2 * g8 + (lane >> 5)) >> (8 * ((lane >> 3) & 3))) & 255u;
+                            const float4 a1 = ftab[((o >> 7) & 1u) * 8 + c], a2 = ftab[16 + ((o >> 6) & 3u) * 8 + c], a3 = ftab[48 + ((o >> 4) & 15u) * 8 + c];
+                            if (g8 * 64 + lane < nvec) {
+                                o1[g8 * 64 + lane] = add4(v[b], a1);
+                                o2[g8 * 64 + lane] = add4(v[b], a2);
+                                o3[g8 * 64 + lane] = add4(v[b], a3);
+                            }
+                        }
+                }
             }
 #ifdef CONV_TIMING
             te[bt + 1] = clock64();
@@ -617,10 +655,21 @@
     return GPCC_OK;
 }
 
-int sparse_conv(gpcc_ctx *ctx, int level, hipStream_t st, const ConvBatch &jobs, int njobs, const ConvTiles &T, int64_t n, int relu)
+bool conv_fanout_on()
+{
+    static const bool on = dev_env_int("GAUSPCC_CONV_FANOUT", 1) != 0;
+    return on;
+}
+bool conv_fanout_ok(const ConvTiles &T, int64_t n, int C)
+{
+    return conv_fanout_on() && C == 32 && T.R == 255 && n > 0 && n < ((int64_t)1 << 25) && !conv_is_coop(n, T.R);
+}
+
+int sparse_conv(gpcc_ctx *ctx, int level, hipStream_t st, const ConvBatch &jobs, int njobs, const ConvTiles &T, int64_t n, int relu, const ConvFan *fan)
 {
     if (n <= 0) return GPCC_OK;
     if (n >= (int64_t)1 << 31) return fail(GPCC_ERR_ARG, "level too large");
+    if (fan && (njobs != 1 || !conv_fanout_ok(T, n, jobs.C ? jobs.C : 32))) return fail(GPCC_ERR_ARG, "internal: copy-out fan-out on a launch that cannot carry it");
     if (jobs.C != 0 && jobs.C != 32) return any_sparse_conv(st, jobs, njobs, T, n, relu, jobs.C);
     const bool chained = ctx && ctx->prof.on && ctx->prof.chain_open;
     const bool prof = ctx && ctx->prof.on && !chained;
@@ -637,6 +686,9 @@
         HIP_TRY(hipFuncSetAttribute(reinterpret_cast<const void *>(k_sparse_conv<255, 1, true>), hipFuncAttributeMaxDynamicSharedMemorySize, SC_WAVES * conv_lds_wave_floats(255) * 4));
         HIP_TRY(hipFuncSetAttribute(reinterpret_cast<const void *>(k_sparse_conv<255, 1, true, 1>), hipFuncAttributeMaxDynamicSharedMemorySize, SC_WAVES * conv_lds_wave_floats(255) * 4));
         HIP_TRY(hipFuncSetAttribute(reinterpret_cast<const void *>(k_sparse_conv<255, 1, false>), hipFuncAttributeMaxDynamicSharedMemorySize, SC_WAVES * conv_lds_wave_floats(255) * 4));
+        HIP_TRY(hipFuncSetAttribute(reinterpret_cast<const void *>(k_sparse_conv<255, 1, true, 0, 1>), hipFuncAttributeMaxDynamicSharedMemorySize, SC_WAVES * conv_lds_wave_floats(255) * 4));
+        HIP_TRY(hipFuncSetAttribute(reinterpret_cast<const void *>(k_sparse_conv<255, 1, true, 1, 1>), hipFuncAttributeMaxDynamicSharedMemorySize, SC_WAVES * conv_lds_wave_floats(255) * 4));
+        HIP_TRY(hipFuncSetAttribute(reinterpret_cast<const void *>(k_sparse_conv<255, 1, false, 0, 1>), hipFuncAttributeMaxDynamicSharedMemorySize, SC_WAVES * conv_lds_wave_floats(255) * 4));
         HIP_TRY(hipFuncSetAttribute(reinterpret_cast<const void *>(k_sparse_conv<128, 1, false>), hipFuncAttributeMaxDynamicSharedMemorySize, bytes));
         HIP_TRY(hipFuncSetAttribute(reinterpret_cast<const void *>(k_sparse_conv_coop<16>), hipFuncAttributeMaxDynamicSharedMemorySize, (int)coop_lds_bytes(343, 16)));
         HIP_TRY(hipFuncSetAttribute(reinterpret_cast<const void *>(k_sparse_conv_coop<32>), hipFuncAttributeMaxDynamicSharedMemorySize, (int)coop_lds_bytes(125, 32)));
@@ -708,14 +760,21 @@
     dim3 grid((unsigned)cdiv(T.nblk * njobs, SC_WAVES), 1u);
     const size_t lds_bytes = (size_t)SC_WAVES * conv_lds_wave_floats(T.R) * 4;
     const bool asm_ok = use_asm && n < ((int64_t)1 << 25);
-#define CONV_LAUNCH(RR, DD, AA) k_sparse_conv<RR, DD, AA><<<grid, 64 * SC_WAVES, lds_bytes, st>>>(jobs, T, (int)n, relu, njobs)
+#define CONV_LAUNCH(RR, DD, AA) k_sparse_conv<RR, DD, AA><<<grid, 64 * SC_WAVES, lds_bytes, st>>>(jobs, T, (int)n, relu, njobs, ConvFanArg<0>{})
     switch (T.R) {
     case 16: if (asm_ok) CONV_LAUNCH(16, 1, true); else CONV_LAUNCH(16, 1, false); break;
     case 32: if (asm_ok) CONV_LAUNCH(32, 1, true); else CONV_LAUNCH(32, 1, false); break;
     case 64: if (asm_ok) CONV_LAUNCH(64, 1, true); else CONV_LAUNCH(64, 1, false); break;
     case 96: if (asm_ok) CONV_LAUNCH(96, 1, true); else CONV_LAUNCH(96, 1, false); break;
     case 255:
-        if (asm_ok && T.paired) k_sparse_conv<255, 1, true, 1><<<grid, 64 * SC_WAVES, lds_bytes, st>>>(jobs, T, (int)n, relu, njobs);
+        if (fan) {
+            const ConvFanArg<1> fa = {(const float4 *)fan->emb[0], (const float4 *)fan->emb[1], (const float4 *)fan->emb[2], fan->occ,
+                                      (float4 *)fan->out[0], (float4 *)fan->out[1], (float4 *)fan->out[2]};
+            if (asm_ok && T.paired) k_sparse_conv<255, 1, true, 1, 1><<<grid, 64 * SC_WAVES, lds_bytes, st>>>(jobs, T, (int)n, relu, njobs, fa);
+            else if (asm_ok) k_sparse_conv<255, 1, true, 0, 1><<<grid, 64 * SC_WAVES, lds_bytes, st>>>(jobs, T, (int)n, relu, njobs, fa);
+            else k_sparse_conv<255, 1, false, 0, 1><<<grid, 64 * SC_WAVES, lds_bytes, st>>>(jobs, T, (int)n, relu, njobs, fa);
+        }
+        else if (asm_ok && T.paired) k_sparse_conv<255, 1, true, 1><<<grid, 64 * SC_WAVES, lds_bytes, st>>>(jobs, T, (int)n, relu, njobs, ConvFanArg<0>{});
         else if (asm_ok) CONV_LAUNCH(255, 1, true);
         else CONV_LAUNCH(255, 1, false);
         break;
@@ -847,8 +906,6 @@
     return GPCC_OK;
 }
 
-__device__ __forceinline__ float4 add4(float4 a, float4 b) { return make_float4(a.x + b.x, a.y + b.y, a.z + b.z, a.w + b.w); }
-
 __global__ __launch_bounds__(TB) void k_child_features(const float4 *__restrict__ F, const uint32_t *__restrict__ parent, const uint64_t *__restrict__ rkey_c,
                                                        const float4 *__restrict__ temb, int64_t n, float4 *__restrict__ out)
 {
@@ -928,6 +985,25 @@
     return GPCC_OK;
 }
 
+__global__ __launch_bounds__(TB) void k_assemble_embed_occ(SymPtrs sp, const uint32_t *__restrict__ m2r, int64_t n, uint8_t *__restrict__ occ, const float4 *__restrict__ emb,
+                                                           float4 *__restrict__ out)
+{
+    int64_t t = (int64_t)blockIdx.x * TB + threadIdx.x;
+    int64_t i = t >> 3;
+    if (i >= n) return;
+    const uint32_t r = m2r[i];
+    const uint8_t o = (uint8_t)(sp.s[0][r] * 128 + sp.s[1][r] * 64 + sp.s[2][r] * 16 + sp.s[3][r]);
+    if ((t & 7) == 0) occ[i] = o;
+    out[t] = emb[(size_t)o * 8 + (t & 7)];
+}
+int assemble_embed_occ(hipStream_t st, const uint8_t *const sym_r[4], const uint32_t *m2r, int64_t n, uint8_t *occ, const float *emb, float *out)
+{
+    SymPtrs sp = {{sym_r[0], sym_r[1], sym_r[2], sym_r[3]}};
+    k_assemble_embed_occ<<<nblk(n * 8), TB, 0, st>>>(sp, m2r, n, occ, (const float4 *)emb, (float4 *)out);
+    LAUNCH_CHECK();
+    return GPCC_OK;
+}
+
 __global__ __launch_bounds__(TB) void k_rows_permute(const float *__restrict__ in, float *__restrict__ out, int64_t n, int to_physical)
 {
     int64_t t = (int64_t)blockIdx.x * TB + threadIdx.x;
diff --git a/gauspcc_amd/csrc/network.hpp b/gauspcc_amd/csrc/network.hpp
--- a/gauspcc_amd/csrc/network.hpp
+++ b/gauspcc_amd/csrc/network.hpp
@@ -95,7 +95,9 @@
 int tiles_dense_map(hipStream_t st, const Level *par, const int32_t *cell_par, const Level *chi, int32_t *cell_own, int k, int32_t *nbr, uint16_t *rk, uint32_t *rowcnt);
 int tiles_view(gpcc_ctx *ctx, hipStream_t st, const TilePool &pool, int l0, int l1, const int64_t *row_base, ConvTiles *T);
 
-int sparse_conv(gpcc_ctx *ctx, int level, hipStream_t st, const ConvBatch &jobs, int njobs, const ConvTiles &T, int64_t n, int relu);
+struct ConvFan { const float *emb[3]; const uint8_t *occ; float *out[3]; };
+bool conv_fanout_ok(const ConvTiles &T, int64_t n, int C);
+int sparse_conv(gpcc_ctx *ctx, int level, hipStream_t st, const ConvBatch &jobs, int njobs, const ConvTiles &T, int64_t n, int relu, const ConvFan *fan = nullptr);
 int conv_chain_begin(gpcc_ctx *ctx, hipStream_t st);
 int conv_chain_end(gpcc_ctx *ctx, hipStream_t st);
 int prof_collect(gpcc_ctx *ctx, const unsigned long long *pairs_per_level, int nlevels);
@@ -120,6 +122,8 @@
 int head_cdf(hipStream_t st, const HeadArgs &a);
 
 int assemble_occ(hipStream_t st, const uint8_t *const sym_r[4], const uint32_t *m2r, int64_t n, uint8_t *occ);
+int assemble_embed_occ(hipStream_t st, const uint8_t *const sym_r[4], const uint32_t *m2r, int64_t n, uint8_t *occ, const float *emb, float *out);
+bool conv_fanout_on();
 
 int any_embed_occ(hipStream_t st, const float *emb, const uint8_t *occ, int64_t n, float *out, int C);
 int any_child_features(hipStream_t st, const float *F, const uint32_t *parent, const uint64_t *rkey_c, const float *temb, int64_t n, float *out, int C);
```

Measured after the change: 21.14, median of 6. Within noise of the previous version (+0.1%).
